# paTRICK-swk/D3DP

Hardware: AMD Instinct MI355X
Metric: pose-hypotheses/sec (H x clips) at F=243, J=17, H=20, K=10 (higher is better)
Workload: dtype f16x2-split operands on fp16 MFMA, f32 accumulate (fp32-class: meets 1e-3 mm)

## Files before the change

d3dp_amd/csrc/capi.hip:

```cpp
#include <hip/hip_runtime.h>

#include <cmath>
#include <cstdarg>
#include <cstdio>
#include <cstdlib>
#include <cstring>
#include <string>
#include <vector>

#include "../../include/d3dp_hip.h"
#include "common.h"
#include "kernels.h"

namespace {

thread_local std::string g_err;

int fail(int code, const char* fmt, ...) {
  char buf[512];
  va_list ap;
  va_start(ap, fmt);
  vsnprintf(buf, sizeof buf, fmt, ap);
  va_end(ap);
  g_err = buf;
  return code;
}

#define HIP_TRY(expr)                                                                      \
  do {                                                                                     \
    hipError_t e__ = (expr);                                                               \
    if (e__ != hipSuccess) return fail(D3DP_EHIP, "%s: %s", #expr, hipGetErrorString(e__)); \
  } while (0)

#define LAUNCH_TRY(expr)                                                          \
  do {                                                                            \
    int r__ = (expr);                                                             \
    if (r__ != 0) return fail(r__ == -1 ? D3DP_EINVAL : D3DP_ENOTSUP, "%s -> %d", #expr, r__); \
  } while (0)

}

int d3dp_set_error(int code, const char* msg) { return fail(code, "%s", msg); }
int d3dp_check_launch(const char* what) {
  hipError_t e = hipGetLastError();
  if (e != hipSuccess) return fail(D3DP_EHIP, "%s: %s", what, hipGetErrorString(e));
  return D3DP_OK;
}

namespace {

enum ProfClass { P_QKV = 0, P_PROJ, P_FC1, P_FC2, P_ATTN_S, P_ATTN_T, P_LN, P_LN2, P_EMBED, P_HEAD, P_TIME, P_OTHER,
                 T_LINEAR, T_WGRAD, T_ATTN_FWD_S, T_ATTN_FWD_T, T_ATTN_BQ_S, T_ATTN_BQ_T, T_ATTN_BKV_S, T_ATTN_BKV_T, T_OPERAND,
                 T_LN_FWD, T_LN_BWD, T_OTHER,
                 P_EMPTY };
static_assert(P_EMPTY + 1 == D3DP_PROFILE_CLASSES, "include/d3dp_hip.h: D3DP_PROFILE_CLASSES");
const char* kClassNames[D3DP_PROFILE_CLASSES] = {"gemm_qkv", "gemm_proj", "gemm_fc1", "gemm_fc2", "attn_spatial",
                                                 "attn_temporal", "layernorm", "norm_pair", "embed_ln", "head",
                                                 "time_mlp", "other",
                                                 "train_linear", "train_wgrad", "train_attn_fwd_spatial", "train_attn_fwd_temporal",
                                                 "train_attn_bwd_q_spatial", "train_attn_bwd_q_temporal", "train_attn_bwd_kv_spatial",
                                                 "train_attn_bwd_kv_temporal", "train_operand_pass", "train_ln_fwd", "train_ln_bwd",
                                                 "train_other", "event_pair_overhead"};

struct BlockDev {
  const float *n1w, *n1b, *n2w, *n2b, *qkv_b, *proj_b, *fc1_b, *fc2_b;
  const void *qkv_w, *proj_w, *fc1_w, *fc2_w;
  float qkv_u = 1.f, proj_u = 1.f, fc1_u = 1.f, fc2_u = 1.f;
  const float* fc1_c12 = nullptr;
  float s_kv = kActScale, s_h = kActScale;
};

template <typename E>
__global__ void to_bf16_kernel(const float* __restrict__ s, E* __restrict__ d, size_t n) {
  size_t i = (size_t)blockIdx.x * blockDim.x + threadIdx.x;
  const size_t stride = (size_t)gridDim.x * blockDim.x;
  for (; i < n; i += stride) d[i] = (E)s[i];
}

void launch_to_bf16(const float* s, void* d, size_t n, hipStream_t st, int f16 = 0) {
  const unsigned blocks = (unsigned)std::min<size_t>((n + 255) / 256, 4096);
  if (f16) hipLaunchKernelGGL(to_bf16_kernel<_Float16>, dim3(blocks ? blocks : 1), dim3(256), 0, st, s, (_Float16*)d, n);
  else hipLaunchKernelGGL(to_bf16_kernel<__bf16>, dim3(blocks ? blocks : 1), dim3(256), 0, st, s, (__bf16*)d, n);
}

__device__ __forceinline__ unsigned f32_bits_up(double v) {
  float f = (float)v;
  if ((double)f < v) f = __uint_as_float(__float_as_uint(f) + 1u);
  return __float_as_uint(f) & 0x7fffffffu;
}
__device__ __forceinline__ unsigned wave_max_u(unsigned v) {
#pragma unroll
  for (int o = 32; o > 0; o >>= 1) { const unsigned t = (unsigned)__shfl_xor((int)v, o, 64); v = t > v ? t : v; }
  return v;
}
__global__ __launch_bounds__(256) void fast16_bound_kernel(const float* __restrict__ W, const float* __restrict__ gamma,
                                                           const float* __restrict__ beta, const unsigned* __restrict__ cin,
                                                           const float* __restrict__ bias, int N, int K, double sq, int n_tail,
                                                           unsigned* o_sum, unsigned* o_tail, unsigned* o_in, unsigned* o_w) {
  const int lane = threadIdx.x & 63;
  const int n = blockIdx.x * 4 + (threadIdx.x >> 6);
  if (n >= N) return;
  const double c = cin ? (double)__uint_as_float(cin[0]) : 0.0;
  double a = 0.0;
  unsigned inmax = 0u, wmax = 0u;
  for (int k = lane; k < K; k += 64) {
    const float w = fabsf(W[(size_t)n * K + k]);
    const double in = gamma ? sq * (double)fabsf(gamma[k]) + (double)fabsf(beta[k]) : c;
    const unsigned ib = f32_bits_up(in), wb = __float_as_uint(w);
    inmax = ib > inmax ? ib : inmax;
    wmax = wb > wmax ? wb : wmax;
    a += (double)w * in;
  }
#pragma unroll
  for (int o = 32; o > 0; o >>= 1) a += __shfl_xor(a, o, 64);
  inmax = wave_max_u(inmax);
  wmax = wave_max_u(wmax);
  if (lane == 0) {
    const unsigned sb = f32_bits_up((a + (double)fabsf(bias[n])) * (1.0 + 0x1p-40));
    atomicMax(o_sum, sb);
    if (o_tail && n >= n_tail) atomicMax(o_tail, sb);
    if (o_in) atomicMax(o_in, inmax);
    atomicMax(o_w, wmax);
  }
}
constexpr int kF16Slots = 11;

constexpr size_t kAlign = 256;
size_t align_up(size_t v) { return (v + kAlign - 1) / kAlign * kAlign; }

}

struct d3dp_ctx {
  d3dp_cfg cfg{};
  int device = 0;
  bool weights_set = false;
  float range_bound = 0.f;
  size_t ln_slice_floats = 0;
  unsigned* d_flag = nullptr;
  char* arena = nullptr;
  size_t arena_bytes = 0;
  const float *spos = nullptr, *tpos = nullptr, *ew = nullptr, *eb = nullptr, *freq = nullptr, *t1w = nullptr,
              *t1b = nullptr, *t3w = nullptr, *t3b = nullptr, *snw = nullptr, *snb = nullptr, *tnw = nullptr,
              *tnb = nullptr, *hnw = nullptr, *hnb = nullptr, *hw = nullptr, *hb = nullptr;
  std::vector<BlockDev> ste, tte;
  bool prof = false;
  struct Ev { hipEvent_t a, b; int cls; };
  std::vector<Ev> pool;
  size_t used = 0;
  int64_t counts[D3DP_PROFILE_CLASSES] = {0};
  double total_ms[D3DP_PROFILE_CLASSES] = {0};

  bool fast16() const { return cfg.mode == D3DP_MODE_FAST16; }
  bool fast() const { return cfg.mode == D3DP_MODE_FAST || fast16(); }
  int fast_f16 = 0;
  float fast_bound = 0.f;
  int exact_impl = 0;
  int exact_impl_req = 0;
  bool impl_fallback = false;
  bool train() const { return cfg.mode == D3DP_MODE_TRAIN; }
  bool exact() const { return !fast() && !train(); }
  bool x2() const { return exact() && exact_impl == 0; }
  bool long_rows = false;
  bool x2_attn() const { return x2() && cfg.channels / cfg.heads == 64 && (cfg.frames <= 256 || !long_rows); }
  bool fold_resid() const { return x2() && fold; }
  bool fold = true;
  bool fold_ln() const { return fold_resid() && fold_ln_on && 2 * cfg.hidden <= 2048; }
  bool fold_ln_on = false;
  bool skew() const { return x2_attn() && skew_d > 0 && cfg.channels >= 128 * skew_d; }
  int skew_d = 0;
  int seq_pitch() const {
    const int fj = cfg.frames * cfg.joints;
    return (pad_override < 0 ? skew() : (pad_override > 0 && x2_attn())) ? (fj + 63) / 64 * 64 : fj;
  }
  int pad_override = -1;
  bool train_x2 = true;
  hipStream_t aux = nullptr;
  hipEvent_t ev_fork = nullptr, ev_done[2] = {nullptr, nullptr};
  bool train_overlap = true;
  int train_overlap_sets = 2;
  bool train_gelu_in_prep = true;
  bool train_ln_direct = true;
  bool train_wgrad_merged = true;
  bool train_tail_blocks = true;
  int train_attn_x2 = 2;
  int pingpong = 0;
  bool x3() const { return exact() && exact_impl == 1; }
  int act() const { return fast() ? (fast_f16 ? 4 : 1) : (x3() ? 2 : (x2() ? 3 : 0)); }
  size_t act_size() const { return fast() ? 2 : (x3() ? 6 : 4); }
  size_t wide_size() const { return fast() ? 2 : 4; }
  size_t y_size() const { return fast() ? 2 : 4; }
  int chunk() const { return cfg.chunk_seqs != 0 ? std::abs(cfg.chunk_seqs) : (exact() ? 31 : 15); }
  int n_cu = 0;
  std::vector<int> plan_cache;
  int plan_total = -1;
  const std::vector<int>& plan(int total) {
    if (total == plan_total) return plan_cache;
    const int cap = std::min(chunk(), total), SP = seq_pitch();
    plan_cache.clear();
    plan_total = total;
    if (!x2() || cfg.chunk_seqs < 0 || n_cu <= 0) {
      for (int s0 = 0; s0 < total; s0 += cap) plan_cache.push_back(std::min(cap, total - s0));
      return plan_cache;
    }
    const long tn[4] = {(3 * cfg.channels + 127) / 128, (cfg.channels + 127) / 128, (cfg.hidden + 127) / 128,
                        (cfg.channels + 127) / 128};
    const long kd[4] = {cfg.channels, cfg.channels, cfg.channels, cfg.hidden};
    const bool sk[4] = {skew(), false, skew(), false};
    std::vector<double> cost(cap + 1, 0.0);
    for (int n = 1; n <= cap; ++n) {
      const long R = ((long)n * SP + 255) / 256;
      for (int k = 0; k < 4; ++k) {
        const long Q = n_cu / tn[k];
        if (sk[k] && Q >= 1) cost[n] += ((double)((R + std::min(Q, R) - 1) / std::min(Q, R)) + 3.0 * skew_d * 32.0 / (double)kd[k]) * (double)kd[k];
        else cost[n] += (double)((R * tn[k] + n_cu - 1) / n_cu) * (double)kd[k];
      }
      cost[n] += 1e-3 * (double)kd[0];
    }
    std::vector<double> best(total + 1, 1e300);
    std::vector<int> pick(total + 1, 0);
    best[0] = 0.0;
    for (int b = 1; b <= total; ++b)
      for (int n = 1; n <= std::min(cap, b); ++n)
        if (best[b - n] + cost[n] < best[b]) { best[b] = best[b - n] + cost[n]; pick[b] = n; }
    for (int b = total; b > 0; b -= pick[b]) plan_cache.push_back(pick[b]);
    return plan_cache;
  }

  int flush_events() {
    for (size_t i = 0; i < used; ++i) {
      if (hipEventSynchronize(pool[i].b) != hipSuccess) return -1;
      float ms = 0.f;
      if (hipEventElapsedTime(&ms, pool[i].a, pool[i].b) != hipSuccess) return -1;
      counts[pool[i].cls]++;
      total_ms[pool[i].cls] += ms;
    }
    used = 0;
    return 0;
  }
  int begin(int cls, hipStream_t st) {
    if (!prof) return -1;
    if (used == pool.size()) {
      if (pool.size() >= 32768) { if (flush_events() != 0) return -1; }
      else {
        Ev e{};
        if (hipEventCreateWithFlags(&e.a, hipEventDisableSystemFence) != hipSuccess || hipEventCreateWithFlags(&e.b, hipEventDisableSystemFence) != hipSuccess) return -1;
        pool.push_back(e);
      }
    }
    pool[used].cls = cls;
    (void)hipEventRecord(pool[used].a, st);
    return (int)used++;
  }
  void end(int slot, hipStream_t st) {
    if (slot >= 0) (void)hipEventRecord(pool[slot].b, st);
  }
};

namespace {

struct Scope {
  d3dp_ctx* c; int slot; hipStream_t st;
  Scope(d3dp_ctx* c_, int cls, hipStream_t st_) : c(c_), slot(c_ ? c_->begin(cls, st_) : -1), st(st_) {}
  ~Scope() { if (c) c->end(slot, st); }
};

int linear(d3dp_ctx* c, int cls, int epi, int out_f32, const void* A, const void* W, float wu, const float* bias, void* out,
           int M, int N, int K, hipStream_t st, void* out2 = nullptr, float* aux = nullptr, float a_scale = kActScale,
           float o_scale = kActScale) {
  Scope s(c, cls, st);
  if (c->fast()) return d3dp_launch_linear_bf16_stream(epi, out_f32, A, W, bias, out, M, N, K, st, c->fast_f16);
  if (c->x2()) {
    if (cls == P_QKV && c->x2_attn()) epi = EPI_QKV_PACK;
    const int skew_d = c->skew() && (epi == EPI_QKV_PACK || epi == EPI_GELU) ? c->skew_d : 0;
    const int rev = cls == P_PROJ ? X2_TILES_LAST_TO_FIRST : 0;
    return d3dp_launch_linear_f16x2(epi, A, W, bias, wu / a_scale, o_scale, (float*)out, out2 ? out2 : out, aux, c->d_flag, M, N,
                                    K, st, skew_d, c->pingpong | rev);
  }
  if (c->x3()) return d3dp_launch_linear_bf16x3(epi, A, W, bias, (float*)out, out, M, N, K, st);
  return d3dp_launch_linear_f32(epi, (const float*)A, (const float*)W, bias, (float*)out, M, N, K, st);
}

SeqMap spatial_map(int F, int J, int sp = 0) { return sp > F * J ? SeqMap{J, F, sp, J, 1} : SeqMap{J, 1, J, 0, 1}; }
SeqMap temporal_map(int F, int J, int sp = 0) { return SeqMap{F, J, sp > F * J ? sp : F * J, 1, J}; }

int attention(d3dp_ctx* c, int axis, const void* qkv, void* out, int n_bh, float s_kv, hipStream_t st) {
  const d3dp_cfg& g = c->cfg;
  Scope s(c, axis == 0 ? P_ATTN_S : P_ATTN_T, st);
  if (c->x2_attn())
    return d3dp_launch_attn_x2(3, axis, qkv, out, axis == 0 ? n_bh * g.frames : n_bh * g.joints,
                               axis == 0 ? spatial_map(g.frames, g.joints, c->seq_pitch())
                                         : temporal_map(g.frames, g.joints, c->seq_pitch()),
                               g.channels, g.heads, s_kv, st);
  const bool fast_mfma = c->fast() && g.channels / g.heads == 64;
  if (axis == 0) {
    if (fast_mfma && g.joints <= 32)
      return d3dp_launch_attn_spatial_bf16(qkv, out, n_bh * g.frames, spatial_map(g.frames, g.joints), g.channels,
                                           g.heads, st, c->fast_f16);
    if (fast_mfma && !c->long_rows)
      return d3dp_launch_attn_temporal_bf16(qkv, out, n_bh * g.frames, spatial_map(g.frames, g.joints), g.channels,
                                            g.heads, st, c->fast_f16);
    return d3dp_launch_attn_rows(c->act(), qkv, out, n_bh * g.frames, spatial_map(g.frames, g.joints), g.channels,
                                 g.heads, st);
  }
  if (fast_mfma && (g.frames <= 256 || !c->long_rows))
    return d3dp_launch_attn_temporal_bf16(qkv, out, n_bh * g.joints, temporal_map(g.frames, g.joints), g.channels,
                                          g.heads, st, c->fast_f16);
  if (c->exact() && g.channels / g.heads == 64 && g.frames <= 256)
    return d3dp_launch_attn_temporal_f32(c->act(), qkv, out, n_bh * g.joints, temporal_map(g.frames, g.joints),
                                         g.channels, g.heads, st);
  return d3dp_launch_attn_rows(c->act(), qkv, out, n_bh * g.joints, temporal_map(g.frames, g.joints), g.channels,
                               g.heads, st);
}

int run_block(d3dp_ctx* c, const BlockDev& w, int axis, float* x, void* y1, void* y, void* bufA, void* bufB, float* lnst,
              int n_bh, hipStream_t st) {
  const d3dp_cfg& g = c->cfg;
  const int Tc = n_bh * c->seq_pitch(), C = g.channels;
  const float s_o = c->x2_attn() ? w.s_kv : kActScale;
  LAUNCH_TRY(linear(c, P_QKV, EPI_BIAS, 0, bufA, w.qkv_w, w.qkv_u, w.qkv_b, bufB, Tc, 3 * C, C, st, nullptr, nullptr, kActScale, s_o));
  LAUNCH_TRY(attention(c, axis, bufB, bufA, n_bh, s_o, st));
  const bool fold = c->fold_resid();
  if (c->fold_ln()) {
    float* slices = lnst;
    float* rowstat = lnst + (size_t)c->ln_slice_floats;
    LAUNCH_TRY(linear(c, P_PROJ, EPI_RESID_LN, 0, bufA, w.proj_w, w.proj_u, w.proj_b, x, Tc, C, C, st, y1, slices, s_o));
    {
      Scope s(c, P_LN, st);
      d3dp_launch_ln_combine(slices, rowstat, Tc, C, g.eps_block, st);
    }
    LAUNCH_TRY(linear(c, P_FC1, EPI_GELU_LN, 0, y1, w.fc1_w, w.fc1_u, w.fc1_c12, bufB, Tc, g.hidden, C, st, bufB, rowstat, kActScale, w.s_h));
  } else {
  LAUNCH_TRY(linear(c, P_PROJ, fold ? EPI_RESID : EPI_BIAS, 0, bufA, w.proj_w, w.proj_u, w.proj_b, fold ? (void*)x : y1, Tc, C, C, st, nullptr, nullptr, s_o));
  {
    Scope s(c, P_LN, st);
    LAUNCH_TRY(d3dp_launch_ln(c->act(), x, fold ? nullptr : y1, 0, w.n2w, w.n2b, g.eps_block, bufA, Tc, C, st));
  }
  LAUNCH_TRY(linear(c, P_FC1, EPI_GELU, 0, bufA, w.fc1_w, w.fc1_u, w.fc1_b, bufB, Tc, g.hidden, C, st, nullptr, nullptr, kActScale, w.s_h));
  }
  LAUNCH_TRY(linear(c, P_FC2, fold ? EPI_RESID : EPI_BIAS, 0, bufB, w.fc2_w, w.fc2_u, w.fc2_b, fold ? (void*)x : y, Tc, C, g.hidden, st, nullptr, nullptr, w.s_h));
  return 0;
}

int read_switches(d3dp_ctx* c, bool width_inst) {
  const d3dp_cfg& g = c->cfg;
  const char* xf = getenv("D3DP_EXACT_IMPL");
  c->exact_impl = c->exact_impl_req = (xf && !strcmp(xf, "bf16x3")) ? 1 : (xf && !strcmp(xf, "f32")) ? 2 : 0;
  if (!width_inst) {
    if (c->exact_impl_req == 1)
      return fail(D3DP_ENOTSUP, "D3DP_EXACT_IMPL=bf16x3 exists for channels in {64,128,256,512}; channels=%d runs the fp32 implementation", g.channels);
    c->exact_impl = c->exact_impl_req = 2;
  }
  const char* lr = getenv("D3DP_LONG_ATTN");
  c->long_rows = lr && !strcmp(lr, "rows");
  const char* nf = getenv("D3DP_NO_FOLD");
  c->fold = !(nf && nf[0] == '1');
  const char* ti = getenv("D3DP_TRAIN_IMPL");
  c->train_x2 = !(ti && !strcmp(ti, "f32")) && width_inst;
  const char* ov = getenv("D3DP_TRAIN_OVERLAP");
  c->train_overlap = !(ov && ov[0] == '0');
  c->train_overlap_sets = (ov && ov[0] == '1') ? 1 : 2;
  const char* tg = getenv("D3DP_TRAIN_GELU");
  c->train_gelu_in_prep = !(tg && !strcmp(tg, "pass"));
  const char* tw = getenv("D3DP_TRAIN_WGRAD");
  c->train_wgrad_merged = !(tw && !strcmp(tw, "each"));
  const char* tl = getenv("D3DP_TRAIN_LN_OPERAND");
  c->train_ln_direct = !(tl && !strcmp(tl, "pass"));
  const char* tt = getenv("D3DP_TRAIN_TAIL");
  c->train_tail_blocks = !(tt && !strcmp(tt, "split"));
  const char* ta = getenv("D3DP_TRAIN_ATTN");
  c->train_attn_x2 = (ta && !strcmp(ta, "f32")) ? 0 : (ta && !strcmp(ta, "x2t")) ? 1 : 2;
  if ((!c->train_gelu_in_prep || !c->train_wgrad_merged || !c->train_tail_blocks || !c->train_ln_direct) && !d3dp_x2_variants_built())
    return fail(D3DP_ENOTSUP, "D3DP_TRAIN_WGRAD=each / D3DP_TRAIN_TAIL=split / D3DP_TRAIN_GELU=pass / D3DP_TRAIN_LN_OPERAND=pass select superseded launch forms of the "
                              "training step that only the variants build honours (make -C d3dp_amd/csrc variants; "
                              "D3DP_LIB=d3dp_amd/lib/variants/libd3dp_variants.so)");
  {
    const char* sk = getenv("D3DP_X2_SKEW");
    const char* pp = getenv("D3DP_X2_PP");
    const char* wide = getenv("D3DP_X2_WIDE");
    const char* pd = getenv("D3DP_SEQ_PAD");
    const char* nl = getenv("D3DP_FOLD_LN");
    int skew_d = 0, pingpong = 0, pad = -1;
    if (sk && (sk[0] == '0' || sk[0] == '1' || sk[0] == '2' || sk[0] == '4') && sk[1] == 0) skew_d = sk[0] - '0';
    if (pp && (pp[0] == '0' || pp[0] == '1') && pp[1] == 0) pingpong = pp[0] - '0';
    if (wide && wide[0] == '1' && wide[1] == 0) pingpong = 2;
    if (pd && (pd[0] == '0' || pd[0] == '1') && pd[1] == 0) pad = pd[0] - '0';
    const bool fold_ln = nl && nl[0] == '1';
    if ((skew_d || pingpong || pad > 0 || fold_ln) && !d3dp_x2_variants_built())
      return fail(D3DP_ENOTSUP, "D3DP_X2_SKEW / D3DP_X2_PP / D3DP_X2_WIDE / D3DP_SEQ_PAD / D3DP_FOLD_LN select experiment kernels that this "
                                "library was built without (make -C d3dp_amd/csrc variants; D3DP_LIB=d3dp_amd/lib/variants/libd3dp_variants.so)");
    c->skew_d = skew_d; c->pingpong = pingpong; c->pad_override = pad; c->fold_ln_on = fold_ln;
  }
  return D3DP_OK;
}

}

extern "C" {

int d3dp_abi_version(void) { return D3DP_ABI_VERSION; }
int d3dp_debug_x2_variants(void) { return d3dp_x2_variants_built() ? 1 : 0; }
int d3dp_debug_train_linear(const float* A, const float* W, const float* bias, float* out, int32_t M, int32_t N, int32_t K,
                            int32_t tail, unsigned* amax_out, int32_t amax_pos, void* stream) {
  if (!A || !W || !out || M < 1 || N < 4 || N % 4 || K < 32 || K % 32) return fail(D3DP_EINVAL, "d3dp_debug_train_linear: bad argument");
  hipStream_t st = (hipStream_t)stream;
  char* buf = nullptr;
  const size_t a_bytes = (size_t)M * K * 4, w_bytes = (size_t)N * K * 4;
  HIP_TRY(hipMalloc((void**)&buf, a_bytes + w_bytes + 64));
  unsigned* amax = reinterpret_cast<unsigned*>(buf + a_bytes + w_bytes);
  float* uns = reinterpret_cast<float*>(amax + 8);
  int rc = hipMemsetAsync(amax, 0, 64, st) == hipSuccess ? 0 : -3;
  if (!rc) {
    d3dp_launch_absmax(A, (size_t)M * K, amax, st);
    d3dp_launch_absmax(W, (size_t)N * K, amax + 1, st);
    d3dp_launch_split2_dyn(A, buf, M, K, K, amax, uns, st);
    d3dp_launch_split2_dyn(W, buf + a_bytes, N, K, K, amax + 1, uns + 1, st);
    rc = d3dp_launch_linear_f16x2_dyn(buf, buf + a_bytes, bias, uns, uns + 1, out, M, N, K, 1, st, amax_out, amax_pos, tail);
  }
  const hipError_t e = hipStreamSynchronize(st);
  (void)hipFree(buf);
  if (rc) return fail(rc == -3 ? D3DP_EHIP : D3DP_EINVAL, "d3dp_debug_train_linear: launch refused (%d)", rc);
  if (e != hipSuccess) return fail(D3DP_EHIP, "d3dp_debug_train_linear: %s", hipGetErrorString(e));
  return 0;
}
const char* d3dp_last_error(void) { return g_err.c_str(); }
const char* d3dp_profile_class_name(int32_t cls) {
  return (cls >= 0 && cls < D3DP_PROFILE_CLASSES) ? kClassNames[cls] : "";
}

int d3dp_create(const d3dp_cfg* cfg, d3dp_ctx** out) {
  if (!cfg || !out) return fail(D3DP_EINVAL, "d3dp_create: null argument");
  const d3dp_cfg& g = *cfg;
  if (g.frames < 1 || g.frames > 1024) return fail(D3DP_ENOTSUP, "frames=%d not in [1,1024]", g.frames);
  if (g.joints < 1 || g.joints > 256) return fail(D3DP_ENOTSUP, "joints=%d not in [1,256]", g.joints);
  if (g.heads < 1 || g.channels < 1 || g.channels % g.heads) return fail(D3DP_EINVAL, "heads=%d does not divide channels=%d", g.heads, g.channels);
  if (g.depth < 1) return fail(D3DP_EINVAL, "depth=%d", g.depth);
  if (g.mode != D3DP_MODE_EXACT && g.mode != D3DP_MODE_FAST && g.mode != D3DP_MODE_TRAIN && g.mode != D3DP_MODE_FAST16)
    return fail(D3DP_EINVAL, "mode=%d", g.mode);
  const int hd = g.channels / g.heads;
  const bool width_inst = (g.channels == 64 || g.channels == 128 || g.channels == 256 || g.channels == 512) &&
                          (hd == 8 || hd == 16 || hd == 32 || hd == 64) && g.hidden >= 64 && g.hidden % 64 == 0;
  if (!width_inst) {
    if (g.mode == D3DP_MODE_FAST)
      return fail(D3DP_ENOTSUP, "channels=%d heads=%d hidden=%d: FAST contexts exist for channels in {64,128,256,512} with head dim in "
                                "{8,16,32,64} and hidden a multiple of 64; other widths run in D3DP_MODE_EXACT / D3DP_MODE_TRAIN (fp32 implementation)",
                  g.channels, g.heads, g.hidden);
    if (g.mode == D3DP_MODE_FAST16)
      return fail(D3DP_ENOTSUP, "channels=%d heads=%d hidden=%d: FAST16 contexts exist for the shapes FAST contexts exist for -- channels in "
                                "{64,128,256,512} with head dim in {8,16,32,64} and hidden a multiple of 64; other widths run in D3DP_MODE_EXACT / "
                                "D3DP_MODE_TRAIN (fp32 implementation)",
                  g.channels, g.heads, g.hidden);
    if (g.channels > 1024 || g.channels % 4 || hd % 4 || hd > 128 || g.hidden < 4 || g.hidden % 4)
      return fail(D3DP_ENOTSUP, "channels=%d heads=%d hidden=%d: the fp32 implementation takes channels <= 1024, head dim a multiple of 4 up to 128 "
                                "and hidden a multiple of 4", g.channels, g.heads, g.hidden);
    const int nmax = std::max(g.frames, g.joints), cap = hd <= 16 ? 16 : hd <= 32 ? 32 : hd <= 64 ? 64 : 128;
    if (g.mode == D3DP_MODE_TRAIN && (nmax > 256 || (size_t)nmax * (8 * (cap + 4) + 12) > 160 * 1024))
      return fail(D3DP_ENOTSUP, "channels=%d heads=%d frames=%d joints=%d: training at a width outside {64,128,256,512} runs the fp32 attention "
                                "backward, which holds a whole sequence in LDS (<= 256 tokens; <= 153 at head dims above 64)",
                  g.channels, g.heads, g.frames, g.joints);
  }
  int ndev = 0;
  if (hipGetDeviceCount(&ndev) != hipSuccess || ndev < 1)
    return fail(D3DP_EHIP, "no HIP device visible: libd3dp_hip has no CPU fallback");
  d3dp_ctx* c = new d3dp_ctx();
  c->cfg = g;
  c->fast_f16 = c->fast16() ? 1 : (c->fast() ? D3DP_FAST_F16 : 0);
  if (const int rc = read_switches(c, width_inst); rc != D3DP_OK) {
    delete c;
    return rc;
  }
  HIP_TRY(hipGetDevice(&c->device));
  {
    hipDeviceProp_t prop;
    HIP_TRY(hipGetDeviceProperties(&prop, c->device));
    c->n_cu = prop.multiProcessorCount;
  }
  if (hipMalloc((void**)&c->d_flag, sizeof(unsigned)) != hipSuccess || hipMemset(c->d_flag, 0, sizeof(unsigned)) != hipSuccess) {
    delete c;
    return fail(D3DP_EHIP, "d3dp_create: cannot allocate the status word");
  }
  if (g.mode == D3DP_MODE_TRAIN && c->train_x2 && c->train_overlap && g.channels % 32 == 0 && g.hidden % 32 == 0) {
    bool ok = hipStreamCreateWithFlags(&c->aux, hipStreamNonBlocking) == hipSuccess &&
              hipEventCreateWithFlags(&c->ev_fork, hipEventDisableTiming) == hipSuccess;
    for (hipEvent_t& e : c->ev_done) ok = ok && hipEventCreateWithFlags(&e, hipEventDisableTiming) == hipSuccess;
    if (!ok) {
      (void)d3dp_destroy(c);
      return fail(D3DP_EHIP, "d3dp_create: cannot create the training step's second stream and its events");
    }
  }
  *out = c;
  return D3DP_OK;
}

int d3dp_destroy(d3dp_ctx* c) {
  if (!c) return D3DP_OK;
  for (auto& e : c->pool) { (void)hipEventDestroy(e.a); (void)hipEventDestroy(e.b); }
  if (c->arena) (void)hipFree(c->arena);
  if (c->d_flag) (void)hipFree(c->d_flag);
  if (c->ev_fork) (void)hipEventDestroy(c->ev_fork);
  for (hipEvent_t e : c->ev_done)
    if (e) (void)hipEventDestroy(e);
  if (c->aux) (void)hipStreamDestroy(c->aux);
  delete c;
  return D3DP_OK;
}

int d3dp_set_weights(d3dp_ctx* c, const d3dp_weights* w, void* stream) {
  if (!c || !w || !w->ste || !w->tte) return fail(D3DP_EINVAL, "d3dp_set_weights: null argument");
  hipStream_t st = (hipStream_t)stream;
  const d3dp_cfg& g = c->cfg;
  const size_t C = g.channels, Hd = g.hidden, J = g.joints, F = g.frames;
  c->range_bound = 0.f;
  c->impl_fallback = false;
  c->plan_total = -1;
  std::vector<float> blk_scale(4 * (size_t)g.depth, kActScale);
  if (c->exact() && c->exact_impl_req == 0) {
    c->exact_impl = 0;
    const size_t nb = 2 * (size_t)g.depth;
    unsigned* dbound = nullptr;
    HIP_TRY(hipMalloc((void**)&dbound, nb * 6 * sizeof(unsigned)));
    struct Free { unsigned* p; ~Free() { (void)hipFree(p); } } free_dbound{dbound};
    HIP_TRY(hipMemsetAsync(dbound, 0, nb * 6 * sizeof(unsigned), st));
    for (int kind = 0; kind < 2; ++kind)
      for (int d = 0; d < g.depth; ++d) {
        const d3dp_block_weights& b = (kind == 0 ? w->ste : w->tte)[d];
        if (!b.norm1_w || !b.norm1_b || !b.qkv_w || !b.qkv_b || !b.norm2_w || !b.norm2_b || !b.fc1_w || !b.fc1_b || !b.proj_w ||
            !b.fc2_w)
          return fail(D3DP_EINVAL, "d3dp_set_weights: a weight pointer is null");
        unsigned* o = dbound + ((size_t)kind * g.depth + d) * 6;
        d3dp_launch_rowbound(b.qkv_w, b.norm1_w, b.norm1_b, b.qkv_b, 3 * (int)C, (int)C, o, st);
        d3dp_launch_rowbound(b.fc1_w, b.norm2_w, b.norm2_b, b.fc1_b, (int)Hd, (int)C, o + 2, st);
        d3dp_launch_absmax(b.proj_w, C * C, o + 4, st);
        d3dp_launch_absmax(b.fc2_w, C * Hd, o + 5, st);
      }
    std::vector<float> hb(nb * 6);
    HIP_TRY(hipMemcpyAsync(hb.data(), dbound, nb * 6 * sizeof(float), hipMemcpyDeviceToHost, st));
    HIP_TRY(hipStreamSynchronize(st));
    const float kSafe = 65504.0f / kActScale;
    auto pick = [&](float bound) {
      float sc = kActScale;
      while (!(bound * sc < 65504.0f) && sc > 1e-30f) sc *= 0.5f;
      return sc;
    };
    float worst = 0.f;
    bool fallback = false;
    for (size_t i = 0; i < nb; ++i) {
      const float bq = hb[6 * i], bl1 = hb[6 * i + 1], bh = hb[6 * i + 2], bl2 = hb[6 * i + 3];
      if (!(bq < INFINITY) || !(bh < INFINITY) || !(bl1 < INFINITY) || !(bl2 < INFINITY) || !(hb[6 * i + 4] < INFINITY) ||
          !(hb[6 * i + 5] < INFINITY)) {
        fallback = true;
        worst = INFINITY;
        continue;
      }
      worst = std::max(worst, std::max(std::max(bq, bh), std::max(bl1, bl2)));
      if (!(bl1 < kSafe) || !(bl2 < kSafe)) fallback = true;
      if (!(bq < kSafe) && !c->x2_attn()) fallback = true;
      blk_scale[2 * i] = pick(bq);
      blk_scale[2 * i + 1] = pick(bh);
    }
    c->range_bound = std::min(worst, 3.0e38f);
    if (fallback) {
      c->exact_impl = 1;
      c->impl_fallback = true;
      std::fill(blk_scale.begin(), blk_scale.end(), kActScale);
    }
  }
  if (c->fast16()) {
    const size_t nb = 2 * (size_t)g.depth;
    unsigned* dbound = nullptr;
    HIP_TRY(hipMalloc((void**)&dbound, nb * kF16Slots * sizeof(unsigned)));
    struct Free { unsigned* p; ~Free() { (void)hipFree(p); } } free_dbound{dbound};
    HIP_TRY(hipMemsetAsync(dbound, 0, nb * kF16Slots * sizeof(unsigned), st));
    const double sq = std::sqrt((double)C - 1.0);
    for (int kind = 0; kind < 2; ++kind)
      for (int d = 0; d < g.depth; ++d) {
        const d3dp_block_weights& b = (kind == 0 ? w->ste : w->tte)[d];
        if (!b.norm1_w || !b.norm1_b || !b.qkv_w || !b.qkv_b || !b.proj_w || !b.proj_b || !b.norm2_w || !b.norm2_b || !b.fc1_w ||
            !b.fc1_b || !b.fc2_w || !b.fc2_b) return fail(D3DP_EINVAL, "d3dp_set_weights: a weight pointer is null");
        unsigned* o = dbound + ((size_t)kind * g.depth + d) * kF16Slots;
        const dim3 blk(256);
        hipLaunchKernelGGL(fast16_bound_kernel, dim3((3 * (unsigned)C + 3) / 4), blk, 0, st, b.qkv_w, b.norm1_w, b.norm1_b,
                           (const unsigned*)nullptr, b.qkv_b, 3 * (int)C, (int)C, sq, 2 * (int)C, o + 1, o + 2, o + 0, o + 7);
        hipLaunchKernelGGL(fast16_bound_kernel, dim3(((unsigned)C + 3) / 4), blk, 0, st, b.proj_w, (const float*)nullptr,
                           (const float*)nullptr, (const unsigned*)(o + 2), b.proj_b, (int)C, (int)C, 0.0, 0, o + 3,
                           (unsigned*)nullptr, (unsigned*)nullptr, o + 8);
        hipLaunchKernelGGL(fast16_bound_kernel, dim3(((unsigned)Hd + 3) / 4), blk, 0, st, b.fc1_w, b.norm2_w, b.norm2_b,
                           (const unsigned*)nullptr, b.fc1_b, (int)Hd, (int)C, sq, 0, o + 5, (unsigned*)nullptr, o + 4, o + 9);
        hipLaunchKernelGGL(fast16_bound_kernel, dim3(((unsigned)C + 3) / 4), blk, 0, st, b.fc2_w, (const float*)nullptr,
                           (const float*)nullptr, (const unsigned*)(o + 5), b.fc2_b, (int)C, (int)Hd, 0.0, 0, o + 6,
                           (unsigned*)nullptr, (unsigned*)nullptr, o + 10);
      }
    HIP_TRY(hipGetLastError());
    std::vector<float> hb(nb * kF16Slots);
    HIP_TRY(hipMemcpyAsync(hb.data(), dbound, hb.size() * sizeof(float), hipMemcpyDeviceToHost, st));
    HIP_TRY(hipStreamSynchronize(st));
    float worst = 0.f;
    bool finite = true;
    for (const float v : hb) {
      if (!(v < INFINITY)) finite = false;
      else worst = std::max(worst, v);
    }
    c->fast_bound = finite ? worst : INFINITY;
    c->fast_f16 = (finite && worst < 65504.0f) ? 1 : 0;
  }
  const size_t ws = c->fast() ? 2 : (c->x3() ? 6 : 4);
  size_t off = 0;
  auto take = [&](size_t bytes) { size_t o = off; off += align_up(bytes); return o; };
  struct Item { const void* src; size_t n; bool mat; size_t off; };
  std::vector<Item> items;
  auto add = [&](const void* src, size_t n, bool mat) {
    items.push_back({src, n, mat, take(n * (mat ? ws : 4))});
    return items.size() - 1;
  };
  const size_t i_spos = add(w->spatial_pos, J * C, false), i_tpos = add(w->temporal_pos, F * C, false);
  const size_t i_ew = add(w->embed_w, C * 5, false), i_eb = add(w->embed_b, C, false);
  const size_t i_fr = add(w->time_freq, C / 2, false);
  const size_t i_t1w = add(w->time1_w, 2 * C * C, false), i_t1b = add(w->time1_b, 2 * C, false);
  const size_t i_t3w = add(w->time3_w, 2 * C * C, false), i_t3b = add(w->time3_b, C, false);
  const size_t i_snw = add(w->spatial_norm_w, C, false), i_snb = add(w->spatial_norm_b, C, false);
  const size_t i_tnw = add(w->temporal_norm_w, C, false), i_tnb = add(w->temporal_norm_b, C, false);
  const size_t i_hnw = add(w->head_norm_w, C, false), i_hnb = add(w->head_norm_b, C, false);
  const size_t i_hw = add(w->head_w, 3 * C, false), i_hb = add(w->head_b, 3, false);
  struct BI { size_t v[13]; };
  std::vector<BI> bis;
  std::vector<float*> temps;
  struct TempFree { std::vector<float*>& t; ~TempFree() { for (float* p : t) (void)hipFree(p); } } temp_free{temps};
  for (int kind = 0; kind < 2; ++kind)
    for (int d = 0; d < g.depth; ++d) {
      const d3dp_block_weights& b = (kind == 0 ? w->ste : w->tte)[d];
      if (!b.norm1_w || !b.norm1_b || !b.qkv_w || !b.qkv_b || !b.proj_w || !b.proj_b || !b.norm2_w || !b.norm2_b || !b.fc1_w ||
          !b.fc1_b || !b.fc2_w || !b.fc2_b) return fail(D3DP_EINVAL, "d3dp_set_weights: a weight pointer is null");
      BI bi;
      bi.v[0] = add(b.norm1_w, C, false); bi.v[1] = add(b.norm1_b, C, false);
      bi.v[2] = add(b.qkv_w, 3 * C * C, true); bi.v[3] = add(b.qkv_b, 3 * C, false);
      bi.v[4] = add(b.proj_w, C * C, true); bi.v[5] = add(b.proj_b, C, false);
      bi.v[6] = add(b.norm2_w, C, false); bi.v[7] = add(b.norm2_b, C, false);
      if (c->fold_ln()) {
        float *wp = nullptr, *c12 = nullptr;
        HIP_TRY(hipMalloc((void**)&wp, Hd * C * 4)); temps.push_back(wp);
        HIP_TRY(hipMalloc((void**)&c12, 2 * Hd * 4)); temps.push_back(c12);
        d3dp_launch_fold_ln(b.fc1_w, b.norm2_w, b.norm2_b, b.fc1_b, wp, c12, (int)Hd, (int)C, st);
        bi.v[8] = add(wp, Hd * C, true); bi.v[9] = add(b.fc1_b, Hd, false); bi.v[12] = add(c12, 2 * Hd, false);
      } else {
        bi.v[8] = add(b.fc1_w, Hd * C, true); bi.v[9] = add(b.fc1_b, Hd, false); bi.v[12] = bi.v[9];
      }
      bi.v[10] = add(b.fc2_w, C * Hd, true); bi.v[11] = add(b.fc2_b, C, false);
      bis.push_back(bi);
    }
  for (auto& it : items)
    if (!it.src) return fail(D3DP_EINVAL, "d3dp_set_weights: a weight pointer is null");
  if (!c->arena || c->arena_bytes < off) {
    if (c->arena) HIP_TRY(hipFree(c->arena));
    c->arena = nullptr;
    HIP_TRY(hipMalloc((void**)&c->arena, off));
    c->arena_bytes = off;
  }
  std::vector<float> unscale(items.size(), 1.f);
  if (c->x2()) {
    size_t n_mat = 0;
    for (auto& it : items) n_mat += it.mat;
    unsigned* dmax = nullptr;
    HIP_TRY(hipMalloc((void**)&dmax, n_mat * sizeof(unsigned)));
    HIP_TRY(hipMemsetAsync(dmax, 0, n_mat * sizeof(unsigned), st));
    size_t k = 0;
    for (auto& it : items)
      if (it.mat) d3dp_launch_absmax((const float*)it.src, it.n, dmax + k++, st);
    std::vector<float> hmax(n_mat);
    HIP_TRY(hipMemcpyAsync(hmax.data(), dmax, n_mat * sizeof(float), hipMemcpyDeviceToHost, st));
    HIP_TRY(hipStreamSynchronize(st));
    HIP_TRY(hipFree(dmax));
    k = 0;
    for (size_t i = 0; i < items.size(); ++i) {
      if (!items[i].mat) continue;
      const float mx = hmax[k++];
      if (!(mx < INFINITY)) return fail(D3DP_EINVAL, "d3dp_set_weights: a weight matrix holds inf/nan");
      int e = 0;
      if (mx > 0.f) frexpf(mx, &e);
      unscale[i] = ldexpf(1.f, e - 14);
    }
  }
  for (size_t i = 0; i < items.size(); ++i) {
    auto& it = items[i];
    if (it.mat && c->fast()) launch_to_bf16((const float*)it.src, c->arena + it.off, it.n, st, c->fast_f16);
    else if (it.mat && c->x3()) d3dp_launch_split3((const float*)it.src, c->arena + it.off, it.n, st);
    else if (it.mat && c->x2()) d3dp_launch_split2((const float*)it.src, c->arena + it.off, it.n, 1.0f / unscale[i], st);
    else HIP_TRY(hipMemcpyAsync(c->arena + it.off, it.src, it.n * 4, hipMemcpyDeviceToDevice, st));
  }
  HIP_TRY(hipGetLastError());
  HIP_TRY(hipStreamSynchronize(st));
  auto F32 = [&](size_t i) { return (const float*)(c->arena + items[i].off); };
  auto ANY = [&](size_t i) { return (const void*)(c->arena + items[i].off); };
  c->spos = F32(i_spos); c->tpos = F32(i_tpos); c->ew = F32(i_ew); c->eb = F32(i_eb); c->freq = F32(i_fr);
  c->t1w = F32(i_t1w); c->t1b = F32(i_t1b); c->t3w = F32(i_t3w); c->t3b = F32(i_t3b);
  c->snw = F32(i_snw); c->snb = F32(i_snb); c->tnw = F32(i_tnw); c->tnb = F32(i_tnb);
  c->hnw = F32(i_hnw); c->hnb = F32(i_hnb); c->hw = F32(i_hw); c->hb = F32(i_hb);
  c->ste.clear(); c->tte.clear();
  for (size_t k = 0; k < bis.size(); ++k) {
    const BI& bi = bis[k];
    BlockDev b{F32(bi.v[0]), F32(bi.v[1]), F32(bi.v[6]), F32(bi.v[7]), F32(bi.v[3]), F32(bi.v[5]), F32(bi.v[9]),
               F32(bi.v[11]), ANY(bi.v[2]), ANY(bi.v[4]), ANY(bi.v[8]), ANY(bi.v[10]),
               unscale[bi.v[2]], unscale[bi.v[4]], unscale[bi.v[8]], unscale[bi.v[10]], F32(bi.v[12]),
               blk_scale[2 * k], blk_scale[2 * k + 1]};
    (k < (size_t)g.depth ? c->ste : c->tte).push_back(b);
  }
  c->weights_set = true;
  return D3DP_OK;
}

int d3dp_set_weights_borrowed(d3dp_ctx* c, const d3dp_weights* w) {
  if (!c || !w || !w->ste || !w->tte) return fail(D3DP_EINVAL, "d3dp_set_weights_borrowed: null argument");
  if (!c->train()) return fail(D3DP_ESTATE, "d3dp_set_weights_borrowed needs a D3DP_MODE_TRAIN context (fp32 weights)");
  c->spos = w->spatial_pos; c->tpos = w->temporal_pos; c->ew = w->embed_w; c->eb = w->embed_b; c->freq = w->time_freq;
  c->t1w = w->time1_w; c->t1b = w->time1_b; c->t3w = w->time3_w; c->t3b = w->time3_b;
  c->snw = w->spatial_norm_w; c->snb = w->spatial_norm_b; c->tnw = w->temporal_norm_w; c->tnb = w->temporal_norm_b;
  c->hnw = w->head_norm_w; c->hnb = w->head_norm_b; c->hw = w->head_w; c->hb = w->head_b;
  const float* top[] = {c->spos, c->tpos, c->ew, c->eb, c->freq, c->t1w, c->t1b, c->t3w, c->t3b, c->snw, c->snb, c->tnw,
                        c->tnb, c->hnw, c->hnb, c->hw, c->hb};
  for (const float* p : top)
    if (!p) return fail(D3DP_EINVAL, "d3dp_set_weights_borrowed: a weight pointer is null");
  c->ste.clear(); c->tte.clear();
  for (int kind = 0; kind < 2; ++kind)
    for (int d = 0; d < c->cfg.depth; ++d) {
      const d3dp_block_weights& b = (kind == 0 ? w->ste : w->tte)[d];
      const void* all[] = {b.norm1_w, b.norm1_b, b.qkv_w, b.qkv_b, b.proj_w, b.proj_b, b.norm2_w, b.norm2_b, b.fc1_w,
                           b.fc1_b, b.fc2_w, b.fc2_b};
      for (const void* p : all)
        if (!p) return fail(D3DP_EINVAL, "d3dp_set_weights_borrowed: a weight pointer is null");
      BlockDev bd{b.norm1_w, b.norm1_b, b.norm2_w, b.norm2_b, b.qkv_b, b.proj_b, b.fc1_b, b.fc2_b, b.qkv_w, b.proj_w,
                  b.fc1_w, b.fc2_w};
      (kind == 0 ? c->ste : c->tte).push_back(bd);
    }
  c->weights_set = true;
  return D3DP_OK;
}

int d3dp_workspace_bytes(const d3dp_ctx* c, int32_t B, int32_t H, size_t* bytes) {
  if (!c || !bytes || B < 1 || H < 1) return fail(D3DP_EINVAL, "d3dp_workspace_bytes: bad argument");
  const d3dp_cfg& g = c->cfg;
  const size_t n = (size_t)std::min(c->chunk(), B * H);
  const size_t Tc = n * c->seq_pitch(), C = g.channels;
  const size_t wide = (size_t)std::max(3 * g.channels, g.hidden);
  *bytes = align_up((size_t)B * C * 4) + align_up(Tc * C * 4) + 2 * align_up(Tc * C * c->y_size()) +
           align_up(Tc * C * c->act_size()) + align_up(Tc * wide * c->wide_size()) +
           (c->fold_ln() ? align_up(Tc * ((C + 63) / 64) * 8) + align_up((Tc + 256) * 8) : 0);
  return D3DP_OK;
}

int d3dp_denoise(d3dp_ctx* c, const float* x2d, const float* x_t, const int64_t* t, float* out, int32_t B, int32_t H,
                 void* workspace, size_t workspace_bytes, void* stream) {
  if (!c || !x2d || !x_t || !t || !out || !workspace || B < 1 || H < 1)
    return fail(D3DP_EINVAL, "d3dp_denoise: bad argument");
  if (!c->weights_set) return fail(D3DP_ESTATE, "d3dp_denoise: weights not set");
  size_t need = 0;
  d3dp_workspace_bytes(c, B, H, &need);
  if (workspace_bytes < need) return fail(D3DP_ESTATE, "workspace %zu < required %zu bytes", workspace_bytes, need);
  hipStream_t st = (hipStream_t)stream;
  const d3dp_cfg& g = c->cfg;
  const int C = g.channels, F = g.frames, J = g.joints, FJ = F * J, SP = c->seq_pitch();
  const int BH = B * H, chunk = std::min(c->chunk(), BH);
  const size_t Tmax = (size_t)chunk * SP;
  char* p = (char*)workspace;
  float* temb = (float*)p; p += align_up((size_t)B * C * 4);
  float* x = (float*)p;    p += align_up(Tmax * C * 4);
  void* y1 = p;            p += align_up(Tmax * C * c->y_size());
  void* y = p;             p += align_up(Tmax * C * c->y_size());
  void* bufA = p;          p += align_up(Tmax * C * c->act_size());
  void* bufB = p;          p += align_up(Tmax * (size_t)std::max(3 * g.channels, g.hidden) * c->wide_size());
  float* lnst = (float*)p;
  c->ln_slice_floats = align_up(Tmax * ((C + 63) / 64) * 8) / 4;

  {
    Scope s(c, P_TIME, st);
    LAUNCH_TRY(d3dp_launch_time_mlp(t, c->freq, c->t1w, c->t1b, c->t3w, c->t3b, temb, B, C, st));
  }
  int seq0 = 0;
  for (const int n : c->plan(BH)) {
    const int Tc = n * SP;
    {
      Scope s(c, P_EMBED, st);
      LAUNCH_TRY(d3dp_launch_embed_ln(c->act(), x2d, x_t, temb, c->ew, c->eb, c->spos, c->ste[0].n1w, c->ste[0].n1b,
                                      g.eps_block, x, bufA, seq0, n, H, F, J, C, st, SP));
    }
    const bool fold = c->fold_resid();
    for (int d = 0; d < g.depth; ++d) {
      int r = run_block(c, c->ste[d], 0, x, y1, y, bufA, bufB, lnst, n, st);
      if (r) return r;
      {
        Scope s(c, P_LN2, st);
        LAUNCH_TRY(d3dp_launch_ln2(c->act(), x, fold ? nullptr : y1, fold ? nullptr : y, c->snw, c->snb, d == 0 ? c->tpos : nullptr, c->tte[d].n1w,
                                   c->tte[d].n1b, g.eps_block, bufA, Tc, C, F, J, st, SP));
      }
      r = run_block(c, c->tte[d], 1, x, y1, y, bufA, bufB, lnst, n, st);
      if (r) return r;
      if (d + 1 < g.depth) {
        Scope s(c, P_LN2, st);
        LAUNCH_TRY(d3dp_launch_ln2(c->act(), x, fold ? nullptr : y1, fold ? nullptr : y, c->tnw, c->tnb, nullptr, c->ste[d + 1].n1w, c->ste[d + 1].n1b,
                                   g.eps_block, bufA, Tc, C, F, J, st, SP));
      }
    }
    {
      Scope s(c, P_HEAD, st);
      LAUNCH_TRY(d3dp_launch_head(c->fast() ? c->act() : 0, x, fold ? nullptr : y1, fold ? nullptr : y, c->tnw, c->tnb, g.eps_block, c->hnw, c->hnb, g.eps_head, c->hw, c->hb,
                                  out + (size_t)seq0 * FJ * 3, Tc, C, st, FJ, SP));
    }
    seq0 += n;
  }
  d3dp_launch_nonfinite_flag(out, (size_t)BH * FJ * 3, c->d_flag, st);
  HIP_TRY(hipGetLastError());
  return D3DP_OK;
}

int d3dp_exact_range_bound(const d3dp_ctx* c, float* bound) {
  if (!c || !bound) return fail(D3DP_EINVAL, "d3dp_exact_range_bound: null argument");
  if (!c->weights_set) return fail(D3DP_ESTATE, "d3dp_exact_range_bound: weights not set");
  *bound = c->range_bound;
  return D3DP_OK;
}

int d3dp_exact_scales(const d3dp_ctx* c, float* s_kv, float* s_hidden, int32_t* implementation) {
  if (!c) return fail(D3DP_EINVAL, "d3dp_exact_scales: null argument");
  if (!c->weights_set) return fail(D3DP_ESTATE, "d3dp_exact_scales: weights not set");
  const int dep = c->cfg.depth;
  for (int i = 0; i < 2 * dep; ++i) {
    const BlockDev& b = i < dep ? c->ste[i] : c->tte[i - dep];
    if (s_kv) s_kv[i] = b.s_kv;
    if (s_hidden) s_hidden[i] = b.s_h;
  }
  if (implementation) *implementation = c->exact() ? c->exact_impl : -1;
  return D3DP_OK;
}

int d3dp_fast_operands(const d3dp_ctx* c, int32_t* type, float* bound) {
  if (!c || !type || !bound) return fail(D3DP_EINVAL, "d3dp_fast_operands: null argument");
  if (!c->weights_set) return fail(D3DP_ESTATE, "d3dp_fast_operands: weights not set");
  *type = c->fast() ? c->fast_f16 : -1;
  *bound = c->fast16() ? c->fast_bound : 0.f;
  return D3DP_OK;
}

int d3dp_status(d3dp_ctx* c, int32_t* nonfinite) {
  if (!c || !nonfinite) return fail(D3DP_EINVAL, "d3dp_status: null argument");
  unsigned v = 0;
  HIP_TRY(hipDeviceSynchronize());
  HIP_TRY(hipMemcpy(&v, c->d_flag, sizeof v, hipMemcpyDeviceToHost));
  HIP_TRY(hipMemset(c->d_flag, 0, sizeof v));
  *nonfinite = (int32_t)(v != 0u);
  return D3DP_OK;
}

int d3dp_ddim_pre(const float* img, float* xt2, const int32_t* perm, float scale, int32_t B, int32_t H, int32_t F,
                  int32_t J, void* stream) {
  if (!img || !xt2 || !perm || B < 1) return fail(D3DP_EINVAL, "d3dp_ddim_pre: bad argument");
  LAUNCH_TRY(d3dp_launch_ddim_pre(img, xt2, perm, scale, B, H * F * J * 3, J, (hipStream_t)stream));
  HIP_TRY(hipGetLastError());
  return D3DP_OK;
}

int d3dp_ddim_post(const float* pred2, const float* img, const float* noise, const int32_t* perm, float scale,
                   double sqrt_recip, double sqrt_recipm1, float c_xstart, float c_noise, float sigma, int32_t last,
                   float* x_start, size_t xs_bstride, float* img_next, int32_t B, int32_t H, int32_t F, int32_t J,
                   void* stream) {
  if (!pred2 || !perm || !x_start || B < 1) return fail(D3DP_EINVAL, "d3dp_ddim_post: bad argument");
  if (!last && (!img || !noise || !img_next)) return fail(D3DP_EINVAL, "d3dp_ddim_post: img/noise/img_next required");
  LAUNCH_TRY(d3dp_launch_ddim_post(pred2, img, noise, perm, scale, sqrt_recip, sqrt_recipm1, c_xstart, c_noise, sigma,
                                   last, x_start, xs_bstride, img_next, B, H * F * J * 3, J, (hipStream_t)stream));
  HIP_TRY(hipGetLastError());
  return D3DP_OK;
}

int d3dp_q_sample(const float* x0, const float* noise, const double* a, const double* s, float scale, float* out,
                  int32_t B, int32_t per_b, void* stream) {
  if (!x0 || !noise || !a || !s || !out || B < 1 || per_b < 1) return fail(D3DP_EINVAL, "d3dp_q_sample: bad argument");
  LAUNCH_TRY(d3dp_launch_q_sample(x0, noise, a, s, scale, out, B, per_b, (hipStream_t)stream));
  HIP_TRY(hipGetLastError());
  return D3DP_OK;
}

int d3dp_jpma(const float* pred, const float* traj, const float* cam, const float* gt2d, const float* gt3d, float* agg,
              int32_t* sel, float* err_sel, float* err_min, int32_t B, int32_t K, int32_t H, int32_t F, int32_t J,
              int32_t zero_root, void* stream) {
  if (!pred || !traj || !cam || !gt2d || !agg || B < 1 || K < 1 || H < 1)
    return fail(D3DP_EINVAL, "d3dp_jpma: bad argument");
  if ((err_sel || err_min) && !gt3d) return fail(D3DP_EINVAL, "d3dp_jpma: error outputs need gt3d");
  LAUNCH_TRY(d3dp_launch_jpma(pred, traj, cam, gt2d, gt3d, agg, sel, err_sel, err_min, nullptr, nullptr, nullptr, 0, B,
                              K, H, F, J, zero_root ? 0 : -1, 0, (hipStream_t)stream));
  HIP_TRY(hipGetLastError());
  return D3DP_OK;
}

int d3dp_jpma_gathered(const float* gathered, const float* traj, const float* cam, const float* gt2d, const float* gt3d,
                       float* agg, int32_t* sel, float* err_sel, float* err_min, int32_t R, int32_t B, int32_t K,
                       int32_t H_local, int32_t F, int32_t J, int32_t zero_root, void* stream) {
  if (!gathered || !traj || !cam || !gt2d || !agg || R < 1 || B < 1 || K < 1 || H_local < 1)
    return fail(D3DP_EINVAL, "d3dp_jpma_gathered: bad argument");
  if ((err_sel || err_min) && !gt3d) return fail(D3DP_EINVAL, "d3dp_jpma_gathered: error outputs need gt3d");
  LAUNCH_TRY(d3dp_launch_jpma(gathered, traj, cam, gt2d, gt3d, agg, sel, err_sel, err_min, nullptr, nullptr, nullptr, 0, B,
                              K, R * H_local, F, J, zero_root ? 0 : -1, 0, (hipStream_t)stream, H_local,
                              (size_t)B * K * H_local * F * J * 3));
  HIP_TRY(hipGetLastError());
  return D3DP_OK;
}

int d3dp_jpma_ex(const float* pred, const float* traj, const float* cam, const float* gt2d, const float* gt3d, float* agg,
                 int32_t* sel, float* err_sel, float* err_min, float* jbest, float* mean, int32_t B, int32_t K, int32_t H,
                 int32_t F, int32_t J, int32_t root_joint, int32_t linear_projection, void* stream) {
  if (!pred || !traj || !cam || !gt2d || B < 1 || K < 1 || H < 1 || root_joint >= J)
    return fail(D3DP_EINVAL, "d3dp_jpma_ex: bad argument");
  if ((err_sel || err_min || jbest) && !gt3d) return fail(D3DP_EINVAL, "d3dp_jpma_ex: error / J-Best outputs need gt3d");
  LAUNCH_TRY(d3dp_launch_jpma(pred, traj, cam, gt2d, gt3d, agg, sel, err_sel, err_min, nullptr, jbest, mean, 0, B, K, H,
                              F, J, root_joint, linear_projection, (hipStream_t)stream));
  HIP_TRY(hipGetLastError());
  return D3DP_OK;
}

int d3dp_jpma_winners(const float* pred, const float* traj, const float* cam, const float* gt2d, float* win,
                      int32_t h_offset, int32_t B, int32_t K, int32_t H, int32_t F, int32_t J, int32_t zero_root,
                      void* stream) {
  if (!pred || !traj || !cam || !gt2d || !win || B < 1 || K < 1 || H < 1 || h_offset < 0)
    return fail(D3DP_EINVAL, "d3dp_jpma_winners: bad argument");
  LAUNCH_TRY(d3dp_launch_jpma(pred, traj, cam, gt2d, nullptr, nullptr, nullptr, nullptr, nullptr, win, nullptr, nullptr,
                              h_offset, B, K, H, F, J, zero_root ? 0 : -1, 0, (hipStream_t)stream));
  HIP_TRY(hipGetLastError());
  return D3DP_OK;
}

int d3dp_op_linear(int32_t mode, int32_t epi, const void* A, const void* W, const float* bias, void* out, int32_t M,
                   int32_t N, int32_t K, void* stream) {
  if (!A || !W || !bias || !out) return fail(D3DP_EINVAL, "d3dp_op_linear: null argument");
  if (mode == D3DP_MODE_FAST || mode == 4) {
    const int e = epi & 3, f32 = (epi & 16) != 0;
    if (e == EPI_RESID || (epi & ~19)) return fail(D3DP_EINVAL, "d3dp_op_linear: FAST mode has epilogues 0, 1 and 0|16");
    LAUNCH_TRY(d3dp_launch_linear_bf16_stream(e, f32, A, W, bias, out, M, N, K, (hipStream_t)stream, mode == 4));
  }
  else if (mode == 2) {
    LAUNCH_TRY(d3dp_launch_linear_bf16x3(epi, A, W, bias, (float*)out, out, M, N, K, (hipStream_t)stream));
  }

  else LAUNCH_TRY(d3dp_launch_linear_f32(epi, (const float*)A, (const float*)W, bias, (float*)out, M, N, K, (hipStream_t)stream));
  HIP_TRY(hipGetLastError());
  return D3DP_OK;
}

int d3dp_op_split3(const float* src, void* dst, size_t n, void* stream) {
  if (!src || !dst) return fail(D3DP_EINVAL, "d3dp_op_split3: null argument");
  d3dp_launch_split3(src, dst, n, (hipStream_t)stream);
  HIP_TRY(hipGetLastError());
  return D3DP_OK;
}

int d3dp_op_linear_x2(int32_t epi, const void* A2, const void* W2, const float* bias, float w_scale, void* out, int32_t M,
                      int32_t N, int32_t K, void* stream) {
  if (!A2 || !W2 || !bias || !out || !(w_scale > 0.f)) return fail(D3DP_EINVAL, "d3dp_op_linear_x2: bad argument");
  const int skew_d = (epi >> 8) & 7;
  const int pingpong = (epi >> 12) & 1 ? 2 : (epi >> 11) & 1;
  if ((skew_d || pingpong) && !d3dp_x2_variants_built())
    return fail(D3DP_ENOTSUP, "d3dp_op_linear_x2: epi flags %d select an experiment kernel this library was built without "
                              "(make -C d3dp_amd/csrc variants)", epi & ~0xff);
  epi &= 255;
  if (epi == EPI_RESID_LN || epi == EPI_GELU_LN) return fail(D3DP_EINVAL, "d3dp_op_linear_x2: epilogues 5 / 6 are internal to d3dp_denoise");
  if (skew_d) {
    int dev = 0;
    hipDeviceProp_t prop;
    HIP_TRY(hipGetDevice(&dev));
    HIP_TRY(hipGetDeviceProperties(&prop, dev));
    if (!d3dp_x2_skew_applies(epi, M, N, K, skew_d, prop.multiProcessorCount))
      return fail(D3DP_EINVAL, "d3dp_op_linear_x2: the skewed schedule (D = %d) does not apply to epi %d, M = %d, N = %d, K = %d", skew_d, epi, M, N, K);
  }
  LAUNCH_TRY(d3dp_launch_linear_f16x2(epi, A2, W2, bias, kActUnscale / w_scale, kActScale, (float*)out, out, nullptr, nullptr, M, N, K, (hipStream_t)stream, skew_d, pingpong));
  HIP_TRY(hipGetLastError());
  return D3DP_OK;
}

int d3dp_op_split2(const float* src, void* dst, size_t n, float scale, void* stream) {
  if (!src || !dst) return fail(D3DP_EINVAL, "d3dp_op_split2: null argument");
  if (n % 32 != 0) return fail(D3DP_EINVAL, "d3dp_op_split2: n = %zu is not a multiple of 32 (the h2i layout is made of whole 32-column blocks)", n);
  d3dp_launch_split2(src, dst, n, scale, (hipStream_t)stream);
  HIP_TRY(hipGetLastError());
  return D3DP_OK;
}

int d3dp_op_attention(int32_t act_bf16, int32_t impl, int32_t axis, const void* qkv, void* out, int32_t n_bh, int32_t F,
                      int32_t J, int32_t C, int32_t heads, void* stream) {
  if (!qkv || !out || n_bh < 1) return fail(D3DP_EINVAL, "d3dp_op_attention: bad argument");
  hipStream_t st = (hipStream_t)stream;
  if (act_bf16 != 0 && act_bf16 != 1 && act_bf16 != 4) return fail(D3DP_EINVAL, "act_bf16 must be 0, 1 or 4 (fp16)");
  const int f16 = act_bf16 == 4;
  if (impl == 2) {
    if (act_bf16) return fail(D3DP_EINVAL, "split-fp16 attention takes fp32 activations");
    void* packed = nullptr;
    const size_t T = (size_t)n_bh * F * J;
    HIP_TRY(hipMallocAsync(&packed, T * 12 * (size_t)C, st));
    d3dp_launch_qkv_pack_x2((const float*)qkv, packed, T, C, kActScale, st);
    const int rc = d3dp_launch_attn_x2(0, axis, packed, out, axis == 0 ? n_bh * F : n_bh * J,
                                       axis == 0 ? spatial_map(F, J) : temporal_map(F, J), C, heads, kActScale, st);
    HIP_TRY(hipFreeAsync(packed, st));
    LAUNCH_TRY(rc);
  } else if (axis == 0 && impl == 1) {
    if (!act_bf16) return fail(D3DP_EINVAL, "MFMA spatial attention needs bf16 activations");
    if (J <= 32) LAUNCH_TRY(d3dp_launch_attn_spatial_bf16(qkv, out, n_bh * F, spatial_map(F, J), C, heads, st, f16));
    else if (J > 256) return fail(D3DP_ENOTSUP, "MFMA spatial attention takes up to 256 joints; J=%d", J);
    else LAUNCH_TRY(d3dp_launch_attn_temporal_bf16(qkv, out, n_bh * F, spatial_map(F, J), C, heads, st, f16));
  } else if (axis == 0) LAUNCH_TRY(d3dp_launch_attn_rows(act_bf16, qkv, out, n_bh * F, spatial_map(F, J), C, heads, st));
  else if (impl == 1 && !act_bf16) {
    LAUNCH_TRY(d3dp_launch_attn_temporal_f32(0, qkv, out, n_bh * J, temporal_map(F, J), C, heads, st));
  } else if (impl == 1) {
    if (!act_bf16) return fail(D3DP_EINVAL, "MFMA temporal attention needs bf16 activations");
    LAUNCH_TRY(d3dp_launch_attn_temporal_bf16(qkv, out, n_bh * J, temporal_map(F, J), C, heads, st, f16));
  } else LAUNCH_TRY(d3dp_launch_attn_rows(act_bf16, qkv, out, n_bh * J, temporal_map(F, J), C, heads, st));
  HIP_TRY(hipGetLastError());
  return D3DP_OK;
}

int d3dp_op_layernorm(int32_t out_bf16, const float* x, const float* w, const float* b, float eps, void* out, int32_t T,
                      int32_t C, void* stream) {
  if (!x || !w || !b || !out) return fail(D3DP_EINVAL, "d3dp_op_layernorm: null argument");
  LAUNCH_TRY(d3dp_launch_ln(out_bf16, const_cast<float*>(x), nullptr, 0, w, b, eps, out, T, C, (hipStream_t)stream));
  HIP_TRY(hipGetLastError());
  return D3DP_OK;
}

int d3dp_op_to_bf16(const float* src, void* dst, size_t n, void* stream) {
  if (!src || !dst) return fail(D3DP_EINVAL, "d3dp_op_to_bf16: null argument");
  launch_to_bf16(src, dst, n, (hipStream_t)stream);
  HIP_TRY(hipGetLastError());
  return D3DP_OK;
}

int d3dp_profile_enable(d3dp_ctx* c, int32_t on) {
  if (!c) return fail(D3DP_EINVAL, "null ctx");
  c->prof = on != 0;
  c->used = 0;
  memset(c->counts, 0, sizeof c->counts);
  for (auto& v : c->total_ms) v = 0.0;
  return D3DP_OK;
}

int d3dp_profile_read(d3dp_ctx* c, int64_t* counts, double* total_ms) {
  if (!c || !counts || !total_ms) return fail(D3DP_EINVAL, "null argument");
  if (c->flush_events() != 0) return fail(D3DP_EHIP, "event read failed");
  for (int i = 0; i < D3DP_PROFILE_CLASSES; ++i) { counts[i] = c->counts[i]; total_ms[i] = c->total_ms[i]; }
  memset(c->counts, 0, sizeof c->counts);
  for (auto& v : c->total_ms) v = 0.0;
  return D3DP_OK;
}

}

namespace {

struct TrainLayout {
  size_t T, Tpad, C, Hd, unit;
  size_t temb, x_final, zero_bias, saved0, saved_stride, tmp0;
  size_t o_xin, o_qkv, o_att, o_xmid, o_hpre, o_xout;
  size_t xn, y, hid, dA, dB, dC, dqkv, dh, z, At, Xt, Wt, dtemb, stats;
  size_t op_a, op_w, op_at, op_xt, part, part_rem, slots;
  size_t part_floats;
  size_t op_a2, op_at2, part2;
  size_t x_cols, x_block;
  size_t w_rows, w_cols, w_block;
  size_t Tp_max;
  size_t stats_x2, stats_x2_stride;
  size_t red, red_floats;
  size_t total_floats;
};

constexpr int kGroupSlices = 32;

TrainLayout train_layout(const d3dp_cfg& g, int B) {
  TrainLayout L{};
  L.T = (size_t)B * g.frames * g.joints;
  L.Tpad = (L.T + 15) / 16 * 16;
  L.C = g.channels; L.Hd = g.hidden; L.unit = L.T * L.C;
  size_t off = 0;
  auto take = [&](size_t n) { size_t o = off; off += (n + 63) / 64 * 64; return o; };
  L.temb = take((size_t)B * L.C);
  L.x_final = take(L.unit);
  L.zero_bias = take(4 * L.C);
  L.o_xin = 0; L.o_qkv = L.unit; L.o_att = 4 * L.unit; L.o_xmid = 5 * L.unit; L.o_hpre = 6 * L.unit;
  L.o_xout = 6 * L.unit + L.T * L.Hd;
  L.saved_stride = (7 * L.unit + L.T * L.Hd + 63) / 64 * 64;
  L.saved0 = take(L.saved_stride * 2 * g.depth);
  L.xn = take(L.unit); L.y = take(L.unit); L.hid = take(L.T * L.Hd);
  L.dA = take(L.unit); L.dB = take(L.unit); L.dC = take(L.unit);
  L.dqkv = take(3 * L.unit); L.dh = take(L.T * L.Hd); L.z = take(L.unit);
  const size_t wide = std::max<size_t>(3 * L.C, L.Hd);
  L.At = take(wide * L.Tpad); L.Xt = take(wide * L.Tpad); L.Wt = take(wide * wide);
  L.dtemb = take((size_t)B * 2 * L.C);
  L.stats = take(d3dp_train_attn_stats_bytes(B * std::max(g.frames, g.joints), std::max(g.frames, g.joints), g.heads) / 4 + 64);
  {
    const size_t fmax = std::max<size_t>(3 * L.C, L.Hd), kmax = std::max<size_t>(L.C, L.Hd);
    L.Tp_max = ((L.T + 31) / 32 + 64) * 32;
    const size_t dy_all = 5 * L.C + L.Hd;
    L.op_a = take(L.Tp_max * dy_all);
    L.op_w = take(fmax * kmax);
    L.op_at = take(fmax * L.Tp_max);
    L.op_xt = take(kmax * L.Tp_max);
    L.part_floats = (size_t)(1024 + 64) * 256 * 128;
    L.part = take(L.part_floats);
    L.op_a2 = take(L.Tp_max * dy_all); L.op_at2 = take(fmax * L.Tp_max); L.part2 = take(L.part_floats);
    L.part_rem = take((size_t)16 * 256 * fmax);
    L.slots = take(2 * 8192);
    L.w_block = 4 * L.C * L.C + 2 * L.Hd * L.C;
    L.x_block = (3 * L.C + L.Hd) * L.Tp_max;
    L.x_cols = take(L.x_block * 2 * g.depth);
    L.w_rows = take(L.w_block * 2 * g.depth);
    L.w_cols = take(L.w_block * 2 * g.depth);
  }
  L.stats_x2_stride = (d3dp_train_attn_x2_stats_bytes(B * g.joints, g.frames, g.heads) / 4 + 63) / 64 * 64;
  L.stats_x2 = take(L.stats_x2_stride * 2 * g.depth);
  {
    const size_t lnb = (size_t)D3DP_LN_BWD_BLOCKS * 2 * L.C;
    L.red_floats = (size_t)(6 * g.depth + 2) * lnb
                   + (size_t)2 * g.depth * std::max(D3DP_DYPREP_ROWS, D3DP_ROWPREP_ROWS) * (5 * L.C + L.Hd + 256)
                   + (size_t)512 * (3 * L.C + 4) + (size_t)D3DP_EMBED_BWD_ROWS * 5 * L.C + (size_t)512 * L.C
                   + (size_t)kGroupSlices * (g.joints + (size_t)B) * L.C + 4096;
    L.red = take(L.red_floats);
  }
  L.total_floats = off;
  return L;
}

const float* mask_ptr(const float* masks, const d3dp_cfg& g, int B, int blk, int branch) {
  if (!masks) return nullptr;
  const size_t smax = (size_t)B * std::max(g.frames, g.joints);
  return masks + ((size_t)blk * 2 + branch) * smax;
}

struct Reducer {
  float* base;
  size_t cap, used = 0;
  hipStream_t st;
  std::vector<D3dpReduceItem> items{};
  int rc = 0;
  float* take(size_t n) {
    n = (n + 63) / 64 * 64;
    if (used + n > cap) { rc = -1; return nullptr; }
    float* p = base + used;
    used += n;
    return p;
  }
  void add(const float* part, float* dst, size_t n, size_t count, size_t stride, bool accumulate = false) {
    if (!part || !dst || rc) { rc = rc ? rc : -1; return; }
    items.push_back(D3dpReduceItem{part, dst, (unsigned)n, (unsigned)count, (unsigned)stride, accumulate ? 1u : 0u});
  }
  void flush() {
    for (size_t i = 0; i < items.size() && rc == 0; i += D3DP_REDUCE_MAX) {
      D3dpReduceTable tb{};
      tb.count = (int)std::min<size_t>(D3DP_REDUCE_MAX, items.size() - i);
      for (int j = 0; j < tb.count; ++j) tb.it[j] = items[i + j];
      rc = d3dp_train_reduce_many(tb, st);
    }
    items.clear();
  }
};

int lin32(const float* A, const float* W, const float* bias, float* out, int M, int N, int K, hipStream_t st) {
  return d3dp_launch_linear_f32(EPI_BIAS, A, W, bias, out, M, N, K, st);
}

struct X2Train {
  hipStream_t st;
  float* ws;
  const TrainLayout& L;
  int n_cu;
  d3dp_ctx* pc = nullptr;
  hipStream_t st_w = nullptr;
  bool tail_blocks = true;
  size_t o_a = 0, o_at = 0, o_part = 0, set_base = 0, set_used = 0;
  void use_set(int s) {
    set_base = o_a = s ? L.op_a2 : L.op_a; set_used = 0; n_def = 0;
    o_at = s ? L.op_at2 : L.op_at; o_part = s ? L.part2 : L.part;
  }
  bool merged = false;
  int mZ = 1, mTp = 0, n_def = 0;
  D3dpTnProduct def[D3DP_TN_MAX];
  float* def_dw[D3DP_TN_MAX];
  void merged_setup(int T, bool on) {
    const int C = (int)L.C, Hd = (int)L.Hd;
    const int shapes[4][2] = {{C, Hd}, {Hd, C}, {C, C}, {3 * C, C}};
    int tiles = 0;
    bool ok = on;
    size_t nk_sum = 0;
    for (auto& sh : shapes) { ok = ok && d3dp_tn_applies(sh[0], sh[1]); tiles += ((sh[0] + 255) / 256) * ((sh[1] + 127) / 128); nk_sum += (size_t)sh[0] * sh[1]; }
    const int nk = (T + 31) / 32;
    mZ = std::max(1, std::min(std::min(n_cu / std::max(tiles, 1), 64), nk / 4));
    mTp = mZ * ((nk + mZ - 1) / mZ) * 32;
    merged = ok && (size_t)mTp <= L.Tp_max && (size_t)mZ * nk_sum <= L.part_floats;
  }
  int pad_rows(int T, int N, int K) const {
    int Z, Tp;
    wgrad_split(T, N, K, Z, Tp);
    return merged ? std::max(Tp, mTp) : Tp;
  }
  int flush_wgrads() {
    if (!n_def) return 0;
    hipStream_t sw = st_w ? st_w : st;
    Scope ps(pc, T_WGRAD, sw);
    int r = d3dp_launch_linear_f16x2_tn_many(def, n_def, mTp, mZ, sw);
    if (r) return r;
    D3dpSumTable tb{};
    tb.n = n_def; tb.Z = mZ;
    for (int i = 0; i < n_def; ++i) { tb.part[i] = def[i].out; tb.out[i] = def_dw[i]; tb.n4[i] = (size_t)def[i].N * def[i].K / 4; }
    d3dp_launch_sum_partials_many(tb, sw);
    n_def = 0;
    return 0;
  }
  static constexpr int kBwdSlot0 = 4096;
  static constexpr int kQkvSlot0 = 2048;
  int next = 0;
  unsigned* amax() const { return reinterpret_cast<unsigned*>(ws + L.slots); }
  float* uns() const { return ws + L.slots + 8192; }
  int begin(bool forward_pass) {
    next = forward_pass ? 0 : kBwdSlot0;
    return hipMemsetAsync(ws + L.slots + next, 0, (size_t)kBwdSlot0 * 4, st) == hipSuccess ? 0 : -3;
  }
  int take() { return (next < kBwdSlot0 || next >= 8192) ? -1 : next++; }
  int slot_for(const float* src, size_t n) {
    if (next < kBwdSlot0 || next >= 8192) return -1;
    d3dp_launch_absmax(src, n, amax() + next, st);
    return next++;
  }
  void rows(const float* src, int R, int C, void* dst, int slot) {
    d3dp_launch_split2_dyn(src, dst, R, C, C, amax() + slot, uns() + slot, st);
  }
  void cols(const float* src, int R, int C, int Rpad, void* dst, int slot) {
    d3dp_launch_split2_t_dyn(src, dst, R, C, Rpad, amax() + slot, uns() + slot, st);
  }
  bool batched = false;
  size_t xoff(int l) const { return (size_t)(l >> 2) * L.x_block + (size_t)(l & 3) * L.C * L.Tp_max; }
  size_t woff(int l) const {
    const size_t CC = L.C * L.C, j = (size_t)(l & 3);
    return (size_t)(l >> 2) * L.w_block + (j == 0 ? 0 : j == 1 ? 3 * CC : j == 2 ? 4 * CC : 4 * CC + L.Hd * L.C);
  }
  int prepare_weights(const d3dp_ctx* c) {
    const int nl = 8 * c->cfg.depth;
    batched = nl <= D3DP_WPREP_MAX;
    if (!batched) return 0;
    D3dpWPrepTable tb{};
    tb.n = nl;
    const int C = (int)L.C, Hd = (int)L.Hd;
    for (int l = 0; l < nl; ++l) {
      const int blk = l >> 2, j = l & 3;
      const BlockDev& w = (blk & 1) ? c->tte[blk >> 1] : c->ste[blk >> 1];
      const void* p = j == 0 ? w.qkv_w : j == 1 ? w.proj_w : j == 2 ? w.fc1_w : w.fc2_w;
      tb.it[l] = D3dpWPrepItem{(const float*)p, j == 0 ? 3 * C : j == 2 ? Hd : C, j == 3 ? Hd : C, 2 * l + 1, 0, woff(l)};
    }
    return d3dp_launch_wprep(tb, ws + L.w_rows, ws + L.w_cols, amax(), uns(), st);
  }
  int gemm(const float* A2, const float* W2, const float* bias, const float* ua, const float* uw, float* out, int T, int N,
           int K, unsigned* out_amax = nullptr, int amax_pos = 0) {
    Scope ps(pc, T_LINEAR, st);
    const int tn = (N + 127) / 128, q = T / 256, rem = T - q * 256;
    const int rounds_all = ((q + (rem ? 1 : 0)) * tn + n_cu - 1) / n_cu, rounds_full = (q * tn + n_cu - 1) / n_cu;
    const int nk = K / 32;
    int Z = 1;
    for (int z = 2; z <= 16; ++z)
      if (nk % z == 0) Z = z;
    if (tail_blocks && rem && q && rounds_all > rounds_full && nk % 16 == 0)
      return d3dp_launch_linear_f16x2_dyn(A2, W2, bias, ua, uw, out, T, N, K, 1, st, out_amax, amax_pos, 1);
    if (rem == 0 || q == 0 || rounds_all == rounds_full || Z == 1 || nk < 32 || (size_t)Z * rem * N > (size_t)16 * 256 * std::max<size_t>(3 * L.C, L.Hd))
      return d3dp_launch_linear_f16x2_dyn(A2, W2, bias, ua, uw, out, T, N, K, 1, st, out_amax, amax_pos);
    int r = d3dp_launch_linear_f16x2_dyn(A2, W2, bias, ua, uw, out, q * 256, N, K, 1, st, out_amax, amax_pos);
    if (r) return r;
    r = d3dp_launch_linear_f16x2_dyn(A2 + (size_t)q * 256 * K, W2, nullptr, ua, uw, ws + L.part_rem, rem, N, K, Z, st);
    if (r) return r;
    d3dp_launch_sum_partials_bias(ws + L.part_rem, bias, out + (size_t)q * 256 * N, (size_t)rem * N, N, Z, st, out_amax, amax_pos);
    return 0;
  }
  bool ln_operand_applies(int N, int K) const { return d3dp_tn_applies(N, K) && K <= 512; }
  int forward(int l, const float* A, const float* W, const float* bias, float* out, int T, int N, int K, bool a_amax_ready = false,
              unsigned* out_amax = nullptr, int amax_pos = 0, bool a_prepared = false, const float* ln_w = nullptr,
              const float* ln_b = nullptr, float ln_eps = 0.f) {
    const int sa = 2 * l, sw = 2 * l + 1;
    if (l < 0 || sw >= kBwdSlot0) return -1;
    const float* a2 = ws + o_a;
    if (a_prepared) a2 = ws + L.x_cols + xoff(l);
    else {
      Scope ps(pc, T_OPERAND, st);
      if (!a_amax_ready) d3dp_launch_absmax(A, (size_t)T * K, amax() + sa, st);
      const int Tp = pad_rows(T, N, K);
      if ((size_t)Tp > L.Tp_max) return -1;
      int r;
      if (ln_w) {
        if (!ln_operand_applies(N, K) || !a_amax_ready) return -1;
        a2 = ws + L.x_cols + xoff(l);
        r = d3dp_launch_rowprep_ln(A, ln_w, ln_b, ln_eps, ws + L.x_cols + xoff(l), T, Tp, K, amax() + sa, uns() + sa, st);
      } else if (d3dp_tn_applies(N, K)) {
        a2 = ws + L.x_cols + xoff(l);
        r = d3dp_launch_rowprep(A, ws + L.x_cols + xoff(l), nullptr, nullptr, T, Tp, K, amax() + sa, uns() + sa, st);
      } else r = d3dp_launch_dyprep(A, ws + o_a, ws + L.x_cols + xoff(l), nullptr, T, K, Tp, amax() + sa, uns() + sa, st);
      if (r) return r;
    }
    const float* w2 = ws + L.op_w;
    if (batched) w2 = ws + L.w_rows + woff(l);
    else {
      Scope ps(pc, T_OPERAND, st);
      d3dp_launch_absmax(W, (size_t)N * K, amax() + sw, st);
      rows(W, N, K, ws + L.op_w, sw);
    }
    return gemm(a2, w2, bias, uns() + sa, uns() + sw, out, T, N, K, out_amax, amax_pos);
  }
  bool gelu_operand_applies(int N, int K) const { return d3dp_tn_applies(N, K); }
  static constexpr int kPmaxSlot0 = 3072;
  int gelu_operand(int l, const float* hpre, int blk, int T, int N, int K) {
    const int Tp = pad_rows(T, N, K);
    if ((size_t)Tp > L.Tp_max) return -1;
    Scope ps(pc, T_OPERAND, st);
    return d3dp_launch_gelu_rowprep(hpre, ws + L.x_cols + xoff(l), T, Tp, K, amax() + kPmaxSlot0 + blk, amax() + 2 * l, uns() + 2 * l, st);
  }
  int dgrad(int l, const float* dY, int sdy, const float* W, float* dX, int T, int N, int K, unsigned* out_amax = nullptr) {
    const int sw = 2 * l + 1;
    {
      Scope ps(pc, T_OPERAND, st);
      if (!dy_ready) rows(dY, T, N, ws + o_a, sdy);
      if (!batched) cols(W, N, K, N, ws + L.op_w, sw);
    }
    const float* wt = ws + L.op_w;
    if (batched) wt = ws + L.w_cols + woff(l);
    return gemm(ws + o_a, wt, nullptr, uns() + sdy, uns() + sw, dX, T, K, N, out_amax);
  }
  void wgrad_split(int T, int N, int K, int& Z, int& Tp) const {
    const int tiles = ((N + 255) / 256) * ((K + 127) / 128);
    const int nk = (T + 31) / 32;
    Z = std::max(1, std::min(std::min(n_cu / tiles, 64), nk / 4));
    const int nkz = (nk + Z - 1) / Z;
    Tp = Z * nkz * 32;
  }
  bool dy_ready = false;
  static constexpr int kBiasRows = D3DP_DYPREP_ROWS > D3DP_ROWPREP_ROWS ? D3DP_DYPREP_ROWS : D3DP_ROWPREP_ROWS;
  bool mask_in_prep_applies(int N, int K) const { return d3dp_tn_applies(N, K); }
  bool gelu_in_prep_applies(int N, int K) const { return d3dp_tn_applies(N, K) && N <= 1536; }
  int prep_dy(const float* dY, int sdy, float* bias_part, int* bias_rows, int T, int N, int K, const float* mask = nullptr,
              int axis = 0, int F = 1, int J = 1, const float* gelu_pre = nullptr) {
    const int Tp = pad_rows(T, N, K);
    if ((size_t)Tp > L.Tp_max) return -1;
    if (merged) {
      if (set_used + L.Tp_max * (size_t)N > L.Tp_max * (5 * L.C + L.Hd)) return -1;
      o_a = set_base + set_used;
      set_used += L.Tp_max * (size_t)N;
    }
    dy_ready = true;
    Scope ps(pc, T_OPERAND, st);
    if (d3dp_tn_applies(N, K))
      return d3dp_launch_rowprep(dY, ws + o_a, bias_part, bias_rows, T, Tp, N, amax() + sdy, uns() + sdy, st, mask, axis, F, J,
                                 gelu_pre);
    if (mask || gelu_pre) return -1;
    *bias_rows = D3DP_DYPREP_ROWS;
    return d3dp_launch_dyprep(dY, ws + o_a, ws + o_at, bias_part, T, N, Tp, amax() + sdy, uns() + sdy, st);
  }
  int wgrad(int l, const float* dY, int sdy, const float* X, float* dW, int T, int N, int K) {
    const int sx = 2 * l;
    int Z, Tp;
    wgrad_split(T, N, K, Z, Tp);
    if ((size_t)Tp > L.Tp_max || (size_t)Z * N * K > L.part_floats) return -1;
    (void)X;
    if (merged) {
      if (!dy_ready || n_def >= D3DP_TN_MAX || !d3dp_tn_applies(N, K)) return -1;
      size_t po = 0;
      for (int i = 0; i < n_def; ++i) po += (size_t)mZ * def[i].N * def[i].K;
      def[n_def] = D3dpTnProduct{ws + o_a, ws + L.x_cols + xoff(l), uns() + sdy, uns() + sx, ws + o_part + po, N, K, 0, 0};
      def_dw[n_def++] = dW;
      return 0;
    }
    int r;
    hipStream_t sw = st_w ? st_w : st;
    Scope ps(pc, T_WGRAD, sw);
    if (d3dp_tn_applies(N, K)) {
      if (!dy_ready) return -1;
      r = d3dp_launch_linear_f16x2_tn(ws + o_a, ws + L.x_cols + xoff(l), uns() + sdy, uns() + sx, ws + o_part, N, K, Tp, Z, sw);
    } else {
      if (!dy_ready) return -1;
      r = d3dp_launch_linear_f16x2_dyn(ws + o_at, ws + L.x_cols + xoff(l), nullptr, uns() + sdy, uns() + sx, ws + o_part, N, K,
                                       Tp, Z, sw);
    }
    if (r) return r;
    d3dp_launch_sum_partials(ws + o_part, dW, (size_t)N * K, Z, sw);
    return 0;
  }
};

}

extern "C" {

int d3dp_train_workspace_bytes(const d3dp_ctx* c, int32_t B, size_t* bytes) {
  if (!c || !bytes || B < 1) return fail(D3DP_EINVAL, "d3dp_train_workspace_bytes: bad argument");
  *bytes = train_layout(c->cfg, B).total_floats * 4;
  return D3DP_OK;
}

int d3dp_train_forward(d3dp_ctx* c, const float* x2d, const float* x3d, const int64_t* t, const float* masks, float* out,
                       int32_t B, void* workspace, size_t workspace_bytes, void* stream) {
  if (!c || !x2d || !x3d || !t || !out || !workspace || B < 1) return fail(D3DP_EINVAL, "d3dp_train_forward: bad argument");
  if (!c->train()) return fail(D3DP_ESTATE, "d3dp_train_forward needs a D3DP_MODE_TRAIN context");
  if (!c->weights_set) return fail(D3DP_ESTATE, "weights not set");
  const d3dp_cfg& g = c->cfg;
  if (g.frames > 256 && !(c->train_x2 && c->train_attn_x2 == 2 && g.channels / g.heads == 64 && g.channels % 32 == 0 && g.hidden % 32 == 0))
    return fail(D3DP_ENOTSUP, "frames=%d > 256: the training step runs such clips on its split-fp16 attention kernels only (head dim 64, "
                              "no D3DP_TRAIN_IMPL=f32 / D3DP_TRAIN_ATTN=f32|x2t cross-check)", g.frames);
  const TrainLayout L = train_layout(g, B);
  if (workspace_bytes < L.total_floats * 4) return fail(D3DP_ESTATE, "train workspace too small");
  hipStream_t st = (hipStream_t)stream;
  float* ws = (float*)workspace;
  const int T = (int)L.T, C = g.channels, F = g.frames, J = g.joints, Hd = g.hidden;
  float *xn = ws + L.xn, *y = ws + L.y, *hid = ws + L.hid;
  X2Train x2{st, ws, L, c->n_cu};
  x2.pc = c->prof ? c : nullptr;
  d3dp_ctx* const pc = x2.pc;
#define TP(cls, call) { Scope ps_(pc, cls, st); LAUNCH_TRY(call); }
  x2.use_set(0);
  x2.tail_blocks = c->train_tail_blocks;
  x2.merged_setup(T, c->train_wgrad_merged);
  const bool use_x2 = c->train_x2 && C % 32 == 0 && Hd % 32 == 0;
  if (use_x2) {
    Scope ps_(pc, T_OTHER, st);
    LAUNCH_TRY(x2.begin(true));
    LAUNCH_TRY(x2.prepare_weights(c));
  }
  auto lin = [&](int l, const float* A, const float* W, const float* bias, float* out, int M, int N, int K, bool a_amax_ready = false,
                 unsigned* out_amax = nullptr, int amax_pos = 0, bool a_prepared = false, const float* ln_w = nullptr,
                 const float* ln_b = nullptr, float ln_eps = 0.f) {
    if (use_x2) return x2.forward(l, A, W, bias, out, M, N, K, a_amax_ready, out_amax, amax_pos, a_prepared, ln_w, ln_b, ln_eps);
    Scope ps_(pc, T_LINEAR, st);
    return lin32(A, W, bias, out, M, N, K, st);
  };
  const bool ln_fused = use_x2 && x2.ln_operand_applies(3 * C, C) && x2.ln_operand_applies(Hd, C);
  const bool ln_direct = ln_fused && c->train_ln_direct && C % 256 == 0;
  const bool attn_x2 = use_x2 && c->train_attn_x2 > 0 && C / g.heads == 64 && F <= 1024;
  const bool attn_x2_s = attn_x2 && c->train_attn_x2 > 1;
  TP(T_OTHER, d3dp_train_time_mlp(t, c->freq, c->t1w, c->t1b, c->t3w, c->t3b, ws + L.dtemb, ws + L.temb, B, C, st));
  float* slab0 = ws + L.saved0;
  TP(T_LN_FWD, d3dp_launch_embed_ln(0, x2d, x3d, ws + L.temb, c->ew, c->eb, c->spos, c->ste[0].n1w, c->ste[0].n1b,
                                    g.eps_block, slab0 + L.o_xin, xn, 0, B, 1, F, J, C, st));
  auto slot = [&](int l) -> unsigned* { return use_x2 ? x2.amax() + 2 * l : nullptr; };
  if (use_x2) { Scope ps_(pc, T_OTHER, st); d3dp_launch_absmax(xn, (size_t)T * C, slot(0), st); }
  for (int blk = 0; blk < 2 * g.depth; ++blk) {
    const int kind = blk & 1, d = blk >> 1;
    const BlockDev& w = kind ? c->tte[d] : c->ste[d];
    float* S = ws + L.saved0 + (size_t)blk * L.saved_stride;
    const bool ax2 = kind == 1 ? attn_x2 : attn_x2_s;
    unsigned* qkv_amax = ax2 ? x2.amax() + X2Train::kQkvSlot0 + blk : nullptr;
    if (ln_direct && blk > 0) LAUNCH_TRY(lin(4 * blk, nullptr, (const float*)w.qkv_w, w.qkv_b, S + L.o_qkv, T, 3 * C, C, true, qkv_amax, 0, true));
    else if (ln_fused) LAUNCH_TRY(lin(4 * blk, S + L.o_xin, (const float*)w.qkv_w, w.qkv_b, S + L.o_qkv, T, 3 * C, C, true, qkv_amax, 0, false,
                                      w.n1w, w.n1b, g.eps_block));
    else LAUNCH_TRY(lin(4 * blk, xn, (const float*)w.qkv_w, w.qkv_b, S + L.o_qkv, T, 3 * C, C, true, qkv_amax));
    bool att_ready = true;
    const bool att_direct = ax2 && ln_direct && d3dp_tn_applies(C, C);
    void* att_op = att_direct ? ws + L.x_cols + x2.xoff(4 * blk + 1) : nullptr;
    const int att_tp = att_direct ? x2.pad_rows(T, C, C) : 0;
    float* att_un = att_direct ? x2.uns() + 2 * (4 * blk + 1) : nullptr;
    auto attention = [&]() -> int {
      if (kind == 0 && ax2)
        return d3dp_train_attn_x2_fwd(S + L.o_qkv, S + L.o_att, ws + L.stats_x2 + (size_t)blk * L.stats_x2_stride, B * F,
                                      spatial_map(F, J), C, g.heads, qkv_amax, slot(4 * blk + 1), st, att_op, T, att_tp, att_un);
      if (kind == 0) return d3dp_launch_attn_rows(0, S + L.o_qkv, S + L.o_att, B * F, spatial_map(F, J), C, g.heads, st, slot(4 * blk + 1));
      if (ax2)
        return d3dp_train_attn_x2_fwd(S + L.o_qkv, S + L.o_att, ws + L.stats_x2 + (size_t)blk * L.stats_x2_stride, B * J,
                                      temporal_map(F, J), C, g.heads, qkv_amax, slot(4 * blk + 1), st, att_op, T, att_tp, att_un);
      if (use_x2 && C / g.heads == 64 && F <= 256) {
        att_ready = false;
        return d3dp_launch_attn_temporal_f32(0, S + L.o_qkv, S + L.o_att, B * J, temporal_map(F, J), C, g.heads, st);
      }
      return d3dp_launch_attn_rows(0, S + L.o_qkv, S + L.o_att, B * J, temporal_map(F, J), C, g.heads, st, slot(4 * blk + 1));
    };
    TP(kind ? T_ATTN_FWD_T : T_ATTN_FWD_S, attention());
    LAUNCH_TRY(lin(4 * blk + 1, S + L.o_att, (const float*)w.proj_w, w.proj_b, y, T, C, C, att_ready, nullptr, 0, att_direct));
    if (ln_direct)
      TP(T_LN_FWD, d3dp_train_add_mask_ln(S + L.o_xin, y, mask_ptr(masks, g, B, blk, 0), kind, F, J, w.n2w, w.n2b, g.eps_block,
                                          S + L.o_xmid, nullptr, slot(4 * blk + 2), T, C, st, ws + L.x_cols + x2.xoff(4 * blk + 2),
                                          x2.pad_rows(T, Hd, C), x2.uns() + 2 * (4 * blk + 2)))
    else
      TP(T_LN_FWD, d3dp_train_add_mask_ln(S + L.o_xin, y, mask_ptr(masks, g, B, blk, 0), kind, F, J, w.n2w, w.n2b, g.eps_block,
                                          S + L.o_xmid, ln_fused ? nullptr : xn, slot(4 * blk + 2), T, C, st));
    const float* fc1_in = ln_fused ? S + L.o_xmid : xn;
    const float *f1w = ln_fused ? w.n2w : nullptr, *f1b = ln_fused ? w.n2b : nullptr;
    if (use_x2 && x2.gelu_operand_applies(C, Hd)) {
      if (ln_direct) LAUNCH_TRY(lin(4 * blk + 2, nullptr, (const float*)w.fc1_w, w.fc1_b, S + L.o_hpre, T, Hd, C, true,
                                    x2.amax() + X2Train::kPmaxSlot0 + blk, 1, true));
      else LAUNCH_TRY(lin(4 * blk + 2, fc1_in, (const float*)w.fc1_w, w.fc1_b, S + L.o_hpre, T, Hd, C, true,
                          x2.amax() + X2Train::kPmaxSlot0 + blk, 1, false, f1w, f1b, g.eps_block));
      LAUNCH_TRY(x2.gelu_operand(4 * blk + 3, S + L.o_hpre, blk, T, C, Hd));
      LAUNCH_TRY(lin(4 * blk + 3, nullptr, (const float*)w.fc2_w, w.fc2_b, y, T, C, Hd, true, nullptr, 0, true));
    } else {
      LAUNCH_TRY(lin(4 * blk + 2, fc1_in, (const float*)w.fc1_w, w.fc1_b, S + L.o_hpre, T, Hd, C, true, nullptr, 0, ln_direct, f1w, f1b,
                     g.eps_block));
      TP(T_OPERAND, d3dp_train_gelu_fwd(S + L.o_hpre, hid, (size_t)T * Hd, slot(4 * blk + 3), st));
      LAUNCH_TRY(lin(4 * blk + 3, hid, (const float*)w.fc2_w, w.fc2_b, y, T, C, Hd, true));
    }
    const bool last = blk == 2 * g.depth - 1;
    float* x_next = last ? ws + L.x_final : S + L.saved_stride + L.o_xin;
    const float *nw = c->hnw, *nb = c->hnb;
    if (!last) { const BlockDev& wn = kind ? c->ste[d + 1] : c->tte[d]; nw = wn.n1w; nb = wn.n1b; }
    TP(T_LN_FWD, d3dp_train_add_mask_ln2(S + L.o_xmid, y, mask_ptr(masks, g, B, blk, 1), kind, F, J, kind ? c->tnw : c->snw,
                                         kind ? c->tnb : c->snb, g.eps_block, (kind == 0 && d == 0) ? c->tpos : nullptr, nw, nb,
                                         last ? g.eps_head : g.eps_block, S + L.o_xout, x_next,
                                         last ? ws + L.z : (ln_fused ? nullptr : xn), last ? nullptr : slot(4 * (blk + 1)), T, C, st,
                                         (ln_direct && !last) ? ws + L.x_cols + x2.xoff(4 * (blk + 1)) : nullptr,
                                         (ln_direct && !last) ? x2.pad_rows(T, 3 * C, C) : 0,
                                         (ln_direct && !last) ? x2.uns() + 2 * 4 * (blk + 1) : nullptr));
  }
  TP(T_OTHER, d3dp_train_head_linear(ws + L.z, c->hw, c->hb, out, T, C, st));
#undef TP
  HIP_TRY(hipGetLastError());
  return D3DP_OK;
}

int d3dp_train_backward(d3dp_ctx* c, const float* x2d, const float* x3d, const int64_t* t, const float* masks,
                        const float* grad_out, const d3dp_weights* grads, int32_t B, void* workspace,
                        size_t workspace_bytes, void* stream) {
  if (!c || !x2d || !x3d || !t || !grad_out || !grads || !grads->ste || !grads->tte || !workspace || B < 1)
    return fail(D3DP_EINVAL, "d3dp_train_backward: bad argument");
  if (!c->train()) return fail(D3DP_ESTATE, "d3dp_train_backward needs a D3DP_MODE_TRAIN context");
  const d3dp_cfg& g = c->cfg;
  const TrainLayout L = train_layout(g, B);
  if (workspace_bytes < L.total_floats * 4) return fail(D3DP_ESTATE, "train workspace too small");
  hipStream_t st = (hipStream_t)stream;
  float* ws = (float*)workspace;
  const int T = (int)L.T, Tp = (int)L.Tpad, C = g.channels, F = g.frames, J = g.joints, Hd = g.hidden;
  auto G = [](const float* p) { return const_cast<float*>(p); };
  D3dpZeroTable ztab{};
  auto zero = [&](const float* p, size_t n) -> hipError_t {
    if (ztab.count < D3DP_ZERO_MAX && n < ((size_t)1 << 32)) {
      ztab.p[ztab.count] = G(p); ztab.n[ztab.count] = (unsigned)n; ++ztab.count;
      return hipSuccess;
    }
    return hipMemsetAsync(G(p), 0, n * 4, st);
  };
  const size_t CC = (size_t)C * C;
  HIP_TRY(zero(grads->time1_w, 2 * CC)); HIP_TRY(zero(grads->time1_b, 2 * C));
  HIP_TRY(zero(grads->time3_w, 2 * CC)); HIP_TRY(zero(grads->time3_b, C));
  HIP_TRY(zero(ws + L.zero_bias, 4 * (size_t)C));
  d3dp_ctx* const pc = c->prof ? c : nullptr;
#define TP(cls, call) { Scope ps_(pc, cls, st); LAUNCH_TRY(call); }
  if (ztab.count) TP(T_OTHER, d3dp_train_zero_many(ztab, st));
  const float* zb = ws + L.zero_bias;
  float *xn = ws + L.xn, *hid = ws + L.hid, *dA = ws + L.dA, *dB = ws + L.dB, *dC = ws + L.dC, *dqkv = ws + L.dqkv,
        *dh = ws + L.dh, *At = ws + L.At, *Xt = ws + L.Xt, *Wt = ws + L.Wt;

  X2Train x2{st, ws, L, c->n_cu};
  x2.pc = pc;
  x2.use_set(0);
  x2.tail_blocks = c->train_tail_blocks;
  x2.merged_setup(T, c->train_wgrad_merged);
  const bool use_x2 = c->train_x2 && C % 32 == 0 && Hd % 32 == 0;
  if (use_x2) {
    TP(T_OTHER, x2.begin(false));
    x2.batched = 8 * g.depth <= D3DP_WPREP_MAX;
  }
  const bool overlap = use_x2 && c->train_overlap && !c->prof;
  if (overlap && !c->aux) return fail(D3DP_ESTATE, "d3dp_train_backward: the second stream was not created (d3dp_create makes it)");
  bool pending[2] = {false, false};
  int n_wgrad = 0, cur_set = 0;
  const int n_sets = c->train_overlap_sets;
  auto wait_set = [&](int s) -> int {
    if (!pending[s]) return 0;
    pending[s] = false;
    return hipStreamWaitEvent(st, c->ev_done[s], 0) == hipSuccess ? 0 : -3;
  };
  auto join = [&]() -> int { int r = wait_set(0); return r ? r : wait_set(1); };
  const bool attn_x2 = use_x2 && c->train_attn_x2 > 0 && C / g.heads == 64 && F <= 1024;
  const bool attn_x2_s = attn_x2 && c->train_attn_x2 > 1;
  Reducer red{ws + L.red, L.red_floats, 0, st};
  red.items.reserve(24 * (size_t)g.depth + 32);
  const int lnrows = d3dp_train_ln_bwd_blocks(T);
  auto ln_part = [&](const float* dgamma, const float* dbeta, int calls) -> float* {
    float* p = red.take((size_t)calls * lnrows * 2 * C);
    if (p) {
      red.add(p, G(dgamma), C, (size_t)calls * lnrows, 2 * (size_t)C);
      red.add(p + C, G(dbeta), C, (size_t)calls * lnrows, 2 * (size_t)C);
    }
    return p;
  };
  float* part_sn = ln_part(grads->spatial_norm_w, grads->spatial_norm_b, g.depth);
  float* part_tn = ln_part(grads->temporal_norm_w, grads->temporal_norm_b, g.depth);
  float* part_hn = ln_part(grads->head_norm_w, grads->head_norm_b, 1);
  if (red.rc) return fail(D3DP_ESTATE, "d3dp_train_backward: partial-sum region too small");
  int sdy = -1;
  auto wgrad = [&](int l, const float* dY, int N, const float* X, int K, float* dW, float* dbias, int pre_slot = -1,
                   const float* mk = nullptr, int mk_axis = 0, const float* gelu_pre = nullptr) -> int {
    int r;
    if (use_x2) {
      sdy = pre_slot >= 0 ? pre_slot : x2.slot_for(dY, (size_t)T * N);
      if (sdy < 0) return -1;
      float* bp = red.take((size_t)X2Train::kBiasRows * N);
      int brows = 0;
      if (!bp) return -1;
      if (x2.merged) {
        if ((l & 3) == 3) {
          cur_set = overlap ? (n_wgrad++ % n_sets) : 0;
          if ((r = wait_set(cur_set))) return r;
          x2.use_set(cur_set);
        }
        if ((r = x2.prep_dy(dY, sdy, bp, &brows, T, N, K, mk, mk_axis, F, J, gelu_pre))) return r;
        red.add(bp, dbias, N, brows, N);
        if ((r = x2.wgrad(l, dY, sdy, X, dW, T, N, K))) return r;
        if ((l & 3) != 0) return 0;
        if (overlap) {
          if (hipEventRecord(c->ev_fork, st) != hipSuccess || hipStreamWaitEvent(c->aux, c->ev_fork, 0) != hipSuccess) return -3;
          x2.st_w = c->aux;
        }
        if ((r = x2.flush_wgrads())) return r;
        if (overlap) {
          if (hipEventRecord(c->ev_done[cur_set], c->aux) != hipSuccess) return -3;
          pending[cur_set] = true;
        }
        return 0;
      }
      const int set = overlap ? (n_wgrad++ % n_sets) : 0;
      if ((r = wait_set(set))) return r;
      x2.use_set(set);
      if ((r = x2.prep_dy(dY, sdy, bp, &brows, T, N, K, mk, mk_axis, F, J, gelu_pre))) return r;
      red.add(bp, dbias, N, brows, N);
      if (!overlap) return x2.wgrad(l, dY, sdy, X, dW, T, N, K);
      if (hipEventRecord(c->ev_fork, st) != hipSuccess || hipStreamWaitEvent(c->aux, c->ev_fork, 0) != hipSuccess) return -3;
      x2.st_w = c->aux;
      if ((r = x2.wgrad(l, dY, sdy, X, dW, T, N, K))) return r;
      if (hipEventRecord(c->ev_done[set], c->aux) != hipSuccess) return -3;
      pending[set] = true;
      return 0;
    }
    float* bp = red.take((size_t)D3DP_DYPREP_ROWS * N);
    int rows = 0;
    if (!bp || mk || gelu_pre) return -1;
    {
      Scope ps_(pc, T_OPERAND, st);
      if ((r = d3dp_train_colsum(dY, bp, &rows, D3DP_DYPREP_ROWS, T, N, st))) return r;
      red.add(bp, dbias, N, rows, N);
      if ((r = d3dp_train_transpose_pad(dY, At, T, N, Tp, st))) return r;
      if ((r = d3dp_train_transpose_pad(X, Xt, T, K, Tp, st))) return r;
    }
    Scope ps_(pc, T_WGRAD, st);
    return d3dp_launch_linear_f32_splitk(At, Xt, dW, N, K, Tp, st, ws + L.part, L.part_floats);
  };
  auto dgrad = [&](int l, const float* dY, int N, const float* W, int K, float* dX, unsigned* out_amax = nullptr) -> int {
    if (use_x2) return sdy < 0 ? -1 : x2.dgrad(l, dY, sdy, W, dX, T, N, K, out_amax);
    int r;
    { Scope ps_(pc, T_OPERAND, st); if ((r = d3dp_train_transpose_pad(W, Wt, N, K, N, st))) return r; }
    Scope ps_(pc, T_LINEAR, st);
    return lin32(dY, Wt, zb, dX, T, K, N, st);
  };
  auto fresh = [&](int& slot) -> unsigned* {
    slot = use_x2 ? x2.take() : -1;
    return slot >= 0 ? x2.amax() + slot : nullptr;
  };
#define D3DP_FRESH(ps, pa)                                                                              \
  int ps = -1;                                                                                          \
  unsigned* pa = fresh(ps);                                                                             \
  if (use_x2 && ps < 0) return fail(D3DP_ESTATE, "d3dp_train_backward: out of operand slots");

  const int nblk = 2 * g.depth;
  {
    float* hp = red.take((size_t)512 * (3 * C + 4));
    int rows = 0;
    if (!hp) return fail(D3DP_ESTATE, "d3dp_train_backward: partial-sum region too small");
    TP(T_OTHER, d3dp_train_head_bwd(grad_out, ws + L.z, c->hw, dC, hp, &rows, T, C, st));
    red.add(hp, G(grads->head_w), 3 * (size_t)C, rows, 3 * (size_t)C + 4);
    red.add(hp + 3 * C, G(grads->head_b), 3, rows, 3 * (size_t)C + 4);
  }
  const float* dy = nullptr;
  const float* dy_mask = nullptr;
  int ps_next = -1;
  const bool mip2 = use_x2 && x2.mask_in_prep_applies(C, Hd), mip1 = use_x2 && x2.mask_in_prep_applies(C, C);
  {
    const int lb = nblk - 1, lk = lb & 1;
    const float* S = ws + L.saved0 + (size_t)lb * L.saved_stride;
    const float* mk = mask_ptr(masks, g, B, lb, 1);
    D3DP_FRESH(ps, pa)
    TP(T_LN_BWD, d3dp_train_ln_bwd(dC, ws + L.x_final, c->hnw, g.eps_head, nullptr, nullptr, S + L.o_xout, lk ? c->tnw : c->snw,
                                 g.eps_block, dB, mk, lk, F, J, (mk && !mip2) ? dC : nullptr, pa, part_hn,
                                 (lk ? part_tn : part_sn) + (size_t)(lb >> 1) * lnrows * 2 * C, T, C, st));
    dy = (mk && !mip2) ? dC : dB;
    dy_mask = mip2 ? mk : nullptr;
    ps_next = ps;
  }
  for (int blk = nblk - 1; blk >= 0; --blk) {
    const int kind = blk & 1, d = blk >> 1;
    const BlockDev& w = kind ? c->tte[d] : c->ste[d];
    const d3dp_block_weights& gw = (kind ? grads->tte : grads->ste)[d];
    float* S = ws + L.saved0 + (size_t)blk * L.saved_stride;
    if (!use_x2) TP(T_OPERAND, d3dp_train_gelu_fwd(S + L.o_hpre, hid, (size_t)T * Hd, nullptr, st));
    LAUNCH_TRY(wgrad(4 * blk + 3, dy, C, hid, Hd, G(gw.fc2_w), G(gw.fc2_b), ps_next, dy_mask, kind));
    {
      const bool gip = use_x2 && c->train_gelu_in_prep && x2.gelu_in_prep_applies(Hd, C);
      D3DP_FRESH(ps, pa)
      LAUNCH_TRY(dgrad(4 * blk + 3, dy, C, (const float*)w.fc2_w, Hd, dh, gip ? pa : nullptr));
      if (!gip) TP(T_OPERAND, d3dp_train_gelu_bwd(dh, S + L.o_hpre, dh, (size_t)T * Hd, pa, st));
      if (!use_x2) TP(T_LN_FWD, d3dp_train_ln_pos(S + L.o_xmid, w.n2w, w.n2b, g.eps_block, nullptr, F, J, xn, T, C, st));
      LAUNCH_TRY(wgrad(4 * blk + 2, dh, Hd, xn, C, G(gw.fc1_w), G(gw.fc1_b), ps, nullptr, 0, gip ? S + L.o_hpre : nullptr));
      LAUNCH_TRY(dgrad(4 * blk + 2, dh, Hd, (const float*)w.fc1_w, C, dC));
    }
    {
      const float* mk = mask_ptr(masks, g, B, blk, 0);
      float* pn = ln_part(gw.norm2_w, gw.norm2_b, 1);
      D3DP_FRESH(ps, pa)
      if (!pn) return fail(D3DP_ESTATE, "d3dp_train_backward: partial-sum region too small");
      TP(T_LN_BWD, d3dp_train_ln_bwd(dC, S + L.o_xmid, w.n2w, g.eps_block, dB, nullptr, nullptr, nullptr, 0.f, dA, mk, kind, F, J,
                                   (mk && !mip1) ? dC : nullptr, pa, pn, nullptr, T, C, st));
      dy = (mk && !mip1) ? dC : dA;
      LAUNCH_TRY(wgrad(4 * blk + 1, dy, C, S + L.o_att, C, G(gw.proj_w), G(gw.proj_b), ps, mip1 ? mk : nullptr, kind));
    }
    int ps_dqkv = -1;
    if (kind == 1 ? attn_x2 : attn_x2_s) {
      D3DP_FRESH(pdo, pado)
      D3DP_FRESH(pq, paq)
      LAUNCH_TRY(dgrad(4 * blk + 1, dy, C, (const float*)w.proj_w, C, dB, pado));
      for (int part = pc ? 1 : 0; part <= (pc ? 2 : 0); ++part)
        TP(part == 2 ? (kind ? T_ATTN_BKV_T : T_ATTN_BKV_S) : (kind ? T_ATTN_BQ_T : T_ATTN_BQ_S),
           d3dp_train_attn_x2_bwd(S + L.o_qkv, S + L.o_att, dB, dqkv, ws + L.stats_x2 + (size_t)blk * L.stats_x2_stride,
                                  kind ? B * J : B * F, kind ? temporal_map(F, J) : spatial_map(F, J), C, g.heads,
                                  x2.amax() + X2Train::kQkvSlot0 + blk, pado, paq, st, part));
      ps_dqkv = pq;
    } else {
      LAUNCH_TRY(dgrad(4 * blk + 1, dy, C, (const float*)w.proj_w, C, dB));
      if (kind == 0) TP(T_ATTN_BQ_S, d3dp_train_attn_bwd(S + L.o_qkv, S + L.o_att, dB, dqkv, ws + L.stats, B * F, spatial_map(F, J), C, g.heads, st))
      else TP(T_ATTN_BQ_T, d3dp_train_attn_bwd(S + L.o_qkv, S + L.o_att, dB, dqkv, ws + L.stats, B * J, temporal_map(F, J), C, g.heads, st));
    }
    if (!use_x2) TP(T_LN_FWD, d3dp_train_ln_pos(S + L.o_xin, w.n1w, w.n1b, g.eps_block, nullptr, F, J, xn, T, C, st));
    LAUNCH_TRY(wgrad(4 * blk, dqkv, 3 * C, xn, C, G(gw.qkv_w), G(gw.qkv_b), ps_dqkv));
    LAUNCH_TRY(dgrad(4 * blk, dqkv, 3 * C, (const float*)w.qkv_w, C, dC));
    float* pn1 = ln_part(gw.norm1_w, gw.norm1_b, 1);
    if (!pn1) return fail(D3DP_ESTATE, "d3dp_train_backward: partial-sum region too small");
    if (blk > 0) {
      const int pb = blk - 1, pk = pb & 1;
      const float* Sp = ws + L.saved0 + (size_t)pb * L.saved_stride;
      const float* mk = mask_ptr(masks, g, B, pb, 1);
      float* g_out = pb == 0 ? ws + L.y : nullptr;
      D3DP_FRESH(ps, pa)
      TP(T_LN_BWD, d3dp_train_ln_bwd(dC, S + L.o_xin, w.n1w, g.eps_block, dA, g_out, Sp + L.o_xout, pk ? c->tnw : c->snw, g.eps_block,
                                   dB, mk, pk, F, J, (mk && !mip2) ? dC : nullptr, pa, pn1,
                                   (pk ? part_tn : part_sn) + (size_t)(pb >> 1) * lnrows * 2 * C, T, C, st));
      if (g_out) TP(T_OTHER, d3dp_train_groupsum(g_out, G(grads->temporal_pos), T, C, 1, F, J, 1, st));
      dy = (mk && !mip2) ? dC : dB;
      dy_mask = mip2 ? mk : nullptr;
      ps_next = ps;
    } else {
      TP(T_LN_BWD, d3dp_train_ln_bwd(dC, S + L.o_xin, w.n1w, g.eps_block, dA, nullptr, nullptr, nullptr, 0.f, dB, nullptr, 0, F, J,
                                   nullptr, nullptr, pn1, nullptr, T, C, st));
    }
  }
#undef D3DP_FRESH
  LAUNCH_TRY(join());
  {
    Scope ps_(pc, T_OTHER, st);
    float* ep = red.take((size_t)D3DP_EMBED_BWD_ROWS * 5 * C);
    float* bp = red.take((size_t)512 * C);
    float* sp = red.take((size_t)kGroupSlices * J * C);
    float* tp = red.take((size_t)kGroupSlices * B * C);
    int rows = 0;
    if (!ep || !bp || !sp || !tp) return fail(D3DP_ESTATE, "d3dp_train_backward: partial-sum region too small");
    LAUNCH_TRY(d3dp_train_embed_bwd(dB, x2d, x3d, ep, T, C, st));
    red.add(ep, G(grads->embed_w), 5 * (size_t)C, D3DP_EMBED_BWD_ROWS, 5 * (size_t)C);
    LAUNCH_TRY(d3dp_train_colsum(dB, bp, &rows, 512, T, C, st));
    red.add(bp, G(grads->embed_b), C, rows, C);
    LAUNCH_TRY(d3dp_train_groupsum(dB, sp, T, C, 0, F, J, kGroupSlices, st));
    red.add(sp, G(grads->spatial_pos), (size_t)J * C, kGroupSlices, (size_t)J * C);
    LAUNCH_TRY(d3dp_train_groupsum(dB, tp, T, C, 2, F, J, kGroupSlices, st));
    red.add(tp, ws + L.dtemb, (size_t)B * C, kGroupSlices, (size_t)B * C);
    red.flush();
  }
  if (red.rc) return fail(D3DP_EHIP, "d3dp_train_backward: the gradient reduction failed");
  TP(T_OTHER, d3dp_train_time_mlp_bwd(t, c->freq, c->t1w, c->t1b, c->t3w, ws + L.dtemb, G(grads->time1_w),
                                      G(grads->time1_b), G(grads->time3_w), G(grads->time3_b), B, C, st));
#undef TP
  for (int i = 0; pc && i < 8; ++i) { Scope ps_(pc, P_EMPTY, st); }
  HIP_TRY(hipGetLastError());
  return D3DP_OK;
}

}
```

d3dp_amd/csrc/gemm_x2.hip:

```cpp
#include <cstdlib>
#include <cstring>
#include <type_traits>

#include "common.h"
#include "gemm_x2_tile.h"
#include "kernels.h"

#ifndef D3DP_X2_VARIANTS
#define D3DP_X2_VARIANTS 0
#endif

#define OUT_STORE(ptr, val) __builtin_nontemporal_store((val), (ptr))

namespace {

__device__ __forceinline__ void store_planes_paired(char* dst, f16x4 ph, f16x4 pl, bool odd, bool live) {
  const uint2 h = __builtin_bit_cast(uint2, ph), l = __builtin_bit_cast(uint2, pl);
  const uint2 send = odd ? h : l;
  uint2 recv;
  recv.x = __builtin_amdgcn_update_dpp(0, (int)send.x, 0xB1, 0xF, 0xF, false);
  recv.y = __builtin_amdgcn_update_dpp(0, (int)send.y, 0xB1, 0xF, 0xF, false);
  using u32x4 = unsigned __attribute__((ext_vector_type(4)));
  const u32x4 out = odd ? (u32x4){recv.x, recv.y, l.x, l.y} : (u32x4){h.x, h.y, recv.x, recv.y};
  if (live) OUT_STORE(reinterpret_cast<u32x4*>(dst), out);
}

template <int EPI, int TAG>
__global__ __launch_bounds__(768) void gemm_f16x2_kernel(const f16* __restrict__ A2, const f16* __restrict__ W2,
                                                         const float* __restrict__ bias, float unscale, float oscale,
                                                         float* __restrict__ outf, f16* __restrict__ out2,
                                                         float* __restrict__ aux, unsigned* __restrict__ flag, int M,
                                                         int N, int K, int tiles_n_arg, int total_tiles) {
  extern __shared__ __attribute__((aligned(16))) char smem[];
  float* sbias = reinterpret_cast<float*>(smem + XNSTAGE * XSTAGE);
  const int G = gridDim.x;
  const int L = xcd_remap(blockIdx.x, G);
  const int n_my = (total_tiles - L + G - 1) / G;
  const int NK = K / XBK;
  const int gtot = n_my * NK;
  const int tid = threadIdx.x, lane = tid & 63;
  const int wave = __builtin_amdgcn_readfirstlane(tid >> 6);
  const int tiles_n = tiles_n_arg < 0 ? -tiles_n_arg : tiles_n_arg;
  const int t_flip = tiles_n_arg < 0 ? total_tiles - 1 : 0, t_sign = tiles_n_arg < 0 ? -1 : 1;
  auto tile_of = [&](int ti_) { return t_flip + t_sign * (L + ti_ * G); };

  for (int i = tid; i < (EPI == EPI_GELU_LN ? 2 * N : N); i += (XNCW + 4) * 64) sbias[i] = bias[i];
  __syncthreads();

  if (wave >= XNCW) {
    const int lw = wave - XNCW;
    const int lr = lane >> 3, lq = lane & 7;
    int ti = 0, ks = 0, slot = 0;
    const f16* pa[8];
    const f16* pw[4];
    auto issue = [&]() {
      if (ks == 0) {
        const int t = tile_of(ti);
        const int m0 = (t / tiles_n) * XBM, n0 = (t % tiles_n) * XBN;
#pragma unroll
        for (int i = 0; i < 8; ++i) {
          const int row = (lw * 8 + i) * 8 + lr;
          pa[i] = A2 + (size_t)min(m0 + row, M - 1) * (2 * K) + swz128(row, lq) * 8;
        }
#pragma unroll
        for (int i = 0; i < 4; ++i) {
          const int row = (lw * 4 + i) * 8 + lr;
          const int wrow = (row & 64) + colperm(row & 63);
          pw[i] = W2 + (size_t)min(n0 + wrow, N - 1) * (2 * K) + swz128(row, lq) * 8;
        }
      }
      if constexpr (EPI == EPI_GELU_LN) {
        if (ks == 0 && lw == 0) {
          const int t = tile_of(ti);
          const float* rs = aux + (size_t)(t / tiles_n) * XBM * 2 + lane * 4;
          char* dst = smem + XROWSTAT + (ti & 1) * (XBM * 8);
          __builtin_amdgcn_global_load_lds(GPTR(rs), LPTR(dst), 16, 0, 0);
          __builtin_amdgcn_global_load_lds(GPTR(rs + 256), LPTR(dst + 1024), 16, 0, 0);
        }
      }
      char* base = smem + slot * XSTAGE;
      const int ko = ks * (2 * XBK);
#pragma unroll
      for (int i = 0; i < 8; ++i)
        __builtin_amdgcn_global_load_lds(GPTR(pa[i] + ko), LPTR(base + (lw * 8 + i) * 1024), 16, 0, 0);
#pragma unroll
      for (int i = 0; i < 4; ++i)
        __builtin_amdgcn_global_load_lds(GPTR(pw[i] + ko), LPTR(base + XA_BYTES + (lw * 4 + i) * 1024), 16, 0, 0);
      if (++ks == NK) { ks = 0; ++ti; }
      slot = (slot == XNSTAGE - 1) ? 0 : slot + 1;
    };
    if (gtot > 0) issue();
    if (gtot > 1) issue();
    for (int g = 0; g < gtot; ++g) {
      if (g + 1 < gtot) asm volatile("s_waitcnt vmcnt(12)" ::: "memory");
      else asm volatile("s_waitcnt vmcnt(0)" ::: "memory");
      X2_BARRIER();
      if (g + 2 < gtot) issue();
    }
    return;
  }

  const int wr = wave >> 1, wc = wave & 1;
  const int fi = lane & 15, fg = lane >> 4;
  const int offA = (wr * 64 + fi) * 128 + swz128(fi, fg) * 16, offAl = offA ^ 64;
  const int offW = XA_BYTES + (wc * 64 + fi) * 128 + swz128(fi, fg) * 16, offWl = offW ^ 64;
  f32x4 acc[4][4];
  __builtin_amdgcn_s_setprio(1);
  int slot = 0;
  for (int ti = 0; ti < n_my; ++ti) {
#pragma unroll
    for (int i = 0; i < 4; ++i)
#pragma unroll
      for (int j = 0; j < 4; ++j) acc[i][j] = (f32x4){0.f, 0.f, 0.f, 0.f};
    f16x8 wfa[4][2], wfb[4][2], taa[2], tab[2];
#pragma unroll
    for (int ni = 0; ni < 4; ++ni) wfb[ni][0] = wfb[ni][1] = (f16x8){};
    tab[0] = tab[1] = (f16x8){};
    auto kstep = [&](f16x8 (&wf)[4][2], f16x8 (&ta)[2], const f16x8 (&pw)[4][2], const f16x8 (&pa)[2]) {
      __builtin_amdgcn_s_waitcnt(0xc07f);
      X2_BARRIER();
      __builtin_amdgcn_sched_barrier(0);
      const char* sb = smem + slot * XSTAGE;
      slot = (slot == XNSTAGE - 1) ? 0 : slot + 1;
      f16x8 ah[2], al[2];
#pragma unroll
      for (int ni = 0; ni < 4; ++ni)
#pragma unroll
        for (int pl = 0; pl < 2; ++pl)
          wf[ni][pl] = *reinterpret_cast<const f16x8*>(sb + (pl ? offWl : offW) + ni * 2048);
      ah[0] = *reinterpret_cast<const f16x8*>(sb + offA);
      al[0] = *reinterpret_cast<const f16x8*>(sb + offAl);
      __builtin_amdgcn_sched_barrier(0);
#pragma unroll
      for (int ni = 0; ni < 4; ++ni) acc[3][ni] = __builtin_amdgcn_mfma_f32_16x16x32_f16(pa[1], pw[ni][0], acc[3][ni], 0, 0, 0);
#pragma unroll
      for (int ni = 0; ni < 4; ++ni) acc[3][ni] = __builtin_amdgcn_mfma_f32_16x16x32_f16(pa[0], pw[ni][0], acc[3][ni], 0, 0, 0);
      __builtin_amdgcn_sched_barrier(0);
#pragma unroll
      for (int mi = 0; mi < 3; ++mi) {
        const int b = mi & 1;
        if (mi < 2) {
          ah[b ^ 1] = *reinterpret_cast<const f16x8*>(sb + offA + (mi + 1) * 2048);
          al[b ^ 1] = *reinterpret_cast<const f16x8*>(sb + offAl + (mi + 1) * 2048);
        } else {
          ta[0] = *reinterpret_cast<const f16x8*>(sb + offA + 3 * 2048);
          ta[1] = *reinterpret_cast<const f16x8*>(sb + offAl + 3 * 2048);
        }
#pragma unroll
        for (int ni = 0; ni < 4; ++ni) acc[mi][ni] = __builtin_amdgcn_mfma_f32_16x16x32_f16(ah[b], wf[ni][1], acc[mi][ni], 0, 0, 0);
#pragma unroll
        for (int ni = 0; ni < 4; ++ni) acc[mi][ni] = __builtin_amdgcn_mfma_f32_16x16x32_f16(al[b], wf[ni][0], acc[mi][ni], 0, 0, 0);
#pragma unroll
        for (int ni = 0; ni < 4; ++ni) acc[mi][ni] = __builtin_amdgcn_mfma_f32_16x16x32_f16(ah[b], wf[ni][0], acc[mi][ni], 0, 0, 0);
        __builtin_amdgcn_sched_barrier(0);
      }
#pragma unroll
      for (int ni = 0; ni < 4; ++ni) acc[3][ni] = __builtin_amdgcn_mfma_f32_16x16x32_f16(ta[0], wf[ni][1], acc[3][ni], 0, 0, 0);
    };
#pragma unroll 1
    for (int ks = 0; ks < NK; ks += 2) {
      kstep(wfa, taa, wfb, tab);
      kstep(wfb, tab, wfa, taa);
    }
#pragma unroll
    for (int ni = 0; ni < 4; ++ni) acc[3][ni] = __builtin_amdgcn_mfma_f32_16x16x32_f16(tab[1], wfb[ni][0], acc[3][ni], 0, 0, 0);
#pragma unroll
    for (int ni = 0; ni < 4; ++ni) acc[3][ni] = __builtin_amdgcn_mfma_f32_16x16x32_f16(tab[0], wfb[ni][0], acc[3][ni], 0, 0, 0);
    const int t = tile_of(ti);
    const int pm0 = (t / tiles_n) * XBM + wr * 64 + 4 * fg, nb = (t % tiles_n) * XBN + wc * 64 + 4 * fi;
    if (nb < N) {
      const float4 bz = *reinterpret_cast<const float4*>(sbias + nb);
      const bool odd = fi & 1;
      unsigned off, pitch;
      bool planes;
      char* base = reinterpret_cast<char*>(outf);
      const int c0 = nb & ~7;
      const unsigned offp = (unsigned)pm0 * (N * 4) + (c0 >> 5) * 128 + (c0 & 31) * 2 + (odd ? 64 : 0);
      if constexpr (EPI == EPI_GELU || EPI == EPI_GELU_LN) {
        base = reinterpret_cast<char*>(out2);
        pitch = N * 4; planes = true;
        off = offp - (unsigned)pm0 * pitch;
      } else if constexpr (TAG == 1) {
        const int C = N / 3, region = nb / C, cn = nb - region * C;
        pitch = N * 4; planes = region != 0;
        off = planes ? region * 4 * C + cn * 2 + (odd ? 2 * C - 8 : 0) : cn * 4;
      } else {
        pitch = N * 4; planes = false;
        off = nb * 4;
      }
      off += (unsigned)pm0 * pitch;
      const int rows = M - pm0;
      [[maybe_unused]] float4 c1z = {};
      [[maybe_unused]] const float* srow = nullptr;
      if constexpr (EPI == EPI_GELU_LN) {
        c1z = *reinterpret_cast<const float4*>(sbias + N + nb);
        srow = reinterpret_cast<const float*>(smem + XROWSTAT + (ti & 1) * (XBM * 8)) + (wr * 64 + 4 * fg) * 2;
      }
      auto value = [&](int mi, int r, int e) {
        const float bze = e == 0 ? bz.x : e == 1 ? bz.y : e == 2 ? bz.z : bz.w;
        if constexpr (EPI == EPI_GELU_LN) {
          const float2 st = *reinterpret_cast<const float2*>(srow + (mi * 16 + r) * 2);
          const float c1e = e == 0 ? c1z.x : e == 1 ? c1z.y : e == 2 ? c1z.z : c1z.w;
          return fmaf(st.y, fmaf(acc[mi][e][r], unscale, -(st.x * c1e)), bze);
        } else {
          return fmaf(acc[mi][e][r], unscale, bze);
        }
      };
      auto store_rows = [&](auto planes_c, auto checked_c) {
#pragma unroll
        for (int mi = 0; mi < 4; ++mi)
#pragma unroll
          for (int r = 0; r < 4; ++r) {
            const int k = mi * 16 + r;
            const bool live = !decltype(checked_c)::value || k < rows;
            char* dst = base + (off + (unsigned)k * pitch);
            if constexpr (decltype(planes_c)::value) {
              f16x4 ph, pl;
              float v[4] = {value(mi, r, 0), value(mi, r, 1), value(mi, r, 2), value(mi, r, 3)};
              if constexpr (EPI == EPI_GELU || EPI == EPI_GELU_LN) {
                const f32x2 g0 = gelu_erf_rational2((f32x2){v[0], v[1]}), g1 = gelu_erf_rational2((f32x2){v[2], v[3]});
                v[0] = g0.x; v[1] = g0.y; v[2] = g1.x; v[3] = g1.y;
              }
#pragma unroll
              for (int e = 0; e < 4; ++e) {
                f16 h, l;
                split2h_scaled(v[e] * oscale, h, l);
                ph[e] = h; pl[e] = l;
              }
              store_planes_paired(dst, ph, pl, odd, live);
            } else if constexpr (EPI != EPI_RESID && EPI != EPI_RESID_LN) {
              if (live) OUT_STORE(reinterpret_cast<f32x4*>(dst), ((f32x4){value(mi, r, 0), value(mi, r, 1), value(mi, r, 2), value(mi, r, 3)}));
            }
          }
        if constexpr (EPI == EPI_RESID && !decltype(planes_c)::value) {
          f32x4 res[4][4];
#pragma unroll
          for (int mi = 0; mi < 4; ++mi)
#pragma unroll
            for (int r = 0; r < 4; ++r) {
              const int k = mi * 16 + r;
              const bool live = !decltype(checked_c)::value || k < rows;
              res[mi][r] = (f32x4){0.f, 0.f, 0.f, 0.f};
              if (live) res[mi][r] = *reinterpret_cast<const f32x4*>(base + (off + (unsigned)k * pitch));
            }
#pragma unroll
          for (int mi = 0; mi < 4; ++mi)
#pragma unroll
            for (int r = 0; r < 4; ++r) {
              const int k = mi * 16 + r;
              const bool live = !decltype(checked_c)::value || k < rows;
              const f32x4 v = {res[mi][r][0] + value(mi, r, 0), res[mi][r][1] + value(mi, r, 1),
                               res[mi][r][2] + value(mi, r, 2), res[mi][r][3] + value(mi, r, 3)};
              if (live) *reinterpret_cast<f32x4*>(base + (off + (unsigned)k * pitch)) = v;
            }
        }
        if constexpr (EPI == EPI_RESID_LN && !decltype(planes_c)::value) {
          auto rowsum16 = [](float x) {
            x += __builtin_bit_cast(float, __builtin_amdgcn_update_dpp(0, __builtin_bit_cast(int, x), 0xB1, 0xF, 0xF, false));
            x += __builtin_bit_cast(float, __builtin_amdgcn_update_dpp(0, __builtin_bit_cast(int, x), 0x4E, 0xF, 0xF, false));
            x += __builtin_bit_cast(float, __builtin_amdgcn_update_dpp(0, __builtin_bit_cast(int, x), 0x141, 0xF, 0xF, false));
            x += __builtin_bit_cast(float, __builtin_amdgcn_update_dpp(0, __builtin_bit_cast(int, x), 0x140, 0xF, 0xF, false));
            return x;
          };
          const int S = (N + 63) >> 6, slice = nb >> 6;
          float* sdst = aux + ((size_t)pm0 * S + slice) * 2;
          bool over = false;
#pragma unroll
          for (int half = 0; half < 2; ++half) {
            f32x4 res[2][4];
#pragma unroll
            for (int m2 = 0; m2 < 2; ++m2)
#pragma unroll
              for (int r = 0; r < 4; ++r) {
                const int k = (half * 2 + m2) * 16 + r;
                const bool live = !decltype(checked_c)::value || k < rows;
                res[m2][r] = (f32x4){0.f, 0.f, 0.f, 0.f};
                if (live) res[m2][r] = *reinterpret_cast<const f32x4*>(base + (off + (unsigned)k * pitch));
              }
#pragma unroll
            for (int m2 = 0; m2 < 2; ++m2)
#pragma unroll
              for (int r = 0; r < 4; ++r) {
                const int mi = half * 2 + m2, k = mi * 16 + r;
                const bool live = !decltype(checked_c)::value || k < rows;
                const f32x4 v = {res[m2][r][0] + value(mi, r, 0), res[m2][r][1] + value(mi, r, 1),
                                 res[m2][r][2] + value(mi, r, 2), res[m2][r][3] + value(mi, r, 3)};
                if (live) *reinterpret_cast<f32x4*>(base + (off + (unsigned)k * pitch)) = v;
                f16x4 ph, pl;
#pragma unroll
                for (int e = 0; e < 4; ++e) { f16 h, l; split2h_scaled(v[e] * oscale, h, l); ph[e] = h; pl[e] = l; }
                store_planes_paired(reinterpret_cast<char*>(out2) + (offp + (unsigned)k * (N * 4)), ph, pl, odd, live);
                over |= !(fmaxf(fmaxf(fabsf(v[0]), fabsf(v[1])), fmaxf(fabsf(v[2]), fabsf(v[3]))) * oscale < 65504.0f);
                const float mean = rowsum16((v[0] + v[1]) + (v[2] + v[3])) * (1.0f / 64.0f);
                const float d0 = v[0] - mean, d1 = v[1] - mean, d2 = v[2] - mean, d3 = v[3] - mean;
                const float q2 = rowsum16(fmaf(d0, d0, d1 * d1) + fmaf(d2, d2, d3 * d3));
                if (live && fi == 0) *reinterpret_cast<float2*>(sdst + (size_t)k * S * 2) = make_float2(mean, q2);
              }
          }
          if (__builtin_expect(__any(over), 0) && lane == 0) atomicOr(flag, 2u);
        }
      };
      using T_ = std::true_type; using F_ = std::false_type;
      constexpr bool kPlanesOnly = EPI == EPI_GELU || EPI == EPI_GELU_LN;
      if (rows >= 64) {
        if (planes) { if constexpr (kPlanesOnly || TAG == 1) store_rows(T_{}, F_{}); }
        else { if constexpr (!kPlanesOnly) store_rows(F_{}, F_{}); }
      } else {
        if (planes) { if constexpr (kPlanesOnly || TAG == 1) store_rows(T_{}, T_{}); }
        else { if constexpr (!kPlanesOnly) store_rows(F_{}, T_{}); }
      }
    }
  }
}

__global__ void split2h_kernel(const float* __restrict__ s, f16* __restrict__ d, size_t n, float scale) {
  size_t i = (size_t)blockIdx.x * blockDim.x + threadIdx.x;
  const size_t stride = (size_t)gridDim.x * blockDim.x;
  for (; i < n; i += stride) {
    f16 a, b;
    split2h_scaled(s[i] * scale, a, b);
    const size_t o = (i >> 5) * 64 + (i & 31);
    d[o] = a; d[o + 32] = b;
  }
}

__global__ __launch_bounds__(256) void absmax_kernel(const float* __restrict__ s, size_t n, unsigned* __restrict__ out) {
  __shared__ float part[4];
  const size_t stride = (size_t)gridDim.x * blockDim.x;
  float m = 0.f;
  const size_t n4 = n / 4;
  const float4* s4 = reinterpret_cast<const float4*>(s);
  auto amax4 = [](const float4 v) { return fmaxf(fmaxf(fabsf(v.x), fabsf(v.y)), fmaxf(fabsf(v.z), fabsf(v.w))); };
  size_t i = (size_t)blockIdx.x * blockDim.x + threadIdx.x;
  for (; i + 3 * stride < n4; i += 4 * stride) {
    const float4 v0 = s4[i], v1 = s4[i + stride], v2 = s4[i + 2 * stride], v3 = s4[i + 3 * stride];
    m = fmaxf(m, fmaxf(fmaxf(amax4(v0), amax4(v1)), fmaxf(amax4(v2), amax4(v3))));
  }
  for (; i < n4; i += stride) m = fmaxf(m, amax4(s4[i]));
  for (size_t j = n4 * 4 + (size_t)blockIdx.x * blockDim.x + threadIdx.x; j < n; j += stride) m = fmaxf(m, fabsf(s[j]));
  m = wave_max(m);
  if ((threadIdx.x & 63) == 0) part[threadIdx.x >> 6] = m;
  __syncthreads();
  if (threadIdx.x == 0) atomicMax(out, __float_as_uint(fmaxf(fmaxf(part[0], part[1]), fmaxf(part[2], part[3]))));
}

__global__ void rowbound_kernel(const float* __restrict__ W, const float* __restrict__ gamma, const float* __restrict__ beta,
                                const float* __restrict__ bias, int N, int K, float sq, unsigned* __restrict__ out) {
  const int lane = threadIdx.x & 63;
  const int n = blockIdx.x * (blockDim.x >> 6) + (threadIdx.x >> 6);
  if (n >= N) return;
  float a = 0.f, inmax = 0.f;
  for (int k = lane; k < K; k += 64) {
    const float in = fmaf(sq, fabsf(gamma[k]), fabsf(beta[k]));
    inmax = fmaxf(inmax, in);
    a = fmaf(fabsf(W[(size_t)n * K + k]), in, a);
  }
  a = wave_sum(a);
  inmax = wave_max(inmax);
  if (lane == 0) {
    atomicMax(out, __float_as_uint((a + fabsf(bias[n])) * 1.001f));
    atomicMax(out + 1, __float_as_uint(inmax * 1.001f));
  }
}

__global__ void nonfinite_flag_kernel(const float* __restrict__ x, size_t n, unsigned* __restrict__ flag) {
  size_t i = (size_t)blockIdx.x * blockDim.x + threadIdx.x;
  const size_t stride = (size_t)gridDim.x * blockDim.x;
  bool bad = false;
  for (; i < n; i += stride) bad |= !(fabsf(x[i]) <= 3.0e38f);
  if (__any(bad) && (threadIdx.x & 63) == 0) atomicOr(flag, 1u);
}

}

bool d3dp_x2_variants_built() { return D3DP_X2_VARIANTS != 0; }

#if D3DP_X2_VARIANTS
#include "gemm_x2_variants.h"
#else
bool d3dp_x2_skew_applies(int, int, int, int, int, int) { return false; }
void d3dp_launch_ln_combine(const float*, float*, int, int, float, hipStream_t) {}
void d3dp_launch_fold_ln(const float*, const float*, const float*, const float*, float*, float*, int, int, hipStream_t) {}
#endif

int d3dp_launch_linear_f16x2(int epi, const void* A2, const void* W2, const float* bias, float unscale, float oscale,
                             float* outf, void* out2, float* aux, unsigned* flag, int M, int N, int K, hipStream_t st,
                             int skew_d, int pingpong) {
  const bool reverse = (pingpong & X2_TILES_LAST_TO_FIRST) != 0;
  pingpong &= 0xff;
  if (K % (2 * XBK) != 0 || N % 4 != 0 || N > XBIAS_MAX || M <= 0) return -1;
  if ((size_t)M * N * 4 >= ((size_t)1 << 32)) return -1;
  if (epi != EPI_BIAS && epi != EPI_GELU && epi != EPI_QKV_PACK && epi != EPI_RESID && epi != EPI_RESID_LN &&
      epi != EPI_GELU_LN) return -1;
  if ((epi == EPI_RESID_LN || epi == EPI_GELU_LN) && (!aux || !out2)) return -1;
  if (epi == EPI_RESID_LN && !flag) return -1;
  if (epi == EPI_RESID_LN && N % 64 != 0) return -1;
  if (epi == EPI_GELU_LN && 2 * N > XBIAS_MAX) return -1;
  if (epi == EPI_QKV_PACK && (N % 3 != 0 || (N / 3) % 64 != 0)) return -1;
  if ((epi == EPI_GELU || epi == EPI_GELU_LN || epi == EPI_RESID_LN) && N % 32 != 0) return -1;
  if (epi == EPI_GELU_LN && K / XBK < XNSTAGE) return -1;
  const int tm = (M + XBM - 1) / XBM, tn = (N + XBN - 1) / XBN;
  using KernT = void (*)(const f16*, const f16*, const float*, float, float, float*, f16*, float*, unsigned*, int, int, int, int, int);
#if D3DP_X2_VARIANTS
  constexpr int NKERN = 6;
  static const KernT kerns[NKERN] = {gemm_f16x2_kernel<EPI_BIAS, 0>, gemm_f16x2_kernel<EPI_BIAS, 1>,
                                     gemm_f16x2_kernel<EPI_GELU, 0>, gemm_f16x2_kernel<EPI_RESID, 0>,
                                     gemm_f16x2_kernel<EPI_RESID_LN, 0>, gemm_f16x2_kernel<EPI_GELU_LN, 0>};
#else
  if (epi == EPI_RESID_LN || epi == EPI_GELU_LN || skew_d != 0 || pingpong != 0) return -2;
  constexpr int NKERN = 4;
  static const KernT kerns[NKERN] = {gemm_f16x2_kernel<EPI_BIAS, 0>, gemm_f16x2_kernel<EPI_BIAS, 1>,
                                     gemm_f16x2_kernel<EPI_GELU, 0>, gemm_f16x2_kernel<EPI_RESID, 0>};
#endif
  static PerDeviceOnce once;
  const int cus = once.get([&](int dev) {
    for (int k = 0; k < NKERN; ++k)
      if (d3dp_lds_opt_in(reinterpret_cast<const void*>(kerns[k]), XLDS) < 0) return -3;
    return d3dp_cu_count(dev);
  });
  if (cus < 0) return -3;
  const int total = tm * tn, grid = total < cus ? total : cus;
#if D3DP_X2_VARIANTS
  const int taken = x2_variants_launch(epi, A2, W2, bias, unscale, oscale, outf, out2, aux, flag, M, N, K, st, skew_d, pingpong, cus);
  if (taken <= 0) return taken;
#endif
  const KernT kern = kerns[epi == EPI_GELU ? 2 : epi == EPI_RESID ? 3 : epi == EPI_QKV_PACK ? 1 : epi == EPI_RESID_LN ? 4
                           : epi == EPI_GELU_LN ? 5 : 0];
  hipLaunchKernelGGL(kern, dim3(grid), dim3((XNCW + 4) * 64), XLDS, st, (const f16*)A2, (const f16*)W2, bias, unscale, oscale, outf,
                     (f16*)out2, aux, flag, M, N, K, reverse ? -tn : tn, total);
  return 0;
}

void d3dp_launch_split2(const float* src, void* dst, size_t n, float scale, hipStream_t st) {
  const unsigned blocks = (unsigned)((n + 255) / 256 < 4096 ? (n + 255) / 256 : 4096);
  hipLaunchKernelGGL(split2h_kernel, dim3(blocks ? blocks : 1), dim3(256), 0, st, src, (f16*)dst, n, scale);
}

void d3dp_launch_rowbound(const float* W, const float* gamma, const float* beta, const float* bias, int N, int K,
                          unsigned* out, hipStream_t st) {
  hipLaunchKernelGGL(rowbound_kernel, dim3((N + 3) / 4), dim3(256), 0, st, W, gamma, beta, bias, N, K,
                     sqrtf((float)(K - 1)) * 1.0001f, out);
}

void d3dp_launch_absmax(const float* src, size_t n, unsigned* out, hipStream_t st) {
  const unsigned blocks = (unsigned)((n / 4 + 255) / 256 < 512 ? (n / 4 + 255) / 256 : 512);
  hipLaunchKernelGGL(absmax_kernel, dim3(blocks ? blocks : 1), dim3(256), 0, st, src, n, out);
}

void d3dp_launch_nonfinite_flag(const float* x, size_t n, unsigned* flag, hipStream_t st) {
  const unsigned blocks = (unsigned)((n + 255) / 256 < 1024 ? (n + 255) / 256 : 1024);
  hipLaunchKernelGGL(nonfinite_flag_kernel, dim3(blocks ? blocks : 1), dim3(256), 0, st, x, n, flag);
}
```

d3dp_amd/csrc/kernels.h:

```cpp
#pragma once
#include <hip/hip_runtime.h>
#include <stdint.h>

#include <mutex>

struct PerDeviceOnce {
  static constexpr int kMaxDev = 64;
  std::mutex mu;
  int val[kMaxDev] = {0};
  template <class F> int get(F&& fn) {
    int dev = 0;
    if (hipGetDevice(&dev) != hipSuccess || dev < 0 || dev >= kMaxDev) return -3;
    std::lock_guard<std::mutex> lock(mu);
    if (val[dev] <= 0) {
      const int v = fn(dev);
      if (v <= 0) return v < 0 ? v : -3;
      val[dev] = v;
    }
    return val[dev];
  }
};
inline int d3dp_cu_count(int dev) {
  hipDeviceProp_t prop;
  if (hipGetDeviceProperties(&prop, dev) != hipSuccess || prop.multiProcessorCount < 1) return -3;
  return prop.multiProcessorCount;
}
inline int d3dp_lds_opt_in(const void* kern, int bytes) {
  return hipFuncSetAttribute(kern, hipFuncAttributeMaxDynamicSharedMemorySize, bytes) == hipSuccess ? 1 : -3;
}

enum { EPI_BIAS = 0, EPI_GELU = 1, EPI_RESID = 2, EPI_PARTIAL = 3, EPI_QKV_PACK = 4, EPI_RESID_LN = 5, EPI_GELU_LN = 6 };

int d3dp_launch_linear_bf16_stream(int epi, int out_f32, const void* A, const void* W, const float* bias, void* out,
                                   int M, int N, int K, hipStream_t st, int f16 = 0);
int d3dp_launch_linear_bf16x3(int epi, const void* A3, const void* W3, const float* bias, float* outf, void* out3, int M,
                              int N, int K, hipStream_t st);
void d3dp_launch_split3(const float* src, void* dst, size_t n, hipStream_t st);
int d3dp_launch_linear_f16x2(int epi, const void* A2, const void* W2, const float* bias, float unscale, float oscale,
                             float* outf, void* out2, float* aux, unsigned* flag, int M, int N, int K, hipStream_t st,
                             int skew_d = 0, int pingpong = 0);
constexpr int X2_TILES_LAST_TO_FIRST = 0x100;
bool d3dp_x2_skew_applies(int epi, int M, int N, int K, int skew_d, int n_cu);
bool d3dp_x2_variants_built();
void d3dp_launch_rowbound(const float* W, const float* gamma, const float* beta, const float* bias, int N, int K,
                          unsigned* out, hipStream_t st);
void d3dp_launch_ln_combine(const float* slices, float* rowstat, int M, int C, float eps, hipStream_t st);
void d3dp_launch_fold_ln(const float* W, const float* gamma, const float* beta, const float* bias, float* Wp, float* c12,
                         int N, int K, hipStream_t st);
void d3dp_launch_split2(const float* src, void* dst, size_t n, float scale, hipStream_t st);
void d3dp_launch_absmax(const float* src, size_t n, unsigned* out, hipStream_t st);
void d3dp_launch_nonfinite_flag(const float* x, size_t n, unsigned* flag, hipStream_t st);
int d3dp_launch_linear_f16x2_dyn(const void* A2, const void* W2, const float* bias, const float* dynA, const float* dynW,
                                 float* out, int M, int N, int Kfull, int Z, hipStream_t st, unsigned* amax_out = nullptr,
                                 int amax_pos = 0, int rem_blocks = 0);
int d3dp_launch_gelu_rowprep(const float* src, void* drow, int R, int Rpad, int C, const unsigned* pmax, unsigned* amax_out,
                             float* unscale, hipStream_t st);
void d3dp_launch_split2_dyn(const float* src, void* dst, int R, int C, int Cpad, const unsigned* amax, float* unscale,
                            hipStream_t st);
void d3dp_launch_split2_t_dyn(const float* src, void* dst, int R, int C, int Rpad, const unsigned* amax, float* unscale,
                              hipStream_t st);
constexpr int D3DP_DYPREP_ROWS = 96;
int d3dp_launch_dyprep(const float* src, void* drow, void* dcol, float* colpart, int R, int C, int Rpad, const unsigned* amax,
                       float* unscale, hipStream_t st);
constexpr int D3DP_ROWPREP_ROWS = 512;
int d3dp_launch_rowprep(const float* src, void* drow, float* colpart, int* rows, int R, int Rpad, int C, const unsigned* amax,
                        float* unscale, hipStream_t st, const float* mask = nullptr, int axis = 0, int F = 1, int J = 1,
                        const float* gelu_pre = nullptr);
int d3dp_launch_rowprep_ln(const float* src, const float* w, const float* b, float eps, void* drow, int R, int Rpad, int C,
                           const unsigned* amax, float* unscale, hipStream_t st);
bool d3dp_tn_applies(int N, int K);
int d3dp_launch_linear_f16x2_tn(const void* A2, const void* W2, const float* dynA, const float* dynW, float* out, int N, int K,
                                int Tp, int Z, hipStream_t st);
constexpr int D3DP_TN_MAX = 4;
struct D3dpTnProduct {
  const void* A2; const void* W2;
  const float* dynA; const float* dynW;
  float* out;
  int N, K;
  int tiles_k, tile0;
};
struct D3dpTnTable { D3dpTnProduct p[D3DP_TN_MAX]; int n; };
int d3dp_launch_linear_f16x2_tn_many(const D3dpTnProduct* prods, int n, int Tp, int Z, hipStream_t st);
struct D3dpSumTable { const float* part[D3DP_TN_MAX]; float* out[D3DP_TN_MAX]; size_t n4[D3DP_TN_MAX]; int Z; int n; };
void d3dp_launch_sum_partials_many(const D3dpSumTable& tb, hipStream_t st);
constexpr int D3DP_WPREP_MAX = 64;
struct D3dpWPrepItem { const float* w; int N, K, slot, pad; size_t off; };
struct D3dpWPrepTable { D3dpWPrepItem it[D3DP_WPREP_MAX]; int n; };
int d3dp_launch_wprep(const D3dpWPrepTable& tb, void* rows_base, void* cols_base, unsigned* amax, float* unscale, hipStream_t st);
void d3dp_launch_sum_partials(const float* part, float* out, size_t n, int Z, hipStream_t st);
void d3dp_launch_sum_partials_bias(const float* part, const float* bias, float* out, size_t n, int N, int Z, hipStream_t st,
                                   unsigned* amax = nullptr, int amax_pos = 0);
int d3dp_launch_linear_f32_splitk(const float* A, const float* W, float* out, int M, int N, int K, hipStream_t st, float* part,
                                  size_t part_floats);
int d3dp_launch_linear_f32(int epi, const float* A, const float* W, const float* bias, float* out, int M, int N,
                           int K, hipStream_t st);

struct SeqMap { int n_tok, inner, outer_stride, inner_stride, tok_stride; };
int d3dp_launch_attn_rows(int act_bf16, const void* qkv, void* out, int n_seq, SeqMap map, int C, int heads,
                          hipStream_t st, unsigned* amax = nullptr);
int d3dp_launch_attn_temporal_bf16(const void* qkv, void* out, int n_seq, SeqMap map, int C, int heads,
                                   hipStream_t st, int f16 = 0);
int d3dp_launch_attn_temporal_f32(int act, const void* qkv, void* out, int n_seq, SeqMap map, int C, int heads,
                                  hipStream_t st);
int d3dp_launch_attn_x2(int act, int axis, const void* qkv, void* out, int n_seq, SeqMap map, int C, int heads,
                        float act_scale, hipStream_t st);
void d3dp_launch_qkv_pack_x2(const float* src, void* dst, size_t T, int C, float act_scale, hipStream_t st);
int d3dp_launch_attn_spatial_bf16(const void* qkv, void* out, int n_seq, SeqMap map, int C, int heads, hipStream_t st,
                                  int f16 = 0);

int d3dp_launch_time_mlp(const int64_t* t, const float* freq, const float* w1, const float* b1, const float* w2,
                         const float* b2, float* temb, int B, int C, hipStream_t st);
int d3dp_launch_embed_ln(int act_bf16, const float* x2d, const float* x3d, const float* temb, const float* ew,
                         const float* eb, const float* spos, const float* lnw, const float* lnb, float eps, float* x,
                         void* xn, int seq0, int n_seq, int H, int F, int J, int C, hipStream_t st, int SP = 0);
int d3dp_launch_ln(int act_bf16, float* x, const void* yadd, int write_x, const float* w, const float* b, float eps,
                   void* xn, int T, int C, hipStream_t st);
int d3dp_launch_ln2(int act_bf16, float* x, const void* yadd0, const void* yadd, const float* wa, const float* ba, const float* pos,
                    const float* wb, const float* bb, float eps, void* xn, int T, int C, int F, int J, hipStream_t st,
                    int SP = 0);
int d3dp_launch_head(int act_bf16, const float* x, const void* yadd0, const void* yadd, const float* wa, const float* ba, float eps_a, const float* wh,
                     const float* bh, float eps_h, const float* w, const float* b, float* out, int T, int C,
                     hipStream_t st, int FJ = 0, int SP = 0);

int d3dp_launch_ddim_pre(const float* img, float* xt2, const int* perm, float scale, int B, int per_b, int J,
                         hipStream_t st);
int d3dp_launch_ddim_post(const float* pred2, const float* img, const float* noise, const int* perm, float scale,
                          double sqrt_recip, double sqrt_recipm1, float c_xstart, float c_noise, float sigma,
                          int last, float* x_start, size_t xs_bstride, float* img_next, int B, int per_b, int J,
                          hipStream_t st);
int d3dp_launch_q_sample(const float* x0, const float* noise, const double* a, const double* b, float scale,
                         float* out, int B, int per_b, hipStream_t st);

int d3dp_launch_jpma(const float* pred, const float* traj, const float* cam, const float* gt2d, const float* gt3d,
                     float* agg, int* sel, float* err_sel, float* err_min, float* win, float* jbest, float* mean,
                     int h_offset, int B, int K, int H, int F, int J, int root_joint, int linear, hipStream_t st,
                     int h_inner = 0, size_t outer_stride = 0);

int d3dp_set_error(int code, const char* msg);
int d3dp_check_launch(const char* what);
extern "C" int d3dp_clip_count(int32_t n, int32_t F);

int d3dp_train_add_mask_ln(const float* x_in, const float* y, const float* mask, int axis, int F, int J, const float* w,
                           const float* b, float eps, float* x_out, float* xn, unsigned* amax, int T, int C, hipStream_t st,
                           void* op = nullptr, int Tp = 0, float* op_unscale = nullptr);
int d3dp_train_add_mask_ln2(const float* x_in, const float* y, const float* mask, int axis, int F, int J, const float* wa,
                            const float* ba, float eps_a, const float* pos, const float* wb, const float* bb, float eps_b,
                            float* x_out, float* x_next, float* xn, unsigned* amax, int T, int C, hipStream_t st, void* op = nullptr,
                            int Tp = 0, float* op_unscale = nullptr);
int d3dp_train_ln_pos(const float* x, const float* w, const float* b, float eps, const float* pos, int F, int J, float* y,
                      int T, int C, hipStream_t st);
constexpr int D3DP_LN_BWD_BLOCKS = 512;
int d3dp_train_ln_bwd_blocks(int T);
int d3dp_train_ln_bwd(const float* dy, const float* xb, const float* wb, float eps_b, const float* dres, float* g_out,
                      const float* xa, const float* wa, float eps_a, float* dx, const float* mask, int axis, int F, int J,
                      float* dxm, unsigned* amax, float* part_b, float* part_a, int T, int C, hipStream_t st);
constexpr int D3DP_REDUCE_MAX = 80;
struct D3dpReduceItem { const float* part; float* dst; unsigned n, count, stride, accumulate; };
struct D3dpReduceTable { D3dpReduceItem it[D3DP_REDUCE_MAX]; int count; };
int d3dp_train_reduce_many(const D3dpReduceTable& tb, hipStream_t st);
int d3dp_train_gelu_fwd(const float* x, float* y, size_t n, unsigned* amax, hipStream_t st);
int d3dp_train_gelu_bwd(const float* dh, const float* x, float* dpre, size_t n, unsigned* amax, hipStream_t st);
int d3dp_train_colsum(const float* in, float* part, int* rows, int max_rows, int T, int C, hipStream_t st);
constexpr int D3DP_ZERO_MAX = 192;
struct D3dpZeroTable { float* p[D3DP_ZERO_MAX]; unsigned n[D3DP_ZERO_MAX]; int count; };
int d3dp_train_zero_many(const D3dpZeroTable& tb, hipStream_t st);
int d3dp_train_groupsum(const float* in, float* out, int T, int C, int mode, int F, int J, int slices, hipStream_t st);
int d3dp_train_transpose_pad(const float* in, float* out, int R, int C, int Rpad, hipStream_t st);
size_t d3dp_train_attn_stats_bytes(int n_seq, int n_tok, int heads);
int d3dp_train_attn_bwd(const float* qkv, const float* o, const float* dout, float* dqkv, void* stats, int n_seq,
                        SeqMap map, int C, int heads, hipStream_t st);
constexpr int D3DP_EMBED_BWD_ROWS = 64;
size_t d3dp_train_attn_x2_stats_bytes(int n_seq, int n_tok, int heads);
int d3dp_train_attn_x2_fwd(const float* qkv, float* out, void* stats, int n_seq, SeqMap map, int C, int heads,
                           const unsigned* amax_qkv, unsigned* amax_out, hipStream_t st, void* op = nullptr, int T = 0, int Tp = 0,
                           float* op_unscale = nullptr);
int d3dp_train_attn_x2_bwd(const float* qkv, const float* o, const float* dout, float* dqkv, void* stats, int n_seq, SeqMap map,
                           int C, int heads, const unsigned* amax_qkv, const unsigned* amax_do, unsigned* amax_out,
                           hipStream_t st, int part = 0);
int d3dp_train_embed_bwd(const float* dx, const float* x2d, const float* x3d, float* part, int T, int C, hipStream_t st);
int d3dp_train_head_linear(const float* z, const float* w, const float* b, float* out, int T, int C, hipStream_t st);
int d3dp_train_head_bwd(const float* g, const float* z, const float* w, float* dz, float* part, int* rows, int T, int C,
                        hipStream_t st);
int d3dp_train_time_mlp(const int64_t* t, const float* freq, const float* w1, const float* b1, const float* w2, const float* b2,
                        float* hidden, float* temb, int B, int C, hipStream_t st);
int d3dp_train_time_mlp_bwd(const int64_t* t, const float* freq, const float* w1, const float* b1, const float* w2,
                            const float* dtemb, float* dw1, float* db1, float* dw2, float* db2, int B, int C,
                            hipStream_t st);

inline bool d3dp_width_instantiated(int C) { return C == 64 || C == 128 || C == 256 || C == 512; }
int d3dp_train_g_add_mask_ln(const float* x_in, const float* y, const float* mask, int axis, int F, int J, const float* w,
                             const float* b, float eps, float* x_out, float* xn, int T, int C, hipStream_t st);
int d3dp_train_g_add_mask_ln2(const float* x_in, const float* y, const float* mask, int axis, int F, int J, const float* wa,
                              const float* ba, float eps_a, const float* pos, const float* wb, const float* bb, float eps_b,
                              float* x_out, float* x_next, float* xn, int T, int C, hipStream_t st);
int d3dp_train_g_ln_pos(const float* x, const float* w, const float* b, float eps, const float* pos, int F, int J, float* y, int T,
                        int C, hipStream_t st);
int d3dp_train_g_ln_bwd(const float* dy, const float* xb, const float* wb, float eps_b, const float* dres, float* g_out,
                        const float* xa, const float* wa, float eps_a, float* dx, const float* mask, int axis, int F, int J,
                        float* dxm, float* part_b, float* part_a, int T, int C, int blocks, hipStream_t st);
int d3dp_train_g_head_linear(const float* z, const float* w, const float* b, float* out, int T, int C, hipStream_t st);
int d3dp_train_g_time_mlp_bwd(const int64_t* t, const float* freq, const float* w1, const float* b1, const float* w2,
                              const float* dtemb, float* dw1, float* db1, float* dw2, float* db2, int B, int C, hipStream_t st);
```

d3dp_amd/csrc/pointwise.hip:

```cpp
#include <type_traits>

#include "common.h"
#include "kernels.h"

namespace {

#ifndef NT_STREAMS
#define NT_STREAMS 1
#endif
#ifndef NT_Y
#define NT_Y 1
#endif

template <int C> struct Row {
  static constexpr int NV = C / 64;
  static constexpr bool V4 = (NV % 4 == 0);
  static __device__ __forceinline__ int elem(int lane, int i) {
    if constexpr (V4) return ((i >> 2) * 64 + lane) * 4 + (i & 3);
    else return i * 64 + lane;
  }
  static __device__ __forceinline__ void load(const float* p, int lane, float* v) {
    if constexpr (V4) {
#pragma unroll
      for (int g = 0; g < NV / 4; ++g) {
        float4 a = *reinterpret_cast<const float4*>(p + (g * 64 + lane) * 4);
        v[g * 4] = a.x; v[g * 4 + 1] = a.y; v[g * 4 + 2] = a.z; v[g * 4 + 3] = a.w;
      }
    } else {
#pragma unroll
      for (int i = 0; i < NV; ++i) v[i] = p[i * 64 + lane];
    }
  }
  template <typename E, typename = typename std::enable_if<sizeof(E) == 2>::type>
  static __device__ __forceinline__ void load(const E* p, int lane, float* v) {
    if constexpr (V4) {
#pragma unroll
      for (int g = 0; g < NV / 4; ++g) {
        typename Op2<E>::x4 a = *reinterpret_cast<const typename Op2<E>::x4*>(p + (g * 64 + lane) * 4);
        v[g * 4] = (float)a[0]; v[g * 4 + 1] = (float)a[1]; v[g * 4 + 2] = (float)a[2]; v[g * 4 + 3] = (float)a[3];
      }
    } else {
#pragma unroll
      for (int i = 0; i < NV; ++i) v[i] = (float)p[i * 64 + lane];
    }
  }
  static __device__ __forceinline__ void load_nt(const float* p, int lane, float* v) {
    if constexpr (V4) {
#pragma unroll
      for (int g = 0; g < NV / 4; ++g) {
        const f32x4 a = __builtin_nontemporal_load(reinterpret_cast<const f32x4*>(p + (g * 64 + lane) * 4));
        v[g * 4] = a[0]; v[g * 4 + 1] = a[1]; v[g * 4 + 2] = a[2]; v[g * 4 + 3] = a[3];
      }
    } else {
      load(p, lane, v);
    }
  }
  template <typename E, typename = typename std::enable_if<sizeof(E) == 2>::type>
  static __device__ __forceinline__ void load_nt(const E* p, int lane, float* v) {
    if constexpr (V4) {
#pragma unroll
      for (int g = 0; g < NV / 4; ++g) {
        const typename Op2<E>::x4 a = __builtin_nontemporal_load(reinterpret_cast<const typename Op2<E>::x4*>(p + (g * 64 + lane) * 4));
        v[g * 4] = (float)a[0]; v[g * 4 + 1] = (float)a[1]; v[g * 4 + 2] = (float)a[2]; v[g * 4 + 3] = (float)a[3];
      }
    } else {
      load(p, lane, v);
    }
  }
  static __device__ __forceinline__ void store_nt(float* p, int lane, const float* v) {
    if constexpr (V4) {
#pragma unroll
      for (int g = 0; g < NV / 4; ++g) {
        const f32x4 a = {v[g * 4], v[g * 4 + 1], v[g * 4 + 2], v[g * 4 + 3]};
        __builtin_nontemporal_store(a, reinterpret_cast<f32x4*>(p + (g * 64 + lane) * 4));
      }
    } else {
      store(p, lane, v);
    }
  }
  static __device__ __forceinline__ void store(float* p, int lane, const float* v) {
    if constexpr (V4) {
#pragma unroll
      for (int g = 0; g < NV / 4; ++g)
        *reinterpret_cast<float4*>(p + (g * 64 + lane) * 4) = make_float4(v[g * 4], v[g * 4 + 1], v[g * 4 + 2], v[g * 4 + 3]);
    } else {
#pragma unroll
      for (int i = 0; i < NV; ++i) p[i * 64 + lane] = v[i];
    }
  }
  template <typename E, typename = typename std::enable_if<sizeof(E) == 2>::type>
  static __device__ __forceinline__ void store(E* p, int lane, const float* v) {
    if constexpr (V4) {
#pragma unroll
      for (int g = 0; g < NV / 4; ++g) {
        typename Op2<E>::x4 a = {(E)v[g * 4], (E)v[g * 4 + 1], (E)v[g * 4 + 2], (E)v[g * 4 + 3]};
        *reinterpret_cast<typename Op2<E>::x4*>(p + (g * 64 + lane) * 4) = a;
      }
    } else {
#pragma unroll
      for (int i = 0; i < NV; ++i) {
        float t = v[i];
        if constexpr (std::is_same<E, f16>::value) asm volatile("" : "+v"(t));
        p[i * 64 + lane] = (E)t;
      }
    }
  }
  static __device__ __forceinline__ void store3(bf16* p, size_t plane, int lane, const float* v) {
    float a0[NV], a1[NV], a2[NV];
#pragma unroll
    for (int i = 0; i < NV; ++i) {
      bf16 q0, q1, q2;
      split3(v[i], q0, q1, q2);
      a0[i] = (float)q0; a1[i] = (float)q1; a2[i] = (float)q2;
    }
    store(p, lane, a0);
    store(p + plane, lane, a1);
    store(p + 2 * plane, lane, a2);
  }
  static __device__ __forceinline__ void store2h(f16* p, size_t, int lane, const float* v) {
    if constexpr (V4) {
      const bool odd = lane & 1;
#pragma unroll
      for (int g = 0; g < NV / 4; ++g) {
        f16x4 a, b;
#pragma unroll
        for (int e = 0; e < 4; ++e) { f16 h, l; split2h(v[g * 4 + e], h, l); a[e] = h; b[e] = l; }
        const uint2 h = __builtin_bit_cast(uint2, a), l = __builtin_bit_cast(uint2, b);
        const uint2 send = odd ? h : l;
        uint2 recv;
        recv.x = __builtin_amdgcn_update_dpp(0, (int)send.x, 0xB1, 0xF, 0xF, false);
        recv.y = __builtin_amdgcn_update_dpp(0, (int)send.y, 0xB1, 0xF, 0xF, false);
        using u32x4 = unsigned __attribute__((ext_vector_type(4)));
        const u32x4 out = odd ? (u32x4){recv.x, recv.y, l.x, l.y} : (u32x4){h.x, h.y, recv.x, recv.y};
        const int c0 = (g * 64 + (lane & ~1)) * 4;
        *reinterpret_cast<u32x4*>(p + h2i_col(c0) + (odd ? kH2iLo : 0)) = out;
      }
    } else {
#pragma unroll
      for (int i = 0; i < NV; ++i) {
        f16 h, l;
        split2h(v[i], h, l);
        const int c = i * 64 + lane;
        p[h2i_col(c)] = h;
        p[h2i_col(c) + kH2iLo] = l;
      }
    }
  }
  static __device__ __forceinline__ void norm(const float* v, const float* w, const float* b, float eps, int lane,
                                              float* y) {
    float s = 0.f;
#pragma unroll
    for (int i = 0; i < NV; ++i) s += v[i];
    const float mean = wave_sum(s) * (1.0f / C);
    float q = 0.f;
#pragma unroll
    for (int i = 0; i < NV; ++i) { const float d = v[i] - mean; q = fmaf(d, d, q); }
    const float rstd = 1.0f / sqrtf(wave_sum(q) * (1.0f / C) + eps);
    float wv[NV], bv[NV];
    load(w, lane, wv);
    load(b, lane, bv);
#pragma unroll
    for (int i = 0; i < NV; ++i) y[i] = fmaf((v[i] - mean) * rstd, wv[i], bv[i]);
  }
  static __device__ __forceinline__ void norm_r(const float* v, const float* wv, const float* bv, float eps, float* y) {
    float s = 0.f;
#pragma unroll
    for (int i = 0; i < NV; ++i) s += v[i];
    const float mean = wave_sum(s) * (1.0f / C);
    float q = 0.f;
#pragma unroll
    for (int i = 0; i < NV; ++i) { const float d = v[i] - mean; q = fmaf(d, d, q); }
    const float rstd = 1.0f / sqrtf(wave_sum(q) * (1.0f / C) + eps);
#pragma unroll
    for (int i = 0; i < NV; ++i) y[i] = fmaf((v[i] - mean) * rstd, wv[i], bv[i]);
  }
};

template <int C, typename XN> struct ActOut {
  using ptr = XN*;
  static __device__ __forceinline__ void st(ptr base, size_t, size_t off, int lane, const float* v) {
    Row<C>::store(base + off, lane, v);
  }
};
template <int C> struct ActOut<C, b3> {
  using ptr = bf16*;
  static __device__ __forceinline__ void st(ptr base, size_t plane, size_t off, int lane, const float* v) {
    Row<C>::store3(base + off, plane, lane, v);
  }
};

template <int C> struct ActOut<C, h2> {
  using ptr = f16*;
  static __device__ __forceinline__ void st(ptr base, size_t plane, size_t off, int lane, const float* v) {
    Row<C>::store2h(base + 2 * off, plane, lane, v);
  }
};

template <int C, typename XN, typename YT>
__global__ __launch_bounds__(256) void ln_kernel(float* __restrict__ x, const YT* __restrict__ yadd,
                                                 const float* __restrict__ w, const float* __restrict__ b, float eps,
                                                 typename ActOut<C, XN>::ptr xn, size_t plane, int T, int write_x) {
  using R = Row<C>;
  const int lane = threadIdx.x & 63;
  const int tok = blockIdx.x * 4 + (threadIdx.x >> 6);
  if (tok >= T) return;
  float v[R::NV], y[R::NV];
  if (NT_STREAMS) R::load_nt(x + (size_t)tok * C, lane, v); else R::load(x + (size_t)tok * C, lane, v);
  if (yadd != nullptr) {
    if (NT_STREAMS && NT_Y) R::load_nt(yadd + (size_t)tok * C, lane, y); else R::load(yadd + (size_t)tok * C, lane, y);
#pragma unroll
    for (int i = 0; i < R::NV; ++i) v[i] += y[i];
    if (write_x) R::store(x + (size_t)tok * C, lane, v);
  }
  R::norm(v, w, b, eps, lane, y);
  ActOut<C, XN>::st(xn, plane, (size_t)tok * C, lane, y);
}

template <int C, typename XN, typename YT>
__global__ __launch_bounds__(256) void ln2_kernel(float* __restrict__ x, const YT* __restrict__ yadd0,
                                                  const YT* __restrict__ yadd, const float* __restrict__ wa,
                                                  const float* __restrict__ ba, const float* __restrict__ pos,
                                                  const float* __restrict__ wb, const float* __restrict__ bb, float eps,
                                                  typename ActOut<C, XN>::ptr xn, size_t plane, int T, int F, int J,
                                                  int SP) {
  using R = Row<C>;
  const int lane = threadIdx.x & 63;
  const int tok = blockIdx.x * 4 + (threadIdx.x >> 6);
  if (tok >= T) return;
  float v[R::NV], y[R::NV], z[R::NV];
  if (NT_STREAMS) R::load_nt(x + (size_t)tok * C, lane, v); else R::load(x + (size_t)tok * C, lane, v);
  if (yadd0 != nullptr) {
    if (NT_STREAMS && NT_Y) R::load_nt(yadd0 + (size_t)tok * C, lane, y); else R::load(yadd0 + (size_t)tok * C, lane, y);
#pragma unroll
    for (int i = 0; i < R::NV; ++i) v[i] += y[i];
  }
  if (yadd != nullptr) {
    if (NT_STREAMS && NT_Y) R::load_nt(yadd + (size_t)tok * C, lane, y); else R::load(yadd + (size_t)tok * C, lane, y);
#pragma unroll
    for (int i = 0; i < R::NV; ++i) v[i] += y[i];
  }
  R::norm(v, wa, ba, eps, lane, y);
  if (pos != nullptr) {
    const int f = min((tok % SP) / J, F - 1);
    float pv[R::NV];
    R::load(pos + (size_t)f * C, lane, pv);
#pragma unroll
    for (int i = 0; i < R::NV; ++i) y[i] += pv[i];
  }
  if (NT_STREAMS) R::store_nt(x + (size_t)tok * C, lane, y); else R::store(x + (size_t)tok * C, lane, y);
  R::norm(y, wb, bb, eps, lane, z);
  ActOut<C, XN>::st(xn, plane, (size_t)tok * C, lane, z);
}

constexpr int kRowTokens = 8;

template <int C, typename XN>
__global__ __launch_bounds__(256) void embed_ln_kernel(const float* __restrict__ x2d, const float* __restrict__ x3d,
                                                       const float* __restrict__ temb, const float* __restrict__ ew,
                                                       const float* __restrict__ eb, const float* __restrict__ spos,
                                                       const float* __restrict__ lnw, const float* __restrict__ lnb,
                                                       float eps, float* __restrict__ x,
                                                       typename ActOut<C, XN>::ptr xn, size_t plane, int seq0,
                                                       int n_seq, int H, int F, int J, int SP) {
  using R = Row<C>;
  const int lane = threadIdx.x & 63;
  const int wave = __builtin_amdgcn_readfirstlane(threadIdx.x >> 6);
  const int FJ = F * J, T = n_seq * SP;
  float w5[R::NV][5], ebv[R::NV], lw[R::NV], lb[R::NV];
#pragma unroll
  for (int i = 0; i < R::NV; ++i) {
    const float* wr = ew + R::elem(lane, i) * 5;
#pragma unroll
    for (int k = 0; k < 5; ++k) w5[i][k] = wr[k];
  }
  R::load(eb, lane, ebv);
  R::load(lnw, lane, lw);
  R::load(lnb, lane, lb);
  for (int it = 0; it < kRowTokens; ++it) {
    const int tl = (blockIdx.x * kRowTokens + it) * 4 + wave;
    if (tl >= T) break;
    const bool pad = (tl % SP) >= FJ;
    const int seq = seq0 + tl / SP, fj = pad ? 0 : tl % SP, nj = fj % J;
    const int b = seq / H;
    const float* p2 = x2d + ((size_t)b * FJ + fj) * 2;
    const float* p3 = x3d + ((size_t)seq * FJ + fj) * 3;
    float in5[5] = {p2[0], p2[1], p3[0], p3[1], p3[2]};
    if (pad) { in5[0] = in5[1] = in5[2] = in5[3] = in5[4] = 0.f; }
    float v[R::NV], y[R::NV], sp[R::NV], tb[R::NV];
    R::load(spos + (size_t)nj * C, lane, sp);
    R::load(temb + (size_t)b * C, lane, tb);
#pragma unroll
    for (int i = 0; i < R::NV; ++i) {
      float a = 0.f;
#pragma unroll
      for (int k = 0; k < 5; ++k) a = fmaf(in5[k], w5[i][k], a);
      a += ebv[i];
      a += sp[i];
      a += tb[i];
      v[i] = a;
    }
    if (NT_STREAMS) R::store_nt(x + (size_t)tl * C, lane, v); else R::store(x + (size_t)tl * C, lane, v);
    R::norm_r(v, lw, lb, eps, y);
    ActOut<C, XN>::st(xn, plane, (size_t)tl * C, lane, y);
  }
}

template <int C, typename YT>
__global__ __launch_bounds__(256) void head_kernel(const float* __restrict__ x, const YT* __restrict__ yadd0,
                                                   const YT* __restrict__ yadd, const float* __restrict__ wa,
                                                   const float* __restrict__ ba, float eps_a,
                                                   const float* __restrict__ wh, const float* __restrict__ bh,
                                                   float eps_h, const float* __restrict__ w, const float* __restrict__ b,
                                                   float* __restrict__ out, int T, int FJ, int SP) {
  using R = Row<C>;
  const int lane = threadIdx.x & 63;
  const int wave = __builtin_amdgcn_readfirstlane(threadIdx.x >> 6);
  float wav[R::NV], bav[R::NV], whv[R::NV], bhv[R::NV], wv[3][R::NV];
  R::load(wa, lane, wav);
  R::load(ba, lane, bav);
  R::load(wh, lane, whv);
  R::load(bh, lane, bhv);
#pragma unroll
  for (int o = 0; o < 3; ++o) R::load(w + o * C, lane, wv[o]);
  const float b0 = b[0], b1 = b[1], b2 = b[2];
  for (int it = 0; it < kRowTokens; ++it) {
    const int tok = (blockIdx.x * kRowTokens + it) * 4 + wave;
    if (tok >= T) break;
    float v[R::NV], y[R::NV], z[R::NV];
    if (NT_STREAMS) R::load_nt(x + (size_t)tok * C, lane, v); else R::load(x + (size_t)tok * C, lane, v);
    if (yadd0 != nullptr) {
      if (NT_STREAMS && NT_Y) R::load_nt(yadd0 + (size_t)tok * C, lane, y); else R::load(yadd0 + (size_t)tok * C, lane, y);
#pragma unroll
      for (int i = 0; i < R::NV; ++i) v[i] += y[i];
    }
    if (yadd != nullptr) {
      if (NT_STREAMS && NT_Y) R::load_nt(yadd + (size_t)tok * C, lane, y); else R::load(yadd + (size_t)tok * C, lane, y);
#pragma unroll
      for (int i = 0; i < R::NV; ++i) v[i] += y[i];
    }
    R::norm_r(v, wav, bav, eps_a, y);
    R::norm_r(y, whv, bhv, eps_h, z);
    float acc[3];
#pragma unroll
    for (int o = 0; o < 3; ++o) {
      float a = 0.f;
#pragma unroll
      for (int i = 0; i < R::NV; ++i) a = fmaf(z[i], wv[o][i], a);
      acc[o] = wave_sum(a) + (o == 0 ? b0 : o == 1 ? b1 : b2);
    }
    const int fj = tok % SP;
    if (lane < 3 && fj < FJ) out[((size_t)(tok / SP) * FJ + fj) * 3 + lane] = lane == 0 ? acc[0] : (lane == 1 ? acc[1] : acc[2]);
  }
}

__global__ __launch_bounds__(256) void time_mlp_kernel(const int64_t* __restrict__ t, const float* __restrict__ freq,
                                                       const float* __restrict__ w1, const float* __restrict__ b1,
                                                       const float* __restrict__ w2, const float* __restrict__ b2,
                                                       float* __restrict__ temb, int C) {
  extern __shared__ float sm[];
  float* e = sm;
  float* h = sm + C;
  const int b = blockIdx.x, half = C / 2;
  const float tv = (float)t[b];
  for (int i = threadIdx.x; i < half; i += blockDim.x) {
    const float a = tv * freq[i];
    e[i] = sinf(a);
    e[half + i] = cosf(a);
  }
  __syncthreads();
  for (int o = threadIdx.x; o < 2 * C; o += blockDim.x) {
    const float* wr = w1 + (size_t)o * C;
    float a = 0.f;
    for (int k = 0; k < C; ++k) a = fmaf(e[k], wr[k], a);
    h[o] = gelu_erf(a + b1[o]);
  }
  __syncthreads();
  for (int o = threadIdx.x; o < C; o += blockDim.x) {
    const float* wr = w2 + (size_t)o * 2 * C;
    float a = 0.f;
    for (int k = 0; k < 2 * C; ++k) a = fmaf(h[k], wr[k], a);
    temb[(size_t)b * C + o] = a + b2[o];
  }
}

template <int NVM> struct RowG {
  static __device__ __forceinline__ void load(const float* p, int C, int lane, float* v) {
#pragma unroll
    for (int i = 0; i < NVM; ++i) { const int c = i * 64 + lane; v[i] = c < C ? p[c] : 0.f; }
  }
  static __device__ __forceinline__ void store(float* p, int C, int lane, const float* v) {
#pragma unroll
    for (int i = 0; i < NVM; ++i) { const int c = i * 64 + lane; if (c < C) p[c] = v[i]; }
  }
  static __device__ __forceinline__ void norm(const float* v, const float* w, const float* b, float eps, int C, int lane, float* y) {
    const float rc = 1.0f / (float)C;
    float s = 0.f;
#pragma unroll
    for (int i = 0; i < NVM; ++i) s += v[i];
    const float mean = wave_sum(s) * rc;
    float q = 0.f;
#pragma unroll
    for (int i = 0; i < NVM; ++i) { const float d = (i * 64 + lane < C) ? v[i] - mean : 0.f; q = fmaf(d, d, q); }
    const float rstd = 1.0f / sqrtf(wave_sum(q) * rc + eps);
#pragma unroll
    for (int i = 0; i < NVM; ++i) {
      const int c = i * 64 + lane;
      y[i] = c < C ? fmaf((v[i] - mean) * rstd, w[c], b[c]) : 0.f;
    }
  }
};

template <int NVM>
__global__ __launch_bounds__(256) void ln_g_kernel(float* __restrict__ x, const float* __restrict__ yadd, const float* __restrict__ w,
                                                   const float* __restrict__ b, float eps, float* __restrict__ xn, int T, int C,
                                                   int write_x) {
  using R = RowG<NVM>;
  const int lane = threadIdx.x & 63;
  const int tok = blockIdx.x * 4 + (threadIdx.x >> 6);
  if (tok >= T) return;
  float v[NVM], y[NVM];
  R::load(x + (size_t)tok * C, C, lane, v);
  if (yadd != nullptr) {
    R::load(yadd + (size_t)tok * C, C, lane, y);
#pragma unroll
    for (int i = 0; i < NVM; ++i) v[i] += y[i];
    if (write_x) R::store(x + (size_t)tok * C, C, lane, v);
  }
  R::norm(v, w, b, eps, C, lane, y);
  R::store(xn + (size_t)tok * C, C, lane, y);
}

template <int NVM>
__global__ __launch_bounds__(256) void ln2_g_kernel(float* __restrict__ x, const float* __restrict__ yadd0, const float* __restrict__ yadd,
                                                    const float* __restrict__ wa, const float* __restrict__ ba,
                                                    const float* __restrict__ pos, const float* __restrict__ wb,
                                                    const float* __restrict__ bb, float eps, float* __restrict__ xn, int T, int C,
                                                    int F, int J, int SP) {
  using R = RowG<NVM>;
  const int lane = threadIdx.x & 63;
  const int tok = blockIdx.x * 4 + (threadIdx.x >> 6);
  if (tok >= T) return;
  float v[NVM], y[NVM], z[NVM];
  R::load(x + (size_t)tok * C, C, lane, v);
  if (yadd0 != nullptr) {
    R::load(yadd0 + (size_t)tok * C, C, lane, y);
#pragma unroll
    for (int i = 0; i < NVM; ++i) v[i] += y[i];
  }
  if (yadd != nullptr) {
    R::load(yadd + (size_t)tok * C, C, lane, y);
#pragma unroll
    for (int i = 0; i < NVM; ++i) v[i] += y[i];
  }
  R::norm(v, wa, ba, eps, C, lane, y);
  if (pos != nullptr) {
    const int f = min((tok % SP) / J, F - 1);
    float pv[NVM];
    R::load(pos + (size_t)f * C, C, lane, pv);
#pragma unroll
    for (int i = 0; i < NVM; ++i) y[i] += pv[i];
  }
  R::store(x + (size_t)tok * C, C, lane, y);
  R::norm(y, wb, bb, eps, C, lane, z);
  R::store(xn + (size_t)tok * C, C, lane, z);
}

template <int NVM>
__global__ __launch_bounds__(256) void embed_ln_g_kernel(const float* __restrict__ x2d, const float* __restrict__ x3d,
                                                         const float* __restrict__ temb, const float* __restrict__ ew,
                                                         const float* __restrict__ eb, const float* __restrict__ spos,
                                                         const float* __restrict__ lnw, const float* __restrict__ lnb, float eps,
                                                         float* __restrict__ x, float* __restrict__ xn, int seq0, int n_seq, int H,
                                                         int F, int J, int SP, int C) {
  using R = RowG<NVM>;
  const int lane = threadIdx.x & 63;
  const int tl = blockIdx.x * 4 + (threadIdx.x >> 6);
  const int FJ = F * J;
  if (tl >= n_seq * SP) return;
  const bool pad = (tl % SP) >= FJ;
  const int seq = seq0 + tl / SP, fj = pad ? 0 : tl % SP, nj = fj % J;
  const int b = seq / H;
  const float* p2 = x2d + ((size_t)b * FJ + fj) * 2;
  const float* p3 = x3d + ((size_t)seq * FJ + fj) * 3;
  float in5[5] = {p2[0], p2[1], p3[0], p3[1], p3[2]};
  if (pad) { in5[0] = in5[1] = in5[2] = in5[3] = in5[4] = 0.f; }
  float v[NVM], y[NVM];
#pragma unroll
  for (int i = 0; i < NVM; ++i) {
    const int c = i * 64 + lane;
    float a = 0.f;
    if (c < C) {
      const float* wr = ew + c * 5;
#pragma unroll
      for (int k = 0; k < 5; ++k) a = fmaf(in5[k], wr[k], a);
      a += eb[c];
      a += spos[nj * C + c];
      a += temb[b * C + c];
    }
    v[i] = a;
  }
  R::store(x + (size_t)tl * C, C, lane, v);
  R::norm(v, lnw, lnb, eps, C, lane, y);
  R::store(xn + (size_t)tl * C, C, lane, y);
}

template <int NVM>
__global__ __launch_bounds__(256) void head_g_kernel(const float* __restrict__ x, const float* __restrict__ yadd0,
                                                     const float* __restrict__ yadd, const float* __restrict__ wa,
                                                     const float* __restrict__ ba, float eps_a, const float* __restrict__ wh,
                                                     const float* __restrict__ bh, float eps_h, const float* __restrict__ w,
                                                     const float* __restrict__ b, float* __restrict__ out, int T, int C, int FJ,
                                                     int SP) {
  using R = RowG<NVM>;
  const int lane = threadIdx.x & 63;
  const int tok = blockIdx.x * 4 + (threadIdx.x >> 6);
  if (tok >= T) return;
  float v[NVM], y[NVM], z[NVM];
  R::load(x + (size_t)tok * C, C, lane, v);
  if (yadd0 != nullptr) {
    R::load(yadd0 + (size_t)tok * C, C, lane, y);
#pragma unroll
    for (int i = 0; i < NVM; ++i) v[i] += y[i];
  }
  if (yadd != nullptr) {
    R::load(yadd + (size_t)tok * C, C, lane, y);
#pragma unroll
    for (int i = 0; i < NVM; ++i) v[i] += y[i];
  }
  R::norm(v, wa, ba, eps_a, C, lane, y);
  R::norm(y, wh, bh, eps_h, C, lane, z);
  float acc[3];
#pragma unroll
  for (int o = 0; o < 3; ++o) {
    float wv[NVM];
    R::load(w + o * C, C, lane, wv);
    float a = 0.f;
#pragma unroll
    for (int i = 0; i < NVM; ++i) a = fmaf(z[i], wv[i], a);
    acc[o] = wave_sum(a) + b[o];
  }
  const int fj = tok % SP;
  if (lane < 3 && fj < FJ) out[((size_t)(tok / SP) * FJ + fj) * 3 + lane] = lane == 0 ? acc[0] : (lane == 1 ? acc[1] : acc[2]);
}

__host__ inline bool width_instantiated(int C) { return C == 64 || C == 128 || C == 256 || C == 512; }
#define DISPATCH_G(C, ...)                                                  \
  if ((C) < 1 || (C) > 1024) return -2;                                     \
  if ((C) <= 256) { constexpr int NVM = 4; __VA_ARGS__; }                   \
  else if ((C) <= 512) { constexpr int NVM = 8; __VA_ARGS__; }              \
  else { constexpr int NVM = 16; __VA_ARGS__; }

}

#define DISPATCH_C(C, ...)                          \
  switch (C) {                                      \
    case 512: { constexpr int CC = 512; __VA_ARGS__; break; } \
    case 256: { constexpr int CC = 256; __VA_ARGS__; break; } \
    case 128: { constexpr int CC = 128; __VA_ARGS__; break; } \
    case 64:  { constexpr int CC = 64;  __VA_ARGS__; break; } \
    default: return -2;                             \
  }

int d3dp_launch_time_mlp(const int64_t* t, const float* freq, const float* w1, const float* b1, const float* w2,
                         const float* b2, float* temb, int B, int C, hipStream_t st) {
  hipLaunchKernelGGL(time_mlp_kernel, dim3(B), dim3(256), (size_t)3 * C * sizeof(float), st, t, freq, w1, b1, w2, b2,
                     temb, C);
  return 0;
}

int d3dp_launch_embed_ln(int act_bf16, const float* x2d, const float* x3d, const float* temb, const float* ew,
                         const float* eb, const float* spos, const float* lnw, const float* lnb, float eps, float* x,
                         void* xn, int seq0, int n_seq, int H, int F, int J, int C, hipStream_t st, int SP) {
  if (SP <= 0) SP = F * J;
  if (SP < F * J) return -1;
  const int T = n_seq * SP;
  dim3 g((T + 3) / 4), blk(256);
  const size_t plane = (size_t)T * C;
  if (!width_instantiated(C)) {
    if (act_bf16 != 0) return -2;
    DISPATCH_G(C, hipLaunchKernelGGL((embed_ln_g_kernel<NVM>), g, blk, 0, st, x2d, x3d, temb, ew, eb, spos, lnw, lnb, eps, x, (float*)xn, seq0, n_seq, H, F, J, SP, C))
    return 0;
  }
  const dim3 gk((T + 4 * kRowTokens - 1) / (4 * kRowTokens));
  DISPATCH_C(C,
    if (act_bf16 == 1) hipLaunchKernelGGL((embed_ln_kernel<CC, bf16>), gk, blk, 0, st, x2d, x3d, temb, ew, eb, spos, lnw, lnb, eps, x, (bf16*)xn, plane, seq0, n_seq, H, F, J, SP);
    else if (act_bf16 == 4) hipLaunchKernelGGL((embed_ln_kernel<CC, f16>), gk, blk, 0, st, x2d, x3d, temb, ew, eb, spos, lnw, lnb, eps, x, (f16*)xn, plane, seq0, n_seq, H, F, J, SP);
    else if (act_bf16 == 2) hipLaunchKernelGGL((embed_ln_kernel<CC, b3>), gk, blk, 0, st, x2d, x3d, temb, ew, eb, spos, lnw, lnb, eps, x, (bf16*)xn, plane, seq0, n_seq, H, F, J, SP);
    else if (act_bf16 == 3) hipLaunchKernelGGL((embed_ln_kernel<CC, h2>), gk, blk, 0, st, x2d, x3d, temb, ew, eb, spos, lnw, lnb, eps, x, (f16*)xn, plane, seq0, n_seq, H, F, J, SP);
    else hipLaunchKernelGGL((embed_ln_kernel<CC, float>), gk, blk, 0, st, x2d, x3d, temb, ew, eb, spos, lnw, lnb, eps, x, (float*)xn, plane, seq0, n_seq, H, F, J, SP))
  return 0;
}

int d3dp_launch_ln(int act_bf16, float* x, const void* yadd, int write_x, const float* w, const float* b, float eps,
                   void* xn, int T, int C, hipStream_t st) {
  dim3 g((T + 3) / 4), blk(256);
  const size_t plane = (size_t)T * C;
  if (!width_instantiated(C)) {
    if (act_bf16 != 0) return -2;
    DISPATCH_G(C, hipLaunchKernelGGL((ln_g_kernel<NVM>), g, blk, 0, st, x, (const float*)yadd, w, b, eps, (float*)xn, T, C, write_x))
    return 0;
  }
  DISPATCH_C(C,
    if (act_bf16 == 1) hipLaunchKernelGGL((ln_kernel<CC, bf16, bf16>), g, blk, 0, st, x, (const bf16*)yadd, w, b, eps, (bf16*)xn, plane, T, write_x);
    else if (act_bf16 == 4) hipLaunchKernelGGL((ln_kernel<CC, f16, f16>), g, blk, 0, st, x, (const f16*)yadd, w, b, eps, (f16*)xn, plane, T, write_x);
    else if (act_bf16 == 2) hipLaunchKernelGGL((ln_kernel<CC, b3, float>), g, blk, 0, st, x, (const float*)yadd, w, b, eps, (bf16*)xn, plane, T, write_x);
    else if (act_bf16 == 3) hipLaunchKernelGGL((ln_kernel<CC, h2, float>), g, blk, 0, st, x, (const float*)yadd, w, b, eps, (f16*)xn, plane, T, write_x);
    else hipLaunchKernelGGL((ln_kernel<CC, float, float>), g, blk, 0, st, x, (const float*)yadd, w, b, eps, (float*)xn, plane, T, write_x))
  return 0;
}

int d3dp_launch_ln2(int act_bf16, float* x, const void* yadd0, const void* yadd, const float* wa, const float* ba, const float* pos,
                    const float* wb, const float* bb, float eps, void* xn, int T, int C, int F, int J, hipStream_t st, int SP) {
  if (SP <= 0) SP = F * J;
  dim3 g((T + 3) / 4), blk(256);
  const size_t plane = (size_t)T * C;
  if (!width_instantiated(C)) {
    if (act_bf16 != 0) return -2;
    DISPATCH_G(C, hipLaunchKernelGGL((ln2_g_kernel<NVM>), g, blk, 0, st, x, (const float*)yadd0, (const float*)yadd, wa, ba, pos, wb, bb, eps, (float*)xn, T, C, F, J, SP))
    return 0;
  }
  DISPATCH_C(C,
    if (act_bf16 == 1) hipLaunchKernelGGL((ln2_kernel<CC, bf16, bf16>), g, blk, 0, st, x, (const bf16*)yadd0, (const bf16*)yadd, wa, ba, pos, wb, bb, eps, (bf16*)xn, plane, T, F, J, SP);
    else if (act_bf16 == 4) hipLaunchKernelGGL((ln2_kernel<CC, f16, f16>), g, blk, 0, st, x, (const f16*)yadd0, (const f16*)yadd, wa, ba, pos, wb, bb, eps, (f16*)xn, plane, T, F, J, SP);
    else if (act_bf16 == 2) hipLaunchKernelGGL((ln2_kernel<CC, b3, float>), g, blk, 0, st, x, (const float*)yadd0, (const float*)yadd, wa, ba, pos, wb, bb, eps, (bf16*)xn, plane, T, F, J, SP);
    else if (act_bf16 == 3) hipLaunchKernelGGL((ln2_kernel<CC, h2, float>), g, blk, 0, st, x, (const float*)yadd0, (const float*)yadd, wa, ba, pos, wb, bb, eps, (f16*)xn, plane, T, F, J, SP);
    else hipLaunchKernelGGL((ln2_kernel<CC, float, float>), g, blk, 0, st, x, (const float*)yadd0, (const float*)yadd, wa, ba, pos, wb, bb, eps, (float*)xn, plane, T, F, J, SP))
  return 0;
}

int d3dp_launch_head(int act_bf16, const float* x, const void* yadd0, const void* yadd, const float* wa, const float* ba, float eps_a, const float* wh,
                     const float* bh, float eps_h, const float* w, const float* b, float* out, int T, int C,
                     hipStream_t st, int FJ, int SP) {
  if (FJ <= 0 || SP <= 0) { FJ = SP = 1 << 30; }
  dim3 g((T + 3) / 4), blk(256);
  if (!width_instantiated(C)) {
    if (act_bf16 != 0) return -2;
    DISPATCH_G(C, hipLaunchKernelGGL((head_g_kernel<NVM>), g, blk, 0, st, x, (const float*)yadd0, (const float*)yadd, wa, ba, eps_a, wh, bh, eps_h, w, b, out, T, C, FJ, SP))
    return 0;
  }
  const dim3 gk((T + 4 * kRowTokens - 1) / (4 * kRowTokens));
  DISPATCH_C(C,
    if (act_bf16 == 1) hipLaunchKernelGGL((head_kernel<CC, bf16>), gk, blk, 0, st, x, (const bf16*)yadd0, (const bf16*)yadd, wa, ba, eps_a, wh, bh, eps_h, w, b, out, T, FJ, SP);
    else if (act_bf16 == 4) hipLaunchKernelGGL((head_kernel<CC, f16>), gk, blk, 0, st, x, (const f16*)yadd0, (const f16*)yadd, wa, ba, eps_a, wh, bh, eps_h, w, b, out, T, FJ, SP);
    else hipLaunchKernelGGL((head_kernel<CC, float>), gk, blk, 0, st, x, (const float*)yadd0, (const float*)yadd, wa, ba, eps_a, wh, bh, eps_h, w, b, out, T, FJ, SP))
  return 0;
}
```

Measured before the change: 51.35.

## Defer inter-stage LayerNorm write-back into the next proj GEMM residual epilogue

The ln2 kernel between stages no longer writes the normalized residual stream back to x. It records each row's mean and rstd and emits only the next block's normalized activations. The following proj GEMM then applies that pending norm inside a new EPI_RESID_NORM epilogue, using gamma and beta packed after the bias, before adding its output. This removes one full fp32 write of the residual stream per stage but adds reads of row stats and extra epilogue arithmetic. It also adds a separate mi%3 register-rotation read schedule.

```diff
diff --git a/d3dp_amd/csrc/capi.hip b/d3dp_amd/csrc/capi.hip
--- a/d3dp_amd/csrc/capi.hip
+++ b/d3dp_amd/csrc/capi.hip
@@ -68,6 +68,7 @@
   float qkv_u = 1.f, proj_u = 1.f, fc1_u = 1.f, fc2_u = 1.f;
   const float* fc1_c12 = nullptr;
   float s_kv = kActScale, s_h = kActScale;
+  const float* proj_bgb = nullptr;
 };
 
 template <typename E>
@@ -166,6 +167,10 @@
   bool fold = true;
   bool fold_ln() const { return fold_resid() && fold_ln_on && 2 * cfg.hidden <= 2048; }
   bool fold_ln_on = false;
+  bool defer_norm() const {
+    return fold_resid() && defer && !fold_ln() && skew_d == 0 && pingpong == 0 && cfg.channels >= 96 && 3 * cfg.channels <= 2048;
+  }
+  bool defer = true;
   bool skew() const { return x2_attn() && skew_d > 0 && cfg.channels >= 128 * skew_d; }
   int skew_d = 0;
   int seq_pitch() const {
@@ -313,7 +318,7 @@
 }
 
 int run_block(d3dp_ctx* c, const BlockDev& w, int axis, float* x, void* y1, void* y, void* bufA, void* bufB, float* lnst,
-              int n_bh, hipStream_t st) {
+              int n_bh, hipStream_t st, float* nstat = nullptr) {
   const d3dp_cfg& g = c->cfg;
   const int Tc = n_bh * c->seq_pitch(), C = g.channels;
   const float s_o = c->x2_attn() ? w.s_kv : kActScale;
@@ -330,7 +335,8 @@
     }
     LAUNCH_TRY(linear(c, P_FC1, EPI_GELU_LN, 0, y1, w.fc1_w, w.fc1_u, w.fc1_c12, bufB, Tc, g.hidden, C, st, bufB, rowstat, kActScale, w.s_h));
   } else {
-  LAUNCH_TRY(linear(c, P_PROJ, fold ? EPI_RESID : EPI_BIAS, 0, bufA, w.proj_w, w.proj_u, w.proj_b, fold ? (void*)x : y1, Tc, C, C, st, nullptr, nullptr, s_o));
+  if (nstat) LAUNCH_TRY(linear(c, P_PROJ, EPI_RESID_NORM, 0, bufA, w.proj_w, w.proj_u, w.proj_bgb, x, Tc, C, C, st, nullptr, nstat, s_o));
+  else LAUNCH_TRY(linear(c, P_PROJ, fold ? EPI_RESID : EPI_BIAS, 0, bufA, w.proj_w, w.proj_u, w.proj_b, fold ? (void*)x : y1, Tc, C, C, st, nullptr, nullptr, s_o));
   {
     Scope s(c, P_LN, st);
     LAUNCH_TRY(d3dp_launch_ln(c->act(), x, fold ? nullptr : y1, 0, w.n2w, w.n2b, g.eps_block, bufA, Tc, C, st));
@@ -354,6 +360,8 @@
   c->long_rows = lr && !strcmp(lr, "rows");
   const char* nf = getenv("D3DP_NO_FOLD");
   c->fold = !(nf && nf[0] == '1');
+  const char* dn = getenv("D3DP_DEFER_NORM");
+  c->defer = !(dn && dn[0] == '0');
   const char* ti = getenv("D3DP_TRAIN_IMPL");
   c->train_x2 = !(ti && !strcmp(ti, "f32")) && width_inst;
   const char* ov = getenv("D3DP_TRAIN_OVERLAP");
@@ -620,7 +628,7 @@
   const size_t i_tnw = add(w->temporal_norm_w, C, false), i_tnb = add(w->temporal_norm_b, C, false);
   const size_t i_hnw = add(w->head_norm_w, C, false), i_hnb = add(w->head_norm_b, C, false);
   const size_t i_hw = add(w->head_w, 3 * C, false), i_hb = add(w->head_b, 3, false);
-  struct BI { size_t v[13]; };
+  struct BI { size_t v[13]; bool bgb; };
   std::vector<BI> bis;
   std::vector<float*> temps;
   struct TempFree { std::vector<float*>& t; ~TempFree() { for (float* p : t) (void)hipFree(p); } } temp_free{temps};
@@ -633,6 +641,11 @@
       bi.v[0] = add(b.norm1_w, C, false); bi.v[1] = add(b.norm1_b, C, false);
       bi.v[2] = add(b.qkv_w, 3 * C * C, true); bi.v[3] = add(b.qkv_b, 3 * C, false);
       bi.v[4] = add(b.proj_w, C * C, true); bi.v[5] = add(b.proj_b, C, false);
+      bi.bgb = c->defer_norm() && (C * 4) % kAlign == 0;
+      if (bi.bgb) {
+        add(kind == 0 ? w->temporal_norm_w : w->spatial_norm_w, C, false);
+        add(kind == 0 ? w->temporal_norm_b : w->spatial_norm_b, C, false);
+      }
       bi.v[6] = add(b.norm2_w, C, false); bi.v[7] = add(b.norm2_b, C, false);
       if (c->fold_ln()) {
         float *wp = nullptr, *c12 = nullptr;
@@ -700,6 +713,7 @@
                F32(bi.v[11]), ANY(bi.v[2]), ANY(bi.v[4]), ANY(bi.v[8]), ANY(bi.v[10]),
                unscale[bi.v[2]], unscale[bi.v[4]], unscale[bi.v[8]], unscale[bi.v[10]], F32(bi.v[12]),
                blk_scale[2 * k], blk_scale[2 * k + 1]};
+    if (bi.bgb) b.proj_bgb = F32(bi.v[5]);
     (k < (size_t)g.depth ? c->ste : c->tte).push_back(b);
   }
   c->weights_set = true;
@@ -741,7 +755,8 @@
   const size_t wide = (size_t)std::max(3 * g.channels, g.hidden);
   *bytes = align_up((size_t)B * C * 4) + align_up(Tc * C * 4) + 2 * align_up(Tc * C * c->y_size()) +
            align_up(Tc * C * c->act_size()) + align_up(Tc * wide * c->wide_size()) +
-           (c->fold_ln() ? align_up(Tc * ((C + 63) / 64) * 8) + align_up((Tc + 256) * 8) : 0);
+           (c->fold_ln() ? align_up(Tc * ((C + 63) / 64) * 8) + align_up((Tc + 256) * 8) : 0) +
+           (c->defer_norm() ? align_up((Tc + 256) * 8) : 0);
   return D3DP_OK;
 }
 
@@ -767,6 +782,8 @@
   void* bufB = p;          p += align_up(Tmax * (size_t)std::max(3 * g.channels, g.hidden) * c->wide_size());
   float* lnst = (float*)p;
   c->ln_slice_floats = align_up(Tmax * ((C + 63) / 64) * 8) / 4;
+  if (c->fold_ln()) p += align_up(Tmax * ((C + 63) / 64) * 8) + align_up((Tmax + 256) * 8);
+  float* nstat = c->defer_norm() ? (float*)p : nullptr;
 
   {
     Scope s(c, P_TIME, st);
@@ -782,16 +799,23 @@
     }
     const bool fold = c->fold_resid();
     for (int d = 0; d < g.depth; ++d) {
-      int r = run_block(c, c->ste[d], 0, x, y1, y, bufA, bufB, lnst, n, st);
+      const bool defer = nstat != nullptr && c->ste[d].proj_bgb && c->tte[d].proj_bgb;
+      int r = run_block(c, c->ste[d], 0, x, y1, y, bufA, bufB, lnst, n, st, defer && d > 0 ? nstat : nullptr);
       if (r) return r;
-      {
+      if (defer && d > 0) {
+        Scope s(c, P_LN2, st);
+        LAUNCH_TRY(d3dp_launch_ln2_defer(c->act(), x, c->snw, c->snb, c->tte[d].n1w, c->tte[d].n1b, g.eps_block, bufA, nstat, Tc, C, st));
+      } else {
         Scope s(c, P_LN2, st);
         LAUNCH_TRY(d3dp_launch_ln2(c->act(), x, fold ? nullptr : y1, fold ? nullptr : y, c->snw, c->snb, d == 0 ? c->tpos : nullptr, c->tte[d].n1w,
                                    c->tte[d].n1b, g.eps_block, bufA, Tc, C, F, J, st, SP));
       }
-      r = run_block(c, c->tte[d], 1, x, y1, y, bufA, bufB, lnst, n, st);
+      r = run_block(c, c->tte[d], 1, x, y1, y, bufA, bufB, lnst, n, st, defer && d > 0 ? nstat : nullptr);
       if (r) return r;
-      if (d + 1 < g.depth) {
+      if (d + 1 < g.depth && defer) {
+        Scope s(c, P_LN2, st);
+        LAUNCH_TRY(d3dp_launch_ln2_defer(c->act(), x, c->tnw, c->tnb, c->ste[d + 1].n1w, c->ste[d + 1].n1b, g.eps_block, bufA, nstat, Tc, C, st));
+      } else if (d + 1 < g.depth) {
         Scope s(c, P_LN2, st);
         LAUNCH_TRY(d3dp_launch_ln2(c->act(), x, fold ? nullptr : y1, fold ? nullptr : y, c->tnw, c->tnb, nullptr, c->ste[d + 1].n1w, c->ste[d + 1].n1b,
                                    g.eps_block, bufA, Tc, C, F, J, st, SP));
@@ -956,7 +980,7 @@
     return fail(D3DP_ENOTSUP, "d3dp_op_linear_x2: epi flags %d select an experiment kernel this library was built without "
                               "(make -C d3dp_amd/csrc variants)", epi & ~0xff);
   epi &= 255;
-  if (epi == EPI_RESID_LN || epi == EPI_GELU_LN) return fail(D3DP_EINVAL, "d3dp_op_linear_x2: epilogues 5 / 6 are internal to d3dp_denoise");
+  if (epi == EPI_RESID_LN || epi == EPI_GELU_LN || epi == EPI_RESID_NORM) return fail(D3DP_EINVAL, "d3dp_op_linear_x2: epilogues 5 / 6 / 7 are internal to d3dp_denoise");
   if (skew_d) {
     int dev = 0;
     hipDeviceProp_t prop;
diff --git a/d3dp_amd/csrc/gemm_x2.hip b/d3dp_amd/csrc/gemm_x2.hip
--- a/d3dp_amd/csrc/gemm_x2.hip
+++ b/d3dp_amd/csrc/gemm_x2.hip
@@ -44,7 +44,7 @@
   const int t_flip = tiles_n_arg < 0 ? total_tiles - 1 : 0, t_sign = tiles_n_arg < 0 ? -1 : 1;
   auto tile_of = [&](int ti_) { return t_flip + t_sign * (L + ti_ * G); };
 
-  for (int i = tid; i < (EPI == EPI_GELU_LN ? 2 * N : N); i += (XNCW + 4) * 64) sbias[i] = bias[i];
+  for (int i = tid; i < (EPI == EPI_GELU_LN ? 2 * N : EPI == EPI_RESID_NORM ? 3 * N : N); i += (XNCW + 4) * 64) sbias[i] = bias[i];
   __syncthreads();
 
   if (wave >= XNCW) {
@@ -69,7 +69,7 @@
           pw[i] = W2 + (size_t)min(n0 + wrow, N - 1) * (2 * K) + swz128(row, lq) * 8;
         }
       }
-      if constexpr (EPI == EPI_GELU_LN) {
+      if constexpr (EPI == EPI_GELU_LN || EPI == EPI_RESID_NORM) {
         if (ks == 0 && lw == 0) {
           const int t = tile_of(ti);
           const float* rs = aux + (size_t)(t / tiles_n) * XBM * 2 + lane * 4;
@@ -196,6 +196,12 @@
         c1z = *reinterpret_cast<const float4*>(sbias + N + nb);
         srow = reinterpret_cast<const float*>(smem + XROWSTAT + (ti & 1) * (XBM * 8)) + (wr * 64 + 4 * fg) * 2;
       }
+      [[maybe_unused]] float4 gmz = {}, btz = {};
+      if constexpr (EPI == EPI_RESID_NORM) {
+        gmz = *reinterpret_cast<const float4*>(sbias + N + nb);
+        btz = *reinterpret_cast<const float4*>(sbias + 2 * N + nb);
+        srow = reinterpret_cast<const float*>(smem + XROWSTAT + (ti & 1) * (XBM * 8)) + (wr * 64 + 4 * fg) * 2;
+      }
       auto value = [&](int mi, int r, int e) {
         const float bze = e == 0 ? bz.x : e == 1 ? bz.y : e == 2 ? bz.z : bz.w;
         if constexpr (EPI == EPI_GELU_LN) {
@@ -228,7 +234,7 @@
                 ph[e] = h; pl[e] = l;
               }
               store_planes_paired(dst, ph, pl, odd, live);
-            } else if constexpr (EPI != EPI_RESID && EPI != EPI_RESID_LN) {
+            } else if constexpr (EPI != EPI_RESID && EPI != EPI_RESID_LN && EPI != EPI_RESID_NORM) {
               if (live) OUT_STORE(reinterpret_cast<f32x4*>(dst), ((f32x4){value(mi, r, 0), value(mi, r, 1), value(mi, r, 2), value(mi, r, 3)}));
             }
           }
@@ -253,6 +259,37 @@
                                res[mi][r][2] + value(mi, r, 2), res[mi][r][3] + value(mi, r, 3)};
               if (live) *reinterpret_cast<f32x4*>(base + (off + (unsigned)k * pitch)) = v;
             }
+        }
+        if constexpr (EPI == EPI_RESID_NORM && !decltype(planes_c)::value) {
+          f32x4 res[3][4];
+          auto read_block = [&](int mi, f32x4 (&dstv)[4]) {
+#pragma unroll
+            for (int r = 0; r < 4; ++r) {
+              const int k = mi * 16 + r;
+              const bool live = !decltype(checked_c)::value || k < rows;
+              dstv[r] = (f32x4){0.f, 0.f, 0.f, 0.f};
+              if (live) dstv[r] = *reinterpret_cast<const f32x4*>(base + (off + (unsigned)k * pitch));
+            }
+          };
+#pragma unroll
+          for (int mi = 0; mi < 3; ++mi) read_block(mi, res[mi]);
+#pragma unroll
+          for (int mi = 0; mi < 4; ++mi) {
+#pragma unroll
+            for (int r = 0; r < 4; ++r) {
+              const int k = mi * 16 + r;
+              const bool live = !decltype(checked_c)::value || k < rows;
+              const float2 st = *reinterpret_cast<const float2*>(srow + k * 2);
+              const f32x4 x = res[mi % 3][r];
+              const f32x4 v = {fmaf((x[0] - st.x) * st.y, gmz.x, btz.x) + value(mi, r, 0), fmaf((x[1] - st.x) * st.y, gmz.y, btz.y) + value(mi, r, 1),
+                               fmaf((x[2] - st.x) * st.y, gmz.z, btz.z) + value(mi, r, 2), fmaf((x[3] - st.x) * st.y, gmz.w, btz.w) + value(mi, r, 3)};
+              if (live) *reinterpret_cast<f32x4*>(base + (off + (unsigned)k * pitch)) = v;
+            }
+            if (mi == 0) {
+              __builtin_amdgcn_sched_barrier(0);
+              read_block(3, res[0]);
+            }
+          }
         }
         if constexpr (EPI == EPI_RESID_LN && !decltype(planes_c)::value) {
           auto rowsum16 = [](float x) {
@@ -391,7 +428,8 @@
   if (K % (2 * XBK) != 0 || N % 4 != 0 || N > XBIAS_MAX || M <= 0) return -1;
   if ((size_t)M * N * 4 >= ((size_t)1 << 32)) return -1;
   if (epi != EPI_BIAS && epi != EPI_GELU && epi != EPI_QKV_PACK && epi != EPI_RESID && epi != EPI_RESID_LN &&
-      epi != EPI_GELU_LN) return -1;
+      epi != EPI_GELU_LN && epi != EPI_RESID_NORM) return -1;
+  if (epi == EPI_RESID_NORM && (!aux || 3 * N > XBIAS_MAX || K / XBK < XNSTAGE)) return -1;
   if ((epi == EPI_RESID_LN || epi == EPI_GELU_LN) && (!aux || !out2)) return -1;
   if (epi == EPI_RESID_LN && !flag) return -1;
   if (epi == EPI_RESID_LN && N % 64 != 0) return -1;
@@ -402,15 +440,17 @@
   const int tm = (M + XBM - 1) / XBM, tn = (N + XBN - 1) / XBN;
   using KernT = void (*)(const f16*, const f16*, const float*, float, float, float*, f16*, float*, unsigned*, int, int, int, int, int);
 #if D3DP_X2_VARIANTS
-  constexpr int NKERN = 6;
+  constexpr int NKERN = 7;
   static const KernT kerns[NKERN] = {gemm_f16x2_kernel<EPI_BIAS, 0>, gemm_f16x2_kernel<EPI_BIAS, 1>,
                                      gemm_f16x2_kernel<EPI_GELU, 0>, gemm_f16x2_kernel<EPI_RESID, 0>,
+                                     gemm_f16x2_kernel<EPI_RESID_NORM, 0>,
                                      gemm_f16x2_kernel<EPI_RESID_LN, 0>, gemm_f16x2_kernel<EPI_GELU_LN, 0>};
 #else
   if (epi == EPI_RESID_LN || epi == EPI_GELU_LN || skew_d != 0 || pingpong != 0) return -2;
-  constexpr int NKERN = 4;
+  constexpr int NKERN = 5;
   static const KernT kerns[NKERN] = {gemm_f16x2_kernel<EPI_BIAS, 0>, gemm_f16x2_kernel<EPI_BIAS, 1>,
-                                     gemm_f16x2_kernel<EPI_GELU, 0>, gemm_f16x2_kernel<EPI_RESID, 0>};
+                                     gemm_f16x2_kernel<EPI_GELU, 0>, gemm_f16x2_kernel<EPI_RESID, 0>,
+                                     gemm_f16x2_kernel<EPI_RESID_NORM, 0>};
 #endif
   static PerDeviceOnce once;
   const int cus = once.get([&](int dev) {
@@ -424,8 +464,8 @@
   const int taken = x2_variants_launch(epi, A2, W2, bias, unscale, oscale, outf, out2, aux, flag, M, N, K, st, skew_d, pingpong, cus);
   if (taken <= 0) return taken;
 #endif
-  const KernT kern = kerns[epi == EPI_GELU ? 2 : epi == EPI_RESID ? 3 : epi == EPI_QKV_PACK ? 1 : epi == EPI_RESID_LN ? 4
-                           : epi == EPI_GELU_LN ? 5 : 0];
+  const KernT kern = kerns[epi == EPI_GELU ? 2 : epi == EPI_RESID ? 3 : epi == EPI_QKV_PACK ? 1 : epi == EPI_RESID_NORM ? 4
+                           : epi == EPI_RESID_LN ? 5 : epi == EPI_GELU_LN ? 6 : 0];
   hipLaunchKernelGGL(kern, dim3(grid), dim3((XNCW + 4) * 64), XLDS, st, (const f16*)A2, (const f16*)W2, bias, unscale, oscale, outf,
                      (f16*)out2, aux, flag, M, N, K, reverse ? -tn : tn, total);
   return 0;
diff --git a/d3dp_amd/csrc/kernels.h b/d3dp_amd/csrc/kernels.h
--- a/d3dp_amd/csrc/kernels.h
+++ b/d3dp_amd/csrc/kernels.h
@@ -29,7 +29,8 @@
   return hipFuncSetAttribute(kern, hipFuncAttributeMaxDynamicSharedMemorySize, bytes) == hipSuccess ? 1 : -3;
 }
 
-enum { EPI_BIAS = 0, EPI_GELU = 1, EPI_RESID = 2, EPI_PARTIAL = 3, EPI_QKV_PACK = 4, EPI_RESID_LN = 5, EPI_GELU_LN = 6 };
+enum { EPI_BIAS = 0, EPI_GELU = 1, EPI_RESID = 2, EPI_PARTIAL = 3, EPI_QKV_PACK = 4, EPI_RESID_LN = 5, EPI_GELU_LN = 6,
+       EPI_RESID_NORM = 7 };
 
 int d3dp_launch_linear_bf16_stream(int epi, int out_f32, const void* A, const void* W, const float* bias, void* out,
                                    int M, int N, int K, hipStream_t st, int f16 = 0);
@@ -118,6 +119,8 @@
 int d3dp_launch_ln2(int act_bf16, float* x, const void* yadd0, const void* yadd, const float* wa, const float* ba, const float* pos,
                     const float* wb, const float* bb, float eps, void* xn, int T, int C, int F, int J, hipStream_t st,
                     int SP = 0);
+int d3dp_launch_ln2_defer(int act_bf16, const float* x, const float* wa, const float* ba, const float* wb, const float* bb, float eps,
+                          void* xn, float* stat, int T, int C, hipStream_t st);
 int d3dp_launch_head(int act_bf16, const float* x, const void* yadd0, const void* yadd, const float* wa, const float* ba, float eps_a, const float* wh,
                      const float* bh, float eps_h, const float* w, const float* b, float* out, int T, int C,
                      hipStream_t st, int FJ = 0, int SP = 0);
diff --git a/d3dp_amd/csrc/pointwise.hip b/d3dp_amd/csrc/pointwise.hip
--- a/d3dp_amd/csrc/pointwise.hip
+++ b/d3dp_amd/csrc/pointwise.hip
@@ -146,8 +146,8 @@
       }
     }
   }
-  static __device__ __forceinline__ void norm(const float* v, const float* w, const float* b, float eps, int lane,
-                                              float* y) {
+  static __device__ __forceinline__ float2 norm(const float* v, const float* w, const float* b, float eps, int lane,
+                                                float* y) {
     float s = 0.f;
 #pragma unroll
     for (int i = 0; i < NV; ++i) s += v[i];
@@ -161,8 +161,9 @@
     load(b, lane, bv);
 #pragma unroll
     for (int i = 0; i < NV; ++i) y[i] = fmaf((v[i] - mean) * rstd, wv[i], bv[i]);
-  }
-  static __device__ __forceinline__ void norm_r(const float* v, const float* wv, const float* bv, float eps, float* y) {
+    return make_float2(mean, rstd);
+  }
+  static __device__ __forceinline__ float2 norm_r(const float* v, const float* wv, const float* bv, float eps, float* y) {
     float s = 0.f;
 #pragma unroll
     for (int i = 0; i < NV; ++i) s += v[i];
@@ -173,6 +174,7 @@
     const float rstd = 1.0f / sqrtf(wave_sum(q) * (1.0f / C) + eps);
 #pragma unroll
     for (int i = 0; i < NV; ++i) y[i] = fmaf((v[i] - mean) * rstd, wv[i], bv[i]);
+    return make_float2(mean, rstd);
   }
 };
 
@@ -250,6 +252,34 @@
   if (NT_STREAMS) R::store_nt(x + (size_t)tok * C, lane, y); else R::store(x + (size_t)tok * C, lane, y);
   R::norm(y, wb, bb, eps, lane, z);
   ActOut<C, XN>::st(xn, plane, (size_t)tok * C, lane, z);
+}
+
+constexpr int kDeferRows = 4;
+
+template <int C, typename XN>
+__global__ __launch_bounds__(256) void ln2_defer_kernel(const float* __restrict__ x, const float* __restrict__ wa,
+                                                        const float* __restrict__ ba, const float* __restrict__ wb,
+                                                        const float* __restrict__ bb, float eps,
+                                                        typename ActOut<C, XN>::ptr xn, float2* __restrict__ stat,
+                                                        size_t plane, int T) {
+  using R = Row<C>;
+  const int lane = threadIdx.x & 63;
+  const int wave = __builtin_amdgcn_readfirstlane(threadIdx.x >> 6);
+  float wav[R::NV], bav[R::NV], wbv[R::NV], bbv[R::NV];
+  R::load(wa, lane, wav);
+  R::load(ba, lane, bav);
+  R::load(wb, lane, wbv);
+  R::load(bb, lane, bbv);
+  for (int it = 0; it < kDeferRows; ++it) {
+    const int tok = (blockIdx.x * kDeferRows + it) * 4 + wave;
+    if (tok >= T) break;
+    float v[R::NV], y[R::NV], z[R::NV];
+    if (NT_STREAMS) R::load_nt(x + (size_t)tok * C, lane, v); else R::load(x + (size_t)tok * C, lane, v);
+    const float2 st = R::norm_r(v, wav, bav, eps, y);
+    if (lane == 0) stat[tok] = st;
+    R::norm_r(y, wbv, bbv, eps, z);
+    ActOut<C, XN>::st(xn, plane, (size_t)tok * C, lane, z);
+  }
 }
 
 constexpr int kRowTokens = 8;
@@ -628,6 +658,15 @@
   return 0;
 }
 
+int d3dp_launch_ln2_defer(int act_bf16, const float* x, const float* wa, const float* ba, const float* wb, const float* bb, float eps,
+                          void* xn, float* stat, int T, int C, hipStream_t st) {
+  if (act_bf16 != 3 || !stat || !width_instantiated(C)) return -2;
+  dim3 g((T + 4 * kDeferRows - 1) / (4 * kDeferRows)), blk(256);
+  const size_t plane = (size_t)T * C;
+  DISPATCH_C(C, hipLaunchKernelGGL((ln2_defer_kernel<CC, h2>), g, blk, 0, st, x, wa, ba, wb, bb, eps, (f16*)xn, (float2*)stat, plane, T))
+  return 0;
+}
+
 int d3dp_launch_head(int act_bf16, const float* x, const void* yadd0, const void* yadd, const float* wa, const float* ba, float eps_a, const float* wh,
                      const float* bh, float eps_h, const float* w, const float* b, float* out, int T, int C,
                      hipStream_t st, int FJ, int SP) {
```

Result: faster. 52.09, median of 6 (+1.4%).
